# courtois-neuromod/phantom_vlb

Hardware: AMD Instinct MI355X
Metric: clips/sec fine-tune VideoLLaMA2-7B+LoRA->2k-voxel head, 1/2/4/8 MI355X (higher is better)
Workload: dtype bf16; 1 GPU; configs[2]: VideoLLaMA2-7B + LoRA r=16 + 2k-voxel head, bf16; clips_per_gpu=3, global_batch=3, seq_len=2048, frames=12, num_target=2048, weights=random-init, comm=none

## Files before the change

include/vlb.h:

```cpp
#ifndef VLB_H
#define VLB_H

#include <stdint.h>

#ifdef __cplusplus
extern "C" {
#endif
#if defined(__GNUC__) || defined(__clang__)
#pragma GCC visibility push(default)
#endif

#define VLB_OK 0
#define VLB_ERR_INVALID (-1)
#define VLB_ERR_LAUNCH (-2)

#define VLB_ABI_VERSION 2

#define VLB_ACT_NONE 0
#define VLB_ACT_QUICK_GELU 1
#define VLB_ACT_GELU 2
#define VLB_ACT_SILU 3
#define VLB_ACT_SWIGLU_PAIR 4
#define VLB_ACT_SWIGLU_BWD 5

int vlb_abi_version(void);
const char* vlb_last_error(void);

int vlb_gemm_bf16(const void* A, int lda, const void* W, int ldw, void* C, int ldc, int M, int N, int K,
                  const void* bias, const void* residual, int ldr, int act, const void* A2, int lda2,
                  const void* W2, int ldw2, int K2, void* stream);

int vlb_gemm_bf16_ws(const void* A, int lda, const void* W, int ldw, void* C, int ldc, int M, int N, int K,
                     const void* bias, const void* residual, int ldr, int act, const void* A2, int lda2,
                     const void* W2, int ldw2, int K2, void* ws, int64_t ws_bytes, void* stream);
int vlb_gemm_swiglu_save(const void* A, int lda, const void* W_il, int ldw, void* H, int ldh, void* GU, int ldgu, int M, int N,
                         int K, const void* A2, int lda2, const void* W2_il, int ldw2, int K2, void* ws, int64_t ws_bytes,
                         void* stream);
int64_t vlb_gemm_workspace_bytes(void);
int vlb_gemm_plan(int M, int N, int K, int K2, int with_workspace);

int vlb_gemm_bf16_masked_pair(const void* A, int lda, const void* W, int ldw, void* C, int ldc, int M, int N, int K,
                              const void* A2, int lda2, const void* W2, int ldw2, float drop_p, uint32_t seed,
                              void* stream);

int vlb_gemm_bf16_masked_pair_ws(const void* A, int lda, const void* W, int ldw, void* C, int ldc, int M, int N, int K,
                                 const void* A2, int lda2, const void* W2, int ldw2, float drop_p, uint32_t seed,
                                 void* ws, int64_t ws_bytes, void* stream);

int vlb_gemm_masked_pair_swiglu_bwd(const void* dY, int lddy, const void* Wt, int ldw, const void* gu, int ldgu, void* dgu,
                                    int lddgu, int M, int ff, int K, const void* U, int ldu, const void* At, int ldat,
                                    float drop_p, uint32_t seed, void* ws, int64_t ws_bytes, void* stream);

int vlb_gemm_kernel_choice(int M, int N, int K, int K2);

int vlb_transpose_bf16(const void* in, void* out, int R, int C, void* stream);

int vlb_attention_fwd(const void* q, int ldq, const void* k, int ldk, const void* v, int ldv, void* out, int ldo,
                      float* lse, const uint8_t* key_mask, int B, int S, int Hq, int Hkv, int D, int causal,
                      float scale, const int* cu_rows, void* stream);

int vlb_attention_bwd(const void* q, int ldq, const void* k, int ldk, const void* v, int ldv, const void* out,
                      int ldo, const void* dout, int lddo, const float* lse, const uint8_t* key_mask, void* dq,
                      int lddq, void* dk, int lddk, void* dv, int lddv, float* delta, float* dq_acc, int B, int S,
                      int Hq, int Hkv, int D, int causal, float scale, const int* cu_rows, int total_rows,
                      void* stream);

int vlb_rmsnorm_fwd(const void* x, const void* w, void* y, int rows, int dim, float eps, void* stream);
int vlb_rmsnorm_bwd(const void* x, const void* w, const void* dy, const void* dx_in, void* dx, int rows, int dim,
                    float eps, void* stream);
int vlb_layernorm_fwd(const void* x, const void* w, const void* b, const void* residual, void* y, int rows, int dim,
                      float eps, int act, void* stream);

int vlb_rope_inplace(void* x, int ld, const float* cos_t, const float* sin_t, int rows, int S, int heads, int D,
                     int sign, const int* pos, void* stream);
int vlb_swiglu_fwd(const void* gu, void* out, int rows, int ff, void* stream);
int vlb_swiglu_bwd(const void* gu, const void* dout, void* dgu, int rows, int ff, void* stream);
int vlb_add_bf16(const void* a, const void* b, void* y, int64_t n, void* stream);

int vlb_patchify(const float* vision, void* patches, int N, int H, int W, int P, int Kpad, void* stream);
int vlb_vit_assemble(const void* patch_emb, const void* cls, const void* pos, void* tokens, int N, int G, int D,
                     void* stream);
int vlb_drop_cls(const void* tokens, void* out, int N, int G, int D, void* stream);

int vlb_dwconv3x3(const void* x, const void* w, void* y, int N, int H, int W, int C, void* stream);
int vlb_se_pool(const void* x, void* pooled, int N, int HW, int C, void* stream);
int vlb_se_scale(const void* x, const void* gate, void* y, int N, int HW, int C, void* stream);
int vlb_im2col3d_k2s2p1(const void* x, void* cols, int B, int T, int H, int W, int C, void* stream);

int vlb_splice_embed(const int64_t* ids, const void* embed_w, const void* video_tokens, void* embeds,
                     uint8_t* key_mask, int* err_flag, int B, int L, int Nv, int D, int64_t video_id, int vocab,
                     const int* cu_rows, int* row_pos, void* stream);
int vlb_weight_mask(const int64_t* padvals, const double* vis_w, const double* lang_w, float* wmask, int B, int F,
                    int Lw, int tokens_per_frame, int S, int round_bf16, void* stream);

int vlb_head_partial_rows(int S);
int64_t vlb_head_ws_floats(int B, int S, int E, int V);
int vlb_head_fwd(const void* hidden, const float* wmask, const void* ln1_w, const void* ln1_b, const void* ln2_w,
                 const void* ln2_b, const void* ridge_w, const void* ridge_b, const float* y, const float* keep_scale,
                 float* ws, float* stats, float* pooled_raw, float* sumw, float* zhat, float* ln2_rstd, void* z,
                 float* pred, float* loss_terms, int B, int S, int E, int V, float eps, float l2_lambda, const int* cu_rows,
                 void* stream);
int vlb_head_bwd(const void* hidden, const float* wmask, const void* ln1_w, const void* ln2_w, const void* ridge_w,
                 const float* y, const float* keep_scale, const float* stats, const float* pooled_raw,
                 const float* sumw, const float* zhat, const float* ln2_rstd, const void* z, const float* pred,
                 float* d_ridge_w, float* d_ridge_b, float* d_ln2_w, float* d_ln2_b, float* d_ln1_w, float* d_ln1_b,
                 float* ws, float* dz_ws, float* dpooled_ws, void* dhidden, int B, int S, int E, int V, float eps,
                 float l2_lambda, float loss_scale, float l2_scale, const int* cu_rows, int total_rows, void* stream);

int vlb_feature_cache_store(const float* pooled_raw, const float* sumw, const int32_t* rows, float* cache_pooled,
                            float* cache_sumw, int B, int E, int n_rows, void* stream);
int vlb_head_fwd_cached(const float* cache_pooled, const float* cache_sumw, const int32_t* rows, const void* ln1_w,
                        const void* ln1_b, const void* ln2_w, const void* ln2_b, const void* ridge_w, const void* ridge_b,
                        const float* y, const float* keep_scale, float* ws, float* pooled_raw, float* sumw, float* zhat,
                        float* ln2_rstd, void* z, float* pred, float* loss_terms, int B, int E, int V, int n_rows, float eps,
                        float l2_lambda, void* stream);
int vlb_head_bwd_cached(const void* ln1_w, const void* ln2_w, const void* ridge_w, const float* y, const float* keep_scale,
                        const float* pooled_raw, const float* sumw, const float* zhat, const float* ln2_rstd, const void* z,
                        const float* pred, float* d_ridge_w, float* d_ridge_b, float* d_ln2_w, float* d_ln2_b, float* d_ln1_w,
                        float* d_ln1_b, float* ws, float* dz_ws, float* dpooled_ws, int B, int E, int V, float eps,
                        float l2_lambda, float loss_scale, float l2_scale, void* stream);

int vlb_lora_down(const void* x, int ldx, const void* A, void* t, int ldt, int M, int K, int R, float scale,
                  float drop_p, const uint32_t* seeds_host, void* stream);
int vlb_lora_merge(const void* W, int ldw, void* Wm, int ldwm, const void* Bt, const void* A, int N, int K, int R, float scale,
                   int row_map, void* stream);
int vlb_lora_dx_masked(const void* u, int ldu, const void* At, int ldat, void* dx, int lddx, int M, int K, int R, float drop_p,
                       const uint32_t* seeds_host, void* stream);
int64_t vlb_wgrad_u_ws_floats(int M, int K);
int vlb_wgrad_skinny_u(const void* G, int ldg, const void* X, int ldx, float* dW, float* ws, int M, int K, float alpha,
                       float beta, const void* Bt, float u_scale, void* u, int ldu, float* u_ws, void* stream);
int vlb_wgrad_skinny_u_multi(const void* G, int ldg, const void* X, int ldx, int M, int nproj, const int* cols, float* const* dW,
                             const void* const* Bt, float* ws, float alpha, float beta, float u_scale, void* u, int ldu,
                             float* u_ws, void* stream);
int vlb_transpose16_scatter(const void* jobs, int n_jobs, void* stream);
int vlb_wgrad_splits(int M);
int vlb_wgrad_skinny(const void* G, int ldg, const void* X, int ldx, float* dW, float* ws, int M, int N, int K,
                     float alpha, float beta, float drop_p, const uint32_t* seeds_host, void* stream);

int vlb_sumsq_ws_floats(void);
int vlb_grad_sumsq(const float* g, int64_t n, float* sumsq, float* ws, void* stream);
int vlb_adamw_step(float* master, void* param_bf16, const float* grad, float* m, float* v, int64_t n, float lr,
                   float beta1, float beta2, float eps, float weight_decay, int step, const float* sumsq,
                   float max_norm, void* stream);
int vlb_grad_accum(float* acc, const float* g, int64_t n, int first, float* sumsq, float* ws, void* stream);
int vlb_grad_accum_bf16(float* acc, const void* g_bf16, int64_t n, int first, float* sumsq, float* ws, void* stream);

int vlb_transpose_pad(const void* in, int ld_in, void* out, int ld_out, int R, int C, int Rpad, void* stream);
int64_t vlb_norm_bwd_ws_floats(int rows, int dim);
int64_t vlb_colsum_ws_floats(int rows, int dim);
int vlb_rmsnorm_bwd_dw(const void* x, const void* dy, void* dw_bf16, float* ws, int rows, int dim, float eps, void* stream);
int64_t vlb_rmsnorm_bwd_full_ws_floats(int rows, int dim);
int vlb_rmsnorm_bwd_full(const void* x, const void* w, const void* dy, const void* dx_in, void* dx, void* dw_bf16, float* ws,
                         int rows, int dim, float eps, void* stream);
int vlb_layernorm_bwd(const void* x, const void* w, const void* b, const void* residual, const void* dy, void* dx, void* dres,
                      void* dw_bf16, void* db_bf16, float* ws, int rows, int dim, float eps, int act, void* stream);
int vlb_act_fwd(const void* x, void* y, int64_t n, int act, void* stream);
int vlb_act_bwd(const void* x, const void* dy, void* dx, int64_t n, int act, void* stream);
int vlb_colsum(const void* x, int ld, void* out_bf16, float* ws, int rows, int dim, void* stream);
int vlb_embed_grad(const void* d_embeds, int ld, const int* tok, const int* beg, const int* rows, int n_tokens, void* dE, int D,
                   void* stream);
int vlb_grad_sumsq_bf16(const void* g, int64_t n, float* sumsq, float* ws, void* stream);
int vlb_adamw_step_g16(float* master, void* param_bf16, const void* grad_bf16, float* m, float* v, int64_t n, float lr,
                       float beta1, float beta2, float eps, float weight_decay, int step, const float* sumsq, float max_norm,
                       void* stream);
int64_t vlb_dwconv3x3_bwd_w_ws_floats(int N, int H, int C);
int vlb_dwconv3x3_bwd_w(const void* x, const void* dy, void* dw9_bf16, float* ws, int N, int H, int W, int C, void* stream);
int vlb_se_bwd_gate(const void* x, const void* dy, const void* s, void* ds, int N, int HW, int C, void* stream);
int vlb_se_bwd_x(const void* dy, const void* s, const void* dpool, void* dx, int N, int HW, int C, void* stream);
int vlb_col2im3d_k2s2p1(const void* dcols, void* dx, int B, int T, int H, int W, int C, void* stream);

int vlb_quantize_mxfp8(const void* x_bf16, int ldx, void* q, int ldq, void* scales, int lds, int rows, int K, void* stream);
int vlb_transpose_quantize_mxfp8(const void* x_bf16, int ldx, void* q, int ldq, void* scales, int lds, int R, int C, int Rpad,
                                 void* stream);
int vlb_quantize_dual_mxfp8(const void* x_bf16, int ldx, void* q, int ldq, void* scales, int lds, void* qt, int ldqt, void* scales_t,
                            int ldst, int R, int C, int Rpad, void* stream);
int vlb_rmsnorm_fwd_mxfp8(const void* x, const void* w, void* y, void* q, int ldq, void* scales, int lds, int rows, int dim, float eps,
                          void* stream);
int vlb_swiglu_fwd_mxfp8(const void* gu, void* out, void* q, int ldq, void* scales, int lds, int rows, int ff, void* stream);
int vlb_gemm_mxfp8(const void* Aq, int lda, const void* sA, int ldsa, const void* Wq, int ldw, const void* sW, int ldsw, void* C,
                   int ldc, int M, int N, int K, const void* residual, int ldr, void* stream);

int vlb_comm_unique_id(void* id128_host);
int vlb_comm_init(int rank, int world, const void* id128_host, void** comm_out);
int vlb_comm_destroy(void* comm);
int64_t vlb_comm_loopback_stage_bytes(int world);
int vlb_comm_init_loopback(int world, void* stage, int64_t stage_bytes, void** comms_out);
int vlb_comm_rank(void* comm);
int vlb_comm_world(void* comm);
int vlb_allgather_direct(void* comm, const void* shard, void* full, int64_t shard_bytes, void* stream);
int64_t vlb_reducescatter_stage_floats(int64_t n_per_rank, int world);
int vlb_reducescatter_direct(void* comm, const float* send, float* out, int64_t n_per_rank, float* stage, void* stream);
int vlb_reducescatter_direct_bf16(void* comm, const void* send, void* out, int64_t n_per_rank, void* stage, void* stream);
int vlb_reduce_slices(const void* stage, void* out, int64_t n_per_rank, int world, int is_bf16, void* stream);
int vlb_allreduce_scalar(void* comm, float* values, int count, void* stream);

int64_t vlb_hrf_pool_ws_floats(int B, int E);
int vlb_hrf_pool(const void* embeddings, int emb_is_f32, const float* weights, void* out, float* ws, int B, int S, int E, void* stream);
int64_t vlb_ridge_ws_floats(int V);
int vlb_ridge_fwd(const void* x, const void* ridge_w, const void* ridge_b, float* pred, float* l2_out, float* ws, int B, int E, int V,
                  float l2_lambda, void* stream);

int vlb_dropout_keep_scale(float* out, int64_t n, float p, uint32_t seed, void* stream);

int vlb_profile_marker(void* stream);
int vlb_cast_f32_to_bf16(const float* in, void* out, int64_t n, void* stream);
int vlb_cast_bf16_to_f32(const void* in, float* out, int64_t n, void* stream);

#if defined(__GNUC__) || defined(__clang__)
#pragma GCC visibility pop
#endif
#ifdef __cplusplus
}
#endif
#endif
```

phantom_vlb_amd/_lib.py:

```python
from __future__ import annotations

import ctypes
import os
from ctypes import c_char_p, c_double, c_float, c_int, c_int64, c_void_p

import torch

_HERE = os.path.dirname(os.path.abspath(__file__))
LIB_PATH = os.environ.get("VLB_LIB") or os.path.join(_HERE, "libvlb.so")
IS_PRODUCT_LIB = os.path.abspath(LIB_PATH) == os.path.join(_HERE, "libvlb.so")

P, I, F, L = c_void_p, c_int, c_float, c_int64

SIGNATURES = {
    "vlb_abi_version": [],
    "vlb_last_error": [],
    "vlb_gemm_bf16": [P, I, P, I, P, I, I, I, I, P, P, I, I, P, I, P, I, I, P],
    "vlb_gemm_bf16_ws": [P, I, P, I, P, I, I, I, I, P, P, I, I, P, I, P, I, I, P, L, P],
    "vlb_gemm_swiglu_save": [P, I, P, I, P, I, P, I, I, I, I, P, I, P, I, I, P, L, P],
    "vlb_gemm_workspace_bytes": [],
    "vlb_gemm_plan": [I, I, I, I, I],
    "vlb_gemm_kernel_choice": [I, I, I, I],
    "vlb_transpose_bf16": [P, P, I, I, P],
    "vlb_attention_fwd": [P, I, P, I, P, I, P, I, P, P, I, I, I, I, I, I, F, P, P],
    "vlb_attention_bwd": [P, I, P, I, P, I, P, I, P, I, P, P, P, I, P, I, P, I, P, P, I, I, I, I, I, I, F, P, I, P],
    "vlb_rmsnorm_fwd": [P, P, P, I, I, F, P],
    "vlb_rmsnorm_bwd": [P, P, P, P, P, I, I, F, P],
    "vlb_layernorm_fwd": [P, P, P, P, P, I, I, F, I, P],
    "vlb_rope_inplace": [P, I, P, P, I, I, I, I, I, P, P],
    "vlb_swiglu_fwd": [P, P, I, I, P],
    "vlb_swiglu_bwd": [P, P, P, I, I, P],
    "vlb_add_bf16": [P, P, P, L, P],
    "vlb_patchify": [P, P, I, I, I, I, I, P],
    "vlb_vit_assemble": [P, P, P, P, I, I, I, P],
    "vlb_drop_cls": [P, P, I, I, I, P],
    "vlb_dwconv3x3": [P, P, P, I, I, I, I, P],
    "vlb_se_pool": [P, P, I, I, I, P],
    "vlb_se_scale": [P, P, P, I, I, I, P],
    "vlb_im2col3d_k2s2p1": [P, P, I, I, I, I, I, P],
    "vlb_splice_embed": [P, P, P, P, P, P, I, I, I, I, L, I, P, P, P],
    "vlb_weight_mask": [P, P, P, P, I, I, I, I, I, I, P],
    "vlb_head_partial_rows": [I],
    "vlb_head_ws_floats": [I, I, I, I],
    "vlb_head_fwd": [P] * 19 + [I, I, I, I, F, F, P, P],
    "vlb_head_bwd": [P] * 24 + [I, I, I, I, F, F, F, F, P, I, P],
    "vlb_feature_cache_store": [P] * 5 + [I, I, I, P],
    "vlb_head_fwd_cached": [P] * 19 + [I, I, I, I, F, F, P],
    "vlb_head_bwd_cached": [P] * 20 + [I, I, I, F, F, F, F, P],
    "vlb_gemm_bf16_masked_pair": [P, I, P, I, P, I, I, I, I, P, I, P, I, F, ctypes.c_uint32, P],
    "vlb_gemm_masked_pair_swiglu_bwd": [P, I, P, I, P, I, P, I, I, I, I, P, I, P, I, F, ctypes.c_uint32, P, L, P],
    "vlb_gemm_bf16_masked_pair_ws": [P, I, P, I, P, I, I, I, I, P, I, P, I, F, ctypes.c_uint32, P, L, P],
    "vlb_wgrad_u_ws_floats": [I, I],
    "vlb_wgrad_skinny_u": [P, I, P, I, P, P, I, I, F, F, P, F, P, I, P, P],
    "vlb_wgrad_skinny_u_multi": [P, I, P, I, I, I, P, P, P, P, F, F, F, P, I, P, P],
    "vlb_transpose16_scatter": [P, I, P],
    "vlb_wgrad_splits": [I],
    "vlb_wgrad_skinny": [P, I, P, I, P, P, I, I, I, F, F, F, P, P],
    "vlb_lora_down": [P, I, P, P, I, I, I, I, F, F, P, P],
    "vlb_lora_merge": [P, I, P, I, P, P, I, I, I, F, I, P],
    "vlb_lora_dx_masked": [P, I, P, I, P, I, I, I, I, F, P, P],
    "vlb_sumsq_ws_floats": [],
    "vlb_grad_sumsq": [P, L, P, P, P],
    "vlb_adamw_step": [P, P, P, P, P, L, F, F, F, F, F, I, P, F, P],
    "vlb_grad_accum": [P, P, L, I, P, P, P],
    "vlb_grad_accum_bf16": [P, P, L, I, P, P, P],
    "vlb_dropout_keep_scale": [P, L, F, ctypes.c_uint32, P],
    "vlb_transpose_pad": [P, I, P, I, I, I, I, P],
    "vlb_norm_bwd_ws_floats": [I, I],
    "vlb_colsum_ws_floats": [I, I],
    "vlb_rmsnorm_bwd_dw": [P, P, P, P, I, I, F, P],
    "vlb_rmsnorm_bwd_full_ws_floats": [I, I],
    "vlb_rmsnorm_bwd_full": [P, P, P, P, P, P, P, I, I, F, P],
    "vlb_layernorm_bwd": [P, P, P, P, P, P, P, P, P, P, I, I, F, I, P],
    "vlb_act_fwd": [P, P, L, I, P],
    "vlb_act_bwd": [P, P, P, L, I, P],
    "vlb_colsum": [P, I, P, P, I, I, P],
    "vlb_embed_grad": [P, I, P, P, P, I, P, I, P],
    "vlb_grad_sumsq_bf16": [P, L, P, P, P],
    "vlb_adamw_step_g16": [P, P, P, P, P, L, F, F, F, F, F, I, P, F, P],
    "vlb_dwconv3x3_bwd_w_ws_floats": [I, I, I],
    "vlb_dwconv3x3_bwd_w": [P, P, P, P, I, I, I, I, P],
    "vlb_se_bwd_gate": [P, P, P, P, I, I, I, P],
    "vlb_se_bwd_x": [P, P, P, P, I, I, I, P],
    "vlb_col2im3d_k2s2p1": [P, P, I, I, I, I, I, P],
    "vlb_quantize_mxfp8": [P, I, P, I, P, I, I, I, P],
    "vlb_transpose_quantize_mxfp8": [P, I, P, I, P, I, I, I, I, P],
    "vlb_quantize_dual_mxfp8": [P, I, P, I, P, I, P, I, P, I, I, I, I, P],
    "vlb_rmsnorm_fwd_mxfp8": [P, P, P, P, I, P, I, I, I, F, P],
    "vlb_swiglu_fwd_mxfp8": [P, P, P, I, P, I, I, I, P],
    "vlb_gemm_mxfp8": [P, I, P, I, P, I, P, I, P, I, I, I, I, P, I, P],
    "vlb_comm_unique_id": [P],
    "vlb_comm_init": [I, I, P, ctypes.POINTER(c_void_p)],
    "vlb_comm_destroy": [P],
    "vlb_comm_loopback_stage_bytes": [I],
    "vlb_comm_init_loopback": [I, P, L, ctypes.POINTER(c_void_p)],
    "vlb_comm_rank": [P],
    "vlb_comm_world": [P],
    "vlb_allgather_direct": [P, P, P, L, P],
    "vlb_reducescatter_stage_floats": [L, I],
    "vlb_reducescatter_direct": [P, P, P, L, P, P],
    "vlb_reducescatter_direct_bf16": [P, P, P, L, P, P],
    "vlb_reduce_slices": [P, P, L, I, I, P],
    "vlb_profile_marker": [P],
    "vlb_hrf_pool_ws_floats": [I, I],
    "vlb_hrf_pool": [P, I, P, P, P, I, I, I, P],
    "vlb_ridge_ws_floats": [I],
    "vlb_ridge_fwd": [P, P, P, P, P, P, I, I, I, F, P],
    "vlb_allreduce_scalar": [P, P, I, P],
    "vlb_cast_f32_to_bf16": [P, P, L, P],
    "vlb_cast_bf16_to_f32": [P, P, L, P],
}
_RESTYPES = {"vlb_last_error": c_char_p, "vlb_hrf_pool_ws_floats": c_int64, "vlb_ridge_ws_floats": c_int64, "vlb_head_ws_floats": c_int64, "vlb_wgrad_u_ws_floats": c_int64,
             "vlb_gemm_workspace_bytes": c_int64, "vlb_reducescatter_stage_floats": c_int64, "vlb_comm_loopback_stage_bytes": c_int64,
             "vlb_norm_bwd_ws_floats": c_int64, "vlb_rmsnorm_bwd_full_ws_floats": c_int64, "vlb_colsum_ws_floats": c_int64, "vlb_dwconv3x3_bwd_w_ws_floats": c_int64}


class VlbError(RuntimeError):
    pass


def _load():
    if not os.path.exists(LIB_PATH):
        raise ImportError(
            f"{LIB_PATH} is missing: build it with `python -c 'import __graft_entry__ as g; g.build()'` "
            f"or `make -C phantom_vlb_amd/csrc`.  phantom_vlb_amd has no CPU fallback.")
    lib = ctypes.CDLL(LIB_PATH)
    for name, argtypes in SIGNATURES.items():
        try:
            fn = getattr(lib, name)
        except AttributeError as e:
            raise ImportError(f"libvlb.so does not export {name}: rebuild it") from e
        fn.argtypes = argtypes
        fn.restype = _RESTYPES.get(name, c_int)
    if lib.vlb_abi_version() != 2:
        raise ImportError("libvlb.so ABI version mismatch")
    return lib


lib = _load()


def check(rc: int, what: str = "") -> None:
    if rc != 0:
        raise VlbError(f"{what} failed ({rc}): {lib.vlb_last_error().decode()}")
```

phantom_vlb_amd/backbone.py:

```python
from __future__ import annotations

import math

import torch

from . import ops
from .geometry import Geometry, VIDEO_TOKEN_ID

BF16 = torch.bfloat16
V_PRE = "model.vision_tower.vision_tower.vision_model"
M_PRE = "model.mm_projector"


def _bf(t, dev):
    return t.detach().to(device=dev, dtype=BF16).contiguous()


class Weights:

    def __init__(self, g: Geometry, sd: dict, device, keep_transposed: bool = False, gate_up_interleaved: bool | None = None):
        self.g = g
        self.dev = device
        d = device
        w = sd[f"{V_PRE}.embeddings.patch_embedding.weight"].reshape(g.vit_dim, -1)
# ... 51 lines not shown
                                    sd[f"{p}.self_attn.v_proj.weight"]], 0), d),
                wo=_bf(sd[f"{p}.self_attn.o_proj.weight"], d),
                wdown=_bf(sd[f"{p}.mlp.down_proj.weight"], d))
            il = (not keep_transposed) if gate_up_interleaved is None else gate_up_interleaved
            wgu = _bf(torch.cat([sd[f"{p}.mlp.gate_proj.weight"], sd[f"{p}.mlp.up_proj.weight"]], 0), d)
            if keep_transposed:
                lw["wgu"] = wgu
                for k in ("wqkv", "wo", "wgu", "wdown"):
                    lw[k + "_t"] = ops.transpose(lw[k])
                if il:
                    del lw["wgu"]
            if il:
                lw["wgu_il"] = ops.interleave_gate_up(wgu[:g.ff], wgu[g.ff:])
            del wgu
            self.layers.append(lw)
        self.final_norm = _bf(sd["model.norm.weight"], d)
        inv = 1.0 / (g.rope_theta ** (torch.arange(0, g.head_dim, 2, dtype=torch.float32) / g.head_dim))
        fr = torch.arange(g.max_len, dtype=torch.float32)[:, None] * inv[None]
        self.rope_cos = fr.cos().to(d).contiguous()
        self.rope_sin = fr.sin().to(d).contiguous()

    @staticmethod
    def random_state_dict(g: Geometry, device, seed: int = 1234, dtype=BF16) -> dict:
        gen = torch.Generator(device=device).manual_seed(seed)

        def rn(*shape, std=0.02):
            return (torch.randn(*shape, generator=gen, device=device, dtype=torch.float32) * std).to(dtype)

        def ones(n):
            return torch.ones(n, device=device, dtype=dtype)

        def zeros(n):
            return torch.zeros(n, device=device, dtype=dtype)
        sd = {}
        sd[f"{V_PRE}.embeddings.class_embedding"] = rn(g.vit_dim)
        sd[f"{V_PRE}.embeddings.patch_embedding.weight"] = rn(g.vit_dim, 3, g.patch, g.patch)
        sd[f"{V_PRE}.embeddings.position_embedding.weight"] = rn(g.grid * g.grid + 1, g.vit_dim)
        sd[f"{V_PRE}.pre_layrnorm.weight"] = ones(g.vit_dim)
        sd[f"{V_PRE}.pre_layrnorm.bias"] = zeros(g.vit_dim)
        for i in range(g.vit_layers):
            p = f"{V_PRE}.encoder.layers.{i}"
            for ln in ("layer_norm1", "layer_norm2"):
                sd[f"{p}.{ln}.weight"] = ones(g.vit_dim)
                sd[f"{p}.{ln}.bias"] = zeros(g.vit_dim)
            for n in ("q_proj", "k_proj", "v_proj", "out_proj"):
                sd[f"{p}.self_attn.{n}.weight"] = rn(g.vit_dim, g.vit_dim)
                sd[f"{p}.self_attn.{n}.bias"] = zeros(g.vit_dim)
            sd[f"{p}.mlp.fc1.weight"] = rn(g.vit_ff, g.vit_dim)
            sd[f"{p}.mlp.fc1.bias"] = zeros(g.vit_ff)
            sd[f"{p}.mlp.fc2.weight"] = rn(g.vit_dim, g.vit_ff)
            sd[f"{p}.mlp.fc2.bias"] = zeros(g.vit_dim)
        for st, cin in (("s1", g.vit_dim), ("s2", g.dim)):
            for b in range(g.proj_depth):
                ci = cin if b == 0 else g.dim
                q = f"{M_PRE}.{st}.b{b + 1}"
                rd = int(round(ci * g.proj_se_ratio))
                sd[f"{q}.conv1.conv.weight"] = rn(g.dim, ci, 1, 1, std=1 / math.sqrt(ci))
                sd[f"{q}.conv2.conv.weight"] = rn(g.dim, 1, 3, 3, std=1 / 3)
                sd[f"{q}.se.fc1.weight"] = rn(rd, g.dim, 1, 1, std=1 / math.sqrt(g.dim))
                sd[f"{q}.se.fc1.bias"] = zeros(rd)
                sd[f"{q}.se.fc2.weight"] = rn(g.dim, rd, 1, 1, std=1 / math.sqrt(rd))
                sd[f"{q}.se.fc2.bias"] = zeros(g.dim)
                sd[f"{q}.conv3.conv.weight"] = rn(g.dim, g.dim, 1, 1, std=1 / math.sqrt(g.dim))
                for n in ("conv1", "conv2", "conv3"):
                    sd[f"{q}.{n}.bn.weight"] = ones(g.dim)
                    sd[f"{q}.{n}.bn.bias"] = zeros(g.dim)
                if ci != g.dim:
                    sd[f"{q}.downsample.conv.weight"] = rn(g.dim, ci, 1, 1, std=1 / math.sqrt(ci))
                    sd[f"{q}.downsample.bn.weight"] = ones(g.dim)
                    sd[f"{q}.downsample.bn.bias"] = zeros(g.dim)
        sd[f"{M_PRE}.sampler.0.weight"] = rn(g.dim, g.dim, 2, 2, 2, std=1 / math.sqrt(8 * g.dim))
        sd[f"{M_PRE}.sampler.0.bias"] = zeros(g.dim)
        for n in ("readout.0", "readout.2"):
            sd[f"{M_PRE}.{n}.weight"] = rn(g.dim, g.dim, std=1 / math.sqrt(g.dim))
            sd[f"{M_PRE}.{n}.bias"] = zeros(g.dim)
        sd["model.embed_tokens.weight"] = rn(g.vocab, g.dim)
        for i in range(g.layers):
            p = f"model.layers.{i}"
            sd[f"{p}.self_attn.q_proj.weight"] = rn(g.heads * g.head_dim, g.dim)
            sd[f"{p}.self_attn.k_proj.weight"] = rn(g.kv_heads * g.head_dim, g.dim)
            sd[f"{p}.self_attn.v_proj.weight"] = rn(g.kv_heads * g.head_dim, g.dim)
            sd[f"{p}.self_attn.o_proj.weight"] = rn(g.dim, g.heads * g.head_dim)
            sd[f"{p}.mlp.gate_proj.weight"] = rn(g.ff, g.dim)
            sd[f"{p}.mlp.up_proj.weight"] = rn(g.ff, g.dim)
            sd[f"{p}.mlp.down_proj.weight"] = rn(g.dim, g.ff)
            sd[f"{p}.input_layernorm.weight"] = ones(g.dim)
            sd[f"{p}.post_attention_layernorm.weight"] = ones(g.dim)
        sd["model.norm.weight"] = ones(g.dim)
        return sd


class Backbone:

    def __init__(self, g: Geometry, weights: Weights):
        self.g = g
        self.w = weights
        self.err_flag = torch.zeros(1, dtype=torch.int32, device=weights.dev)

    def vision_tower(self, vision_f32):
        g, w = self.g, self.w
        N = vision_f32.shape[0]
        G, T = g.grid * g.grid, g.grid * g.grid + 1
        hd = g.vit_dim // g.vit_heads
        patches = ops.patchify(vision_f32, g.patch, g.patch_k_padded)
        pe = ops.gemm(patches, w.patch_w)
        x = ops.vit_assemble(pe, w.cls, w.pos, N, G, g.vit_dim)
        x = ops.layernorm(x, *w.pre_ln, g.vit_eps)
        D = g.vit_dim
        for lw in w.vit:
            h = ops.layernorm(x, *lw["ln1"], g.vit_eps)
            qkv = ops.gemm(h, lw["wqkv"], bias=lw["bqkv"])
            a = ops.attention_fwd(qkv[:, :D], qkv[:, D:2 * D], qkv[:, 2 * D:], N, T, g.vit_heads, g.vit_heads, hd,
                                  False, hd ** -0.5)
            x = ops.gemm(a, lw["wo"], bias=lw["bo"], residual=x)
            h = ops.layernorm(x, *lw["ln2"], g.vit_eps)
            h = ops.gemm(h, lw["w1"], bias=lw["b1"], act=ops.ACT_QUICK_GELU)
            x = ops.gemm(h, lw["w2"], bias=lw["b2"], residual=x)
        return ops.drop_cls(x, N, G, D)

    def _bottleneck(self, x, blk, N, H):
        g = self.g
        C = g.dim
        y = ops.gemm(x, blk["conv1"])
        y = ops.layernorm(y, *blk["bn1"], g.proj_eps, act=ops.ACT_SILU)
        y = ops.dwconv3x3(y, blk["dw"], N, H, H, C)
        y = ops.layernorm(y, *blk["bn2"], g.proj_eps, act=ops.ACT_SILU)
        s = ops.se_pool(y, N, H * H, C)
        s = ops.gemm(s, blk["se1"], bias=blk["se1b"], act=ops.ACT_SILU)
        s = ops.gemm(s, blk["se2"], bias=blk["se2b"])
        y = ops.se_scale(y, s, N, H * H, C, out=y)
        y = ops.gemm(y, blk["conv3"])
        sc = x
        if "ds" in blk:
            sc = ops.layernorm(ops.gemm(x, blk["ds"]), *blk["dsbn"], g.proj_eps)
        return ops.layernorm(y, *blk["bn3"], g.proj_eps, residual=sc, act=ops.ACT_SILU)

    def connector(self, feats, B):
        g, w = self.g, self.w
        x = feats
        for blk in w.s1:
            x = self._bottleneck(x, blk, B * g.num_frames, g.grid)
        cols = ops.im2col3d(x, B, g.num_frames, g.grid, g.grid, g.dim)
        x = ops.gemm(cols, w.sampler_w, bias=w.sampler_b, act=ops.ACT_SILU)
        for blk in w.s2:
            x = self._bottleneck(x, blk, B * g.ds_frames, g.ds_grid)
        x = ops.gemm(x, w.ro0[0], bias=w.ro0[1], act=ops.ACT_GELU)
        return ops.gemm(x, w.ro2[0], bias=w.ro2[1])

    def decoder_layer(self, x, lw, key_mask, B, S, save=None, layout=None):
        g = self.g
        qd, kd = g.heads * g.head_dim, g.kv_heads * g.head_dim
        h = ops.rmsnorm(x, lw["in_norm"], g.rms_eps)
        qkv = ops.gemm(h, lw["wqkv"])
        ops.rope_(qkv, self.w.rope_cos, self.w.rope_sin, B, S, g.heads + g.kv_heads, g.head_dim,
                  pos=None if layout is None else layout.pos)
        a = ops.attention_fwd(qkv[:, :qd], qkv[:, qd:qd + kd], qkv[:, qd + kd:], B, S, g.heads, g.kv_heads, g.head_dim,
                              True, g.head_dim ** -0.5, key_mask=key_mask, layout=layout)
        x = ops.gemm(a, lw["wo"], residual=x)
        h = ops.rmsnorm(x, lw["post_norm"], g.rms_eps)
        if lw.get("wgu_il") is not None:
            h = ops.gemm(h, lw["wgu_il"], act=ops.ACT_SWIGLU_PAIR)
        else:
            h = ops.swiglu(ops.gemm(h, lw["wgu"]))
        return ops.gemm(h, lw["wdown"], residual=x)

    def named_modules(self):
        from .litmodule import _LinearInfo
        g = self.g
        qd, kd = g.heads * g.head_dim, g.kv_heads * g.head_dim
        for i in range(g.vit_layers):
            p = f"{V_PRE}.encoder.layers.{i}"
            for n in ("q_proj", "k_proj", "v_proj", "out_proj"):
                yield f"{p}.self_attn.{n}", _LinearInfo(g.vit_dim, g.vit_dim)
            yield f"{p}.mlp.fc1", _LinearInfo(g.vit_ff, g.vit_dim)
            yield f"{p}.mlp.fc2", _LinearInfo(g.vit_dim, g.vit_ff)
        for n in ("readout.0", "readout.2"):
            yield f"{M_PRE}.{n}", _LinearInfo(g.dim, g.dim)
        for i in range(g.layers):
            p = f"model.layers.{i}"
            yield f"{p}.self_attn.q_proj", _LinearInfo(qd, g.dim)
            yield f"{p}.self_attn.k_proj", _LinearInfo(kd, g.dim)
            yield f"{p}.self_attn.v_proj", _LinearInfo(kd, g.dim)
            yield f"{p}.self_attn.o_proj", _LinearInfo(g.dim, qd)
            yield f"{p}.mlp.gate_proj", _LinearInfo(g.ff, g.dim)
            yield f"{p}.mlp.up_proj", _LinearInfo(g.ff, g.dim)
            yield f"{p}.mlp.down_proj", _LinearInfo(g.dim, g.ff)
        yield "lm_head", _LinearInfo(g.vocab, g.dim)

    def splice(self, ids, video_tokens, layout=None):
        g = self.g
        return ops.splice_embed(ids, self.w.embed, video_tokens, g.vis_tokens, VIDEO_TOKEN_ID, self.err_flag, layout)

    def row_layout(self, ids_host=None, padvals=None):
        g = self.g
        if ids_host is None or ids_host.device.type != "cpu":
            return None
        B, L = ids_host.shape
        S = L - 1 + g.vis_tokens
        nz = ids_host != 0
        last = L - 1 - torch.flip(nz, dims=[1]).to(torch.int8).argmax(dim=1)
        lens = (last + g.vis_tokens).clamp(max=S)
        lens = torch.where(nz.any(dim=1), lens, torch.full_like(lens, S))
        if padvals is not None:
            lens = torch.maximum(lens, S - padvals[:, 0].to(lens.dtype).cpu().clamp(min=0))
        return ops.RowLayout(B, S, lens.tolist(), device=self.w.dev)

    def enable_sharding(self, group=None, comm=None):
        from .parallel import ShardedLayerStore
        if getattr(self, "trainable_decoder", False):
            raise ValueError("enable_sharding(): the decoder weights train in this configuration (full fine-tune); "
                             "only frozen decoder weights can be sharded per layer")
        side = torch.cuda.Stream(device=self.w.dev)
        keys = tuple(k for k in ("wqkv", "wo", "wgu", "wgu_il", "wdown") if k in self.w.layers[0])
        self.store = ShardedLayerStore(self.w.layers, keys, group, stream=side, comm=comm)
        self.store_t = None
        if "wqkv_t" in self.w.layers[0]:
            tkeys = ("wqkv_t", "wo_t", "wgu_t", "wdown_t")
            self.store_t = ShardedLayerStore(self.w.layers, tkeys, group, stream=side, comm=comm)
        for lw in self.w.layers:
            for k in list(lw):
                if k in keys or k.endswith("_t"):
                    lw[k] = None
        torch.cuda.empty_cache()

    def layer_weights(self, i, transposed=False, direction=1):
        lw = self.w.layers[i]
        store = getattr(self, "store_t" if transposed else "store", None)
        if store is None:
            return lw
        full = store.get(i)
        store.prefetch(i + direction)
        return {**lw, **full}

    def decoder(self, x, key_mask, B, S, layer_outputs=None, layout=None, layers=None):
        for i in range(len(self.w.layers)):
            lw = self.layer_weights(i) if layers is None else layers[i]
            x = self.decoder_layer(x, lw, key_mask, B, S, layout=layout)
            if layer_outputs is not None:
                layer_outputs.append(x)
        return ops.rmsnorm(x, self.w.final_norm, self.g.rms_eps)

    MAX_AHEAD = 4

    def _vision_compute(self, vision_f32, tower_only):
        g, B = self.g, vision_f32.shape[0]
        feats = self.vision_tower(vision_f32.reshape(B * g.num_frames, 3, g.image_size, g.image_size))
        return feats if tower_only else self.connector(feats, B)

    def prefetch_video_tokens(self, vision_f32, ready_event=None, tower_only=False):
        dev = self.w.dev
        if getattr(self, "_vis_stream", None) is None:
            self._vis_stream = torch.cuda.Stream(device=dev)
        if getattr(self, "_vis_queue", None) is None:
            self._vis_queue = []
        st = self._vis_stream
        if ready_event is not None:
            st.wait_event(ready_event)
        else:
            st.wait_stream(torch.cuda.current_stream(dev))
        with torch.cuda.stream(st):
            vid = self._vision_compute(vision_f32, tower_only)
            ev = torch.cuda.Event()
            ev.record(st)
        vision_f32.record_stream(st)
        self._vis_queue.append((vision_f32, vision_f32._version, tower_only, vid, ev))
        del self._vis_queue[:-self.MAX_AHEAD]

    def defer_video_tokens(self, vision_f32, ready_event=None, tower_only=False):
        if getattr(self, "_vis_pending", None) is None:
            self._vis_pending = []
        self._vis_pending.append((vision_f32, vision_f32._version, tower_only, ready_event))
        del self._vis_pending[:-self.MAX_AHEAD]

    def launch_deferred_video_tokens(self):
        pend, self._vis_pending = getattr(self, "_vis_pending", None) or [], []
        for vis, ver, tower_only, ev in pend:
            if vis._version == ver:
                self.prefetch_video_tokens(vis, ev, tower_only=tower_only)

    def discard_video_tokens(self, vision_f32=None):
        for name in ("_vis_queue", "_vis_pending"):
            q = getattr(self, name, None)
            if q:
                q[:] = [e for e in q if vision_f32 is not None and e[0] is not vision_f32]

    def video_tokens(self, vision_f32, tower_only=False):
        q = getattr(self, "_vis_queue", None)
        cur = torch.cuda.current_stream(self.w.dev)
        if q:
            for i, (vis, ver, t_only, vid, ev) in enumerate(q):
                if vis is not vision_f32:
                    continue
                del q[i]
                if ver != vision_f32._version or (t_only is False and tower_only):
                    break
                cur.wait_event(ev)
                vid.record_stream(cur)
                if t_only and not tower_only:
                    return self.connector(vid, vision_f32.shape[0])
                return vid
        pend = getattr(self, "_vis_pending", None)
        if pend:
            for i, (vis, ver, t_only, ev) in enumerate(pend):
                if vis is vision_f32:
                    del pend[i]
                    if ev is not None:
                        cur.wait_event(ev)
                    break
        return self._vision_compute(vision_f32, tower_only)

# ... 17 lines not shown
```

phantom_vlb_amd/csrc/attention.hip:

```cpp
#include "common.hpp"

namespace {

constexpr int KV = 64;
constexpr int QW = 32;
constexpr int NW = 4;
constexpr int QB = QW * NW;
constexpr float NEG = -1e30f;

__device__ __forceinline__ void glds16(const void* g, void* l) {
  __builtin_amdgcn_global_load_lds((const void __attribute__((address_space(1)))*)g,
                                   (void __attribute__((address_space(3)))*)l, 16, 0, 0);
}

typedef short s16x4 __attribute__((ext_vector_type(4)));

__device__ __forceinline__ s16x4 tr_read_asm(const char* lds_ptr) {
  s16x4 v;
  const unsigned a = (unsigned)(uintptr_t)(const char __attribute__((address_space(3)))*)lds_ptr;
  asm volatile("ds_read_b64_tr_b16 %0, %1" : "=v"(v) : "v"(a));
  return v;
}
__device__ __forceinline__ void lds_wait_all() {
  asm volatile("s_waitcnt lgkmcnt(0)" ::: "memory");
  __builtin_amdgcn_sched_barrier(0);
}
__device__ __forceinline__ bf16x8 join8(s16x4 lo, s16x4 hi) {
  typedef short s16x8 __attribute__((ext_vector_type(8)));
  return __builtin_bit_cast(bf16x8, (s16x8)__builtin_shufflevector(lo, hi, 0, 1, 2, 3, 4, 5, 6, 7));
}

struct AttnArgs {
  const bf16* q; const bf16* k; const bf16* v; bf16* o; float* lse;
  const uint8_t* mask;
  const int* cu;
  int ldq, ldk, ldv, ldo;
  int B, S, Hq, Hkv;
  float scale;
};

template <int D> __device__ __forceinline__ int slot_k(int r, int c) {
  if constexpr (D == 128) return c ^ (r & 15); else return c ^ ((r >> 1) & 7);
}
template <int D> __device__ __forceinline__ int slot_v(int r, int c) {
  if constexpr (D == 128) return c ^ ((r & 3) << 2); else return c ^ (((r >> 1) & 1) << 2);
}

__device__ __forceinline__ int xcd_head(int j, int Hq) {
  return (Hq & 7) == 0 ? (j & 7) * (Hq >> 3) + (j >> 3) : j;
}

template <int D, bool CAUSAL>
__global__ __launch_bounds__(256, 2) void attn_fwd_kernel(AttnArgs p) {
  constexpr int CPR = D / 8;
  constexpr int ROWB = D * 2;
  constexpr int TILE = KV * ROWB;
  constexpr int LD = (KV * CPR) / 256;
  constexpr int KS = D / 16;
  constexpr int DT = D / 32;
  extern __shared__ __attribute__((aligned(16))) char smem[];

  const int tid = threadIdx.x, lane = tid & 63;
  const int wave = __builtin_amdgcn_readfirstlane(tid >> 6);
  const int nqb = (p.S + QB - 1) / QB;
  const int per_qb = p.Hq * p.B, slot = blockIdx.x / per_qb;
  const int qb = CAUSAL ? (nqb - 1 - slot) : slot;
  const int hq = xcd_head((blockIdx.x % per_qb) % p.Hq, p.Hq), b = (blockIdx.x % per_qb) / p.Hq;
  const int hkv = hq / (p.Hq / p.Hkv);
  const int Sb = p.cu ? p.cu[b + 1] - p.cu[b] : p.S;
  const int64_t row0 = p.cu ? p.cu[b] : (int64_t)b * p.S;
  if (qb * QB >= Sb) return;
  const int q0 = qb * QB + wave * QW;
  const int ql = lane & 31, h = lane >> 5;

  bf16x8 qf[KS];
  {
    const int qr = min(q0 + ql, Sb - 1);
    const bf16* qp = p.q + (row0 + qr) * p.ldq + hq * D + 8 * h;
#pragma unroll
    for (int ks = 0; ks < KS; ++ks) qf[ks] = *reinterpret_cast<const bf16x8*>(qp + 16 * ks);
  }

  f32x16 ot[DT];
#pragma unroll
  for (int i = 0; i < DT; ++i)
#pragma unroll
    for (int r = 0; r < 16; ++r) ot[i][r] = 0.f;
  float m_run = NEG, l_run = 0.f;
  const float c2 = p.scale * 1.44269504088896341f;

  const int q_hi = min(qb * QB + QB, Sb) - 1;
  const int ntiles = CAUSAL ? (q_hi / KV + 1) : (Sb + KV - 1) / KV;

  const bf16* kbase = p.k + row0 * p.ldk + hkv * D;
  const bf16* vbase = p.v + row0 * p.ldv + hkv * D;

  constexpr int RPI = 1024 / ROWB;
  const int sr = lane / CPR, sp = lane % CPR;
  auto stage = [&](int buf, int t) {
    char* kb = smem + buf * 2 * TILE; char* vb = kb + TILE;
#pragma unroll
    for (int i = 0; i < LD; ++i) {
      const int r = (4 * i + wave) * RPI + sr;
      const int key = min(t * KV + r, Sb - 1);
      glds16(kbase + (int64_t)key * p.ldk + slot_k<D>(r, sp) * 8, kb + (4 * i + wave) * 1024);
      glds16(vbase + (int64_t)key * p.ldv + slot_v<D>(r, sp) * 8, vb + (4 * i + wave) * 1024);
    }
  };

  stage(0, 0);
  asm volatile("s_waitcnt vmcnt(0)" ::: "memory");
  __syncthreads();

  const int g1 = (lane >> 4) & 1, li = lane & 15, tq = li >> 2, tp = li & 3;
  int k_rd[KS], v_rd[DT];
#pragma unroll
  for (int ks = 0; ks < KS; ++ks) k_rd[ks] = ql * ROWB + slot_k<D>(ql, 2 * ks + h) * 16;
#pragma unroll
  for (int dt = 0; dt < DT; ++dt) {
    const int r0 = 4 * h + tq;
    v_rd[dt] = r0 * ROWB + slot_v<D>(r0, 4 * dt + 2 * g1 + (tp >> 1)) * 16 + (tp & 1) * 8;
  }

  for (int t = 0; t < ntiles; ++t) {
    const int cur = t & 1;
    const bool more = (t + 1 < ntiles);
    if (more) stage(cur ^ 1, t + 1);
    const char* kb = smem + cur * 2 * TILE; const char* vb = kb + TILE;
    const int key0 = t * KV;
    const bool active = !CAUSAL || (key0 <= q0 + QW - 1);
    if (active) {
      f32x16 st[2];
#pragma unroll
      for (int s = 0; s < 2; ++s)
#pragma unroll
        for (int r = 0; r < 16; ++r) st[s][r] = 0.f;
#pragma unroll
      for (int ks = 0; ks < KS; ++ks) {
#pragma unroll
        for (int s = 0; s < 2; ++s) {
          const bf16x8 kf = *reinterpret_cast<const bf16x8*>(kb + k_rd[ks] + 32 * s * ROWB);
          st[s] = __builtin_amdgcn_mfma_f32_32x32x16_bf16(kf, qf[ks], st[s], 0, 0, 0);
        }
      }
      unsigned long long kvalid;
      {
        const int key = key0 + lane;
        bool ok = key < Sb;
        if (ok && p.mask) ok = p.mask[row0 + key] != 0;
        kvalid = __ballot(ok);
      }
      const bool diag = CAUSAL && (key0 + KV - 1 > q0);
      const bool partial = diag || (kvalid != ~0ull);
      if (partial) {
        const int qrow = q0 + ql;
        const unsigned lo = (unsigned)(kvalid >> (4 * h)), hi = (unsigned)(kvalid >> (32 + 4 * h));
#pragma unroll
        for (int s = 0; s < 2; ++s) {
          const unsigned word = s ? hi : lo;
#pragma unroll
          for (int r = 0; r < 16; ++r) {
            const int kb = (r & 3) + 8 * (r >> 2);
            bool ok = (word >> kb) & 1u;
            if (CAUSAL) ok = ok && (key0 + 32 * s + 4 * h + kb <= qrow);
            st[s][r] = ok ? st[s][r] : NEG;
          }
        }
        asm volatile("" ::: "memory");
      }
      float mloc = fmaxf(st[0][0], st[1][0]);
#pragma unroll
      for (int r = 1; r < 16; ++r) mloc = fmaxf(fmaxf(mloc, st[0][r]), st[1][r]);
      mloc = fmaxf(mloc, __shfl_xor(mloc, 32, 64));
      const float m_new = fmaxf(m_run, mloc);
      const float alpha = __builtin_amdgcn_exp2f((m_run - m_new) * c2);
      const float mc = m_new * c2;
      float lsum = 0.f;
      const float live = (m_new > 0.5f * NEG) ? 1.f : 0.f;
#pragma unroll
      for (int s = 0; s < 2; ++s)
#pragma unroll
        for (int r = 0; r < 16; ++r) {
          const float e = __builtin_amdgcn_exp2f(st[s][r] * c2 - mc);
          st[s][r] = e;
          lsum += e;
        }
      if (partial && live == 0.f) {
#pragma unroll
        for (int s = 0; s < 2; ++s)
#pragma unroll
          for (int r = 0; r < 16; ++r) st[s][r] = 0.f;
        lsum = 0.f;
      }
      l_run = l_run * alpha + lsum;
      m_run = m_new;
#pragma unroll
      for (int i = 0; i < DT; ++i)
#pragma unroll
        for (int r = 0; r < 16; ++r) ot[i][r] *= alpha;
#pragma unroll
      for (int s = 0; s < 2; ++s)
#pragma unroll
        for (int s2 = 0; s2 < 2; ++s2) {
          bf16x8 pf;
#pragma unroll
          for (int j = 0; j < 8; ++j) pf[j] = (bf16)st[s][8 * s2 + j];
          const int roff = (32 * s + 16 * s2) * ROWB;
#pragma unroll
          for (int dt = 0; dt < DT; ++dt) {
            const s16x4 lo = __builtin_amdgcn_ds_read_tr16_b64_v4i16(
                (s16x4 __attribute__((address_space(3)))*)(vb + v_rd[dt] + roff));
            const s16x4 hi = __builtin_amdgcn_ds_read_tr16_b64_v4i16(
                (s16x4 __attribute__((address_space(3)))*)(vb + v_rd[dt] + roff + 8 * ROWB));
            ot[dt] = __builtin_amdgcn_mfma_f32_32x32x16_bf16(join8(lo, hi), pf, ot[dt], 0, 0, 0);
          }
        }
    }
    asm volatile("s_waitcnt vmcnt(0)" ::: "memory");
    __syncthreads();
  }

  const float l_tot = l_run + __shfl_xor(l_run, 32, 64);
  const float inv = l_tot > 0.f ? 1.f / l_tot : 0.f;
  const int qrow = q0 + ql;
  if (qrow < Sb) {
    bf16* op = p.o + (row0 + qrow) * p.ldo + hq * D;
#pragma unroll
    for (int dt = 0; dt < DT; ++dt)
#pragma unroll
      for (int g = 0; g < 4; ++g) {
        bf16x4 o;
#pragma unroll
        for (int e = 0; e < 4; ++e) o[e] = (bf16)(ot[dt][4 * g + e] * inv);
        *reinterpret_cast<bf16x4*>(op + 32 * dt + 8 * g + 4 * h) = o;
      }
    if (p.lse && h == 0)
      p.lse[((int64_t)b * p.Hq + hq) * p.S + qrow] = l_tot > 0.f ? m_run * p.scale + logf(l_tot) : -INFINITY;
  }
}

template <int D, bool CAUSAL>
int launch_fwd(const AttnArgs& a, hipStream_t s) {
  constexpr int LDS = 2 * 2 * KV * D * 2;
  static const hipError_t attr = hipFuncSetAttribute(reinterpret_cast<const void*>(&attn_fwd_kernel<D, CAUSAL>),
                                                     hipFuncAttributeMaxDynamicSharedMemorySize, LDS);
  if (attr != hipSuccess) { vlb_set_error("attention: LDS reservation failed: %s", hipGetErrorString(attr)); return VLB_ERR_LAUNCH; }
  dim3 grid(((a.S + QB - 1) / QB) * a.Hq * a.B);
  hipLaunchKernelGGL((attn_fwd_kernel<D, CAUSAL>), grid, dim3(256), LDS, s, a);
  VLB_LAUNCH_CHECK();
  return VLB_OK;
}
}

extern "C" int vlb_attention_fwd(const void* q, int ldq, const void* k, int ldk, const void* v, int ldv, void* out,
                                 int ldo, float* lse, const uint8_t* key_mask, int B, int S, int Hq, int Hkv, int D,
                                 int causal, float scale, const int* cu_rows, void* stream) {
  VLB_REQUIRE(q && k && v && out, "attention_fwd: null operand");
  VLB_REQUIRE(D == 64 || D == 128, "attention_fwd: head dim %d not in {64,128}", D);
  VLB_REQUIRE(B > 0 && S > 0 && Hq > 0 && Hkv > 0 && Hq % Hkv == 0, "attention_fwd: bad shape B=%d S=%d Hq=%d Hkv=%d", B, S, Hq, Hkv);
  VLB_REQUIRE(ldq % 8 == 0 && ldk % 8 == 0 && ldv % 8 == 0 && ldo % 4 == 0, "attention_fwd: strides must keep 16-byte alignment");
  VLB_REQUIRE((((uintptr_t)q | (uintptr_t)k | (uintptr_t)v) % 16 == 0) && ((uintptr_t)out % 8 == 0), "attention_fwd: misaligned pointer");
  AttnArgs a{(const bf16*)q, (const bf16*)k, (const bf16*)v, (bf16*)out, lse, key_mask, cu_rows, ldq, ldk, ldv, ldo, B, S, Hq, Hkv, scale};
  hipStream_t s = as_stream(stream);
  if (D == 128) return causal ? launch_fwd<128, true>(a, s) : launch_fwd<128, false>(a, s);
  return causal ? launch_fwd<64, true>(a, s) : launch_fwd<64, false>(a, s);
}

namespace {

constexpr int BK_KEYS = 128;
constexpr int BQ = 32;

#ifdef VLB_TOOLS
int g_attn_ablate = 0;
#else
constexpr int g_attn_ablate = 0;
#endif
struct AttnBwdArgs {
  const bf16* q; const bf16* k; const bf16* v; const bf16* dout;
  const float* lse; const float* delta; const uint8_t* mask; const int* cu;
  bf16* dk; bf16* dv; float* dq_acc;
  int ldq, ldk, ldv, lddo, lddk, lddv;
  int B, S, Hq, Hkv;
  float scale;
  int ablate;
};

__device__ __forceinline__ int sw2(int r) { return ((r & 3) << 2) | ((r >> 2) & 3); }

__global__ __launch_bounds__(256) void attn_delta_kernel(const bf16* __restrict__ o, int ldo, const bf16* __restrict__ d_o,
                                                         int lddo, float* __restrict__ delta, int S, int Hq, int B,
                                                         const int* __restrict__ cu, int64_t total) {
  const int64_t gid = (int64_t)blockIdx.x * 16 + (threadIdx.x >> 4);
  const int c = threadIdx.x & 15;
  float s = 0.f;
  if (gid < total) {
    const int h = gid % Hq; const int64_t tok = gid / Hq;
    const bf16x8 a = *reinterpret_cast<const bf16x8*>(o + tok * ldo + h * 128 + c * 8);
    const bf16x8 b = *reinterpret_cast<const bf16x8*>(d_o + tok * lddo + h * 128 + c * 8);
#pragma unroll
    for (int i = 0; i < 8; ++i) s += (float)a[i] * (float)b[i];
  }
#pragma unroll
  for (int off = 8; off > 0; off >>= 1) s += __shfl_xor(s, off, 64);
  if (gid < total && c == 0) {
    const int h = gid % Hq; const int64_t tok = gid / Hq;
    int64_t b = tok / S; int sidx = tok % S;
    if (cu) {
      int bb = 0;
      while (bb + 1 < B && tok >= cu[bb + 1]) ++bb;
      b = bb; sidx = (int)(tok - cu[bb]);
    }
    delta[(b * Hq + h) * S + sidx] = s;
  }
}

template <bool CAUSAL>
__global__ __launch_bounds__(256, 2) void attn_bwd_dkdv_kernel(AttnBwdArgs p, bf16* __restrict__ part) {
  constexpr int D = 128, ROWB = 256;
  constexpr int V_OFF = 0;
  constexpr int QT_BYTES = BQ * ROWB;
  constexpr int Q_OFF = BK_KEYS * ROWB;
  constexpr int L_OFF = Q_OFF + 4 * QT_BYTES;
  extern __shared__ __attribute__((aligned(16))) char smem[];

  const int tid = threadIdx.x, lane = tid & 63;
  const int w4 = __builtin_amdgcn_readfirstlane(tid >> 6);
  const int per_kb = p.Hq * p.B;
  const int kb = blockIdx.x / per_kb, hq = xcd_head((blockIdx.x % per_kb) % p.Hq, p.Hq), b = (blockIdx.x % per_kb) / p.Hq;
  const int gsz = p.Hq / p.Hkv;
  const int hkv = hq / gsz;
  const int k0 = kb * BK_KEYS;
  const int Sb = p.cu ? p.cu[b + 1] - p.cu[b] : p.S;
  const int64_t row0 = p.cu ? p.cu[b] : (int64_t)b * p.S;
  if (k0 >= Sb) return;
  const int ql = lane & 31, h = lane >> 5;
  const int g1 = (lane >> 4) & 1, li = lane & 15, tq = li >> 2, tp = li & 3;
  const int sr = lane >> 4, sp = lane & 15;

  const int krow = w4 * 32 + ql;
  const int key = k0 + krow;
  bf16x8 kf[8];
  {
    const bf16* kp = p.k + (row0 + min(key, Sb - 1)) * p.ldk + hkv * D + 8 * h;
#pragma unroll
    for (int ks = 0; ks < 8; ++ks) kf[ks] = *reinterpret_cast<const bf16x8*>(kp + 16 * ks);
  }
  const bf16* vbase = p.v + row0 * p.ldv + hkv * D;
#pragma unroll
  for (int i = 0; i < 8; ++i) {
    const int piece = 4 * i + w4, r = piece * 4 + sr;
    glds16(vbase + (int64_t)min(k0 + r, Sb - 1) * p.ldv + (sp ^ sw2(r)) * 8, smem + V_OFF + piece * 1024);
  }
  const int nqb = (Sb + BQ - 1) / BQ;
  const int qb0 = CAUSAL ? (k0 / BQ) : 0;
  const int total = nqb - qb0;
  const bf16* qbase = p.q + row0 * p.ldq + hq * D;
  const bf16* dobase = p.dout + row0 * p.lddo + hq * D;
  const float* lsebase = p.lse + ((int64_t)b * p.Hq + hq) * p.S;
  const float* delbase = p.delta + ((int64_t)b * p.Hq + hq) * p.S;

  auto stage_q = [&](int buf, int item) {
    const int qb = qb0 + item;
    char* qt = smem + Q_OFF + buf * 2 * QT_BYTES;
#pragma unroll
    for (int i = 0; i < 2; ++i) {
      const int piece = 4 * i + w4, r = piece * 4 + sr;
      const int qr = min(qb * BQ + r, Sb - 1);
      glds16(qbase + (int64_t)qr * p.ldq + (sp ^ sw2(r)) * 8, qt + piece * 1024);
      glds16(dobase + (int64_t)qr * p.lddo + (sp ^ sw2(r)) * 8, qt + QT_BYTES + piece * 1024);
    }
    if (w4 == 0) {
      const int qr = min(qb * BQ + (lane & 31), Sb - 1);
      const float* src = (lane < 32 ? lsebase : delbase) + qr;
      __builtin_amdgcn_global_load_lds((const void __attribute__((address_space(1)))*)src,
                                       (void __attribute__((address_space(3)))*)(smem + L_OFF + buf * 256), 4, 0, 0);
    }
  };

  f32x16 dkt[4], dvt[4];
#pragma unroll
  for (int i = 0; i < 4; ++i)
#pragma unroll
    for (int r = 0; r < 16; ++r) { dkt[i][r] = 0.f; dvt[i][r] = 0.f; }

  if (total > 0) stage_q(0, 0);
  asm volatile("s_waitcnt vmcnt(0)" ::: "memory");
  __syncthreads();

  const int v_base = krow * ROWB, v_x = h ^ sw2(krow);
  const int q_base = ql * ROWB, q_x = h ^ sw2(ql);
  int qt_rd[4][2];
#pragma unroll
  for (int dt = 0; dt < 4; ++dt)
#pragma unroll
    for (int e = 0; e < 2; ++e) {
      const int r = 8 * e + 4 * h + tq;
      qt_rd[dt][e] = r * ROWB + (((4 * dt + 2 * g1 + (tp >> 1)) ^ sw2(r)) << 4) + (tp & 1) * 8;
    }

  const float c2 = p.scale * 1.44269504088896341f;
  bool key_ok = key < Sb;
  if (key_ok && p.mask) key_ok = p.mask[row0 + key] != 0;

  for (int item = 0; item < total; ++item) {
    const int cur = item & 1;
    if (item + 1 < total) stage_q(cur ^ 1, item + 1);
    const char* qt = smem + Q_OFF + cur * 2 * QT_BYTES;
    const char* dot = qt + QT_BYTES;
    const float* ls = reinterpret_cast<const float*>(smem + L_OFF) + cur * 64;
    const int q0 = (qb0 + item) * BQ;
    const bool active = !CAUSAL || (k0 + w4 * 32 <= q0 + BQ - 1);
    if (active) {
      f32x16 sacc, pacc;
#pragma unroll
      for (int r = 0; r < 16; ++r) { sacc[r] = 0.f; pacc[r] = 0.f; }
#pragma unroll
      for (int ks = 0; ks < 8; ++ks) {
        const bf16x8 qf = *reinterpret_cast<const bf16x8*>(qt + q_base + (((2 * ks) ^ q_x) << 4));
        sacc = __builtin_amdgcn_mfma_f32_32x32x16_bf16(qf, kf[ks], sacc, 0, 0, 0);
        const bf16x8 dof = *reinterpret_cast<const bf16x8*>(dot + q_base + (((2 * ks) ^ q_x) << 4));
        const bf16x8 vf = *reinterpret_cast<const bf16x8*>(smem + V_OFF + v_base + (((2 * ks) ^ v_x) << 4));
        pacc = __builtin_amdgcn_mfma_f32_32x32x16_bf16(dof, vf, pacc, 0, 0, 0);
      }
      bf16x8 pb[2], dsb[2];
#pragma unroll
      for (int g = 0; g < 4; ++g) {
        const f32x4 l4 = *reinterpret_cast<const f32x4*>(ls + 8 * g + 4 * h);
        const f32x4 d4 = *reinterpret_cast<const f32x4*>(ls + 32 + 8 * g + 4 * h);
#pragma unroll
        for (int e = 0; e < 4; ++e) {
          const int r = 4 * g + e;
          const int qrow = q0 + 8 * g + 4 * h + e;
          bool ok = key_ok && qrow < Sb;
          if (CAUSAL) ok = ok && (key <= qrow);
          const float pv = ok ? __builtin_amdgcn_exp2f(sacc[r] * c2 - l4[e] * 1.44269504088896341f) : 0.f;
          const float ds = pv * (pacc[r] - d4[e]) * p.scale;
          pb[r >> 3][r & 7] = (bf16)pv;
          dsb[r >> 3][r & 7] = (bf16)ds;
        }
      }
#pragma unroll
      for (int s = 0; s < 2; ++s) {
        s16x4 ra[4][2];
#pragma unroll
        for (int dt = 0; dt < 4; ++dt)
#pragma unroll
          for (int e = 0; e < 2; ++e) ra[dt][e] = tr_read_asm(dot + qt_rd[dt][e] + 16 * s * ROWB);
        lds_wait_all();
#pragma unroll
        for (int dt = 0; dt < 4; ++dt)
          dvt[dt] = __builtin_amdgcn_mfma_f32_32x32x16_bf16(join8(ra[dt][0], ra[dt][1]), pb[s], dvt[dt], 0, 0, 0);
#pragma unroll
        for (int dt = 0; dt < 4; ++dt)
#pragma unroll
          for (int e = 0; e < 2; ++e) ra[dt][e] = tr_read_asm(qt + qt_rd[dt][e] + 16 * s * ROWB);
        lds_wait_all();
#pragma unroll
        for (int dt = 0; dt < 4; ++dt)
          dkt[dt] = __builtin_amdgcn_mfma_f32_32x32x16_bf16(join8(ra[dt][0], ra[dt][1]), dsb[s], dkt[dt], 0, 0, 0);
      }
    }
    asm volatile("s_waitcnt vmcnt(0)" ::: "memory");
    asm volatile("s_waitcnt lgkmcnt(0)" ::: "memory");
    __builtin_amdgcn_s_barrier();
  }

  if (key < Sb) {
    bf16* dkp = gsz == 1 ? p.dk + (row0 + key) * p.lddk + hkv * D : part + ((row0 + key) * p.Hq + hq) * (2 * D);
    bf16* dvp = gsz == 1 ? p.dv + (row0 + key) * p.lddv + hkv * D : dkp + D;
#pragma unroll
    for (int dt = 0; dt < 4; ++dt)
#pragma unroll
      for (int g = 0; g < 4; ++g) {
        bf16x4 a, c;
#pragma unroll
        for (int e = 0; e < 4; ++e) { a[e] = (bf16)dkt[dt][4 * g + e]; c[e] = (bf16)dvt[dt][4 * g + e]; }
        *reinterpret_cast<bf16x4*>(dkp + 32 * dt + 8 * g + 4 * h) = a;
        *reinterpret_cast<bf16x4*>(dvp + 32 * dt + 8 * g + 4 * h) = c;
      }
  }
}

__global__ __launch_bounds__(256) void attn_dkdv_reduce_kernel(const bf16* __restrict__ part, bf16* __restrict__ dk, int lddk,
                                                               bf16* __restrict__ dv, int lddv, int Hq, int Hkv, int64_t total) {
  const int64_t i = blockIdx.x * (int64_t)blockDim.x + threadIdx.x;
  if (i >= total) return;
  const int c = i & 15, which = (i >> 4) & 1;
  const int hkv = (int)((i >> 5) % Hkv);
  const int64_t row = (i >> 5) / Hkv;
  const int gsz = Hq / Hkv;
  float acc[8] = {0.f, 0.f, 0.f, 0.f, 0.f, 0.f, 0.f, 0.f};
  const bf16* src = part + (row * Hq + (int64_t)hkv * gsz) * 256 + which * 128 + c * 8;
  for (int j = 0; j < gsz; ++j) {
    const bf16x8 v = *reinterpret_cast<const bf16x8*>(src + (int64_t)j * 256);
#pragma unroll
    for (int e = 0; e < 8; ++e) acc[e] += (float)v[e];
  }
  bf16x8 o;
#pragma unroll
  for (int e = 0; e < 8; ++e) o[e] = (bf16)acc[e];
  bf16* dst = which ? dv + row * lddv : dk + row * lddk;
  *reinterpret_cast<bf16x8*>(dst + hkv * 128 + c * 8) = o;
}

struct AttnDqArgs {
  const bf16* q; const bf16* k; const bf16* v; const bf16* dout;
  const float* lse; const float* delta; const uint8_t* mask; const int* cu;
  bf16* dq;
  int ldq, ldk, ldv, lddo, lddq;
  int B, S, Hq, Hkv;
  float scale;
};

template <bool CAUSAL>
__global__ __launch_bounds__(256, 2) void attn_bwd_dq_kernel(AttnDqArgs p) {
  constexpr int D = 128, ROWB = 256, TILE = KV * ROWB, KS = 8, DT = 4;
  extern __shared__ __attribute__((aligned(16))) char smem[];

  const int tid = threadIdx.x, lane = tid & 63;
  const int wave = __builtin_amdgcn_readfirstlane(tid >> 6);
  const int nqb = (p.S + QB - 1) / QB;
  const int per_qb = p.Hq * p.B, slot = blockIdx.x / per_qb;
  const int qb = CAUSAL ? (nqb - 1 - slot) : slot;
  const int hq = xcd_head((blockIdx.x % per_qb) % p.Hq, p.Hq), b = (blockIdx.x % per_qb) / p.Hq;
  const int hkv = hq / (p.Hq / p.Hkv);
  const int Sb = p.cu ? p.cu[b + 1] - p.cu[b] : p.S;
  const int64_t row0 = p.cu ? p.cu[b] : (int64_t)b * p.S;
  if (qb * QB >= Sb) return;
  const int q0 = qb * QB + wave * QW;
  const int ql = lane & 31, h = lane >> 5;
  const int qrow = q0 + ql;
  const int qr = min(qrow, Sb - 1);

  bf16x8 qf[KS], dof[KS];
  {
    const bf16* qp = p.q + (row0 + qr) * p.ldq + hq * D + 8 * h;
    const bf16* dp = p.dout + (row0 + qr) * p.lddo + hq * D + 8 * h;
#pragma unroll
    for (int ks = 0; ks < KS; ++ks) {
      qf[ks] = *reinterpret_cast<const bf16x8*>(qp + 16 * ks);
      dof[ks] = *reinterpret_cast<const bf16x8*>(dp + 16 * ks);
    }
  }
  const float lse_q = p.lse[((int64_t)b * p.Hq + hq) * p.S + qr];
  const float delta_q = p.delta[((int64_t)b * p.Hq + hq) * p.S + qr];
  const float c2 = p.scale * 1.44269504088896341f;
  const float lse2 = (lse_q > -1e37f) ? lse_q * 1.44269504088896341f : 1e37f;

  f32x16 dqt[DT];
#pragma unroll
  for (int i = 0; i < DT; ++i)
#pragma unroll
    for (int r = 0; r < 16; ++r) dqt[i][r] = 0.f;

  const int q_hi = min(qb * QB + QB, Sb) - 1;
  const int ntiles = CAUSAL ? (q_hi / KV + 1) : (Sb + KV - 1) / KV;
  const bf16* kbase = p.k + row0 * p.ldk + hkv * D;
  const bf16* vbase = p.v + row0 * p.ldv + hkv * D;

  const int sr = lane >> 4, sp = lane & 15;
  auto stage = [&](int buf, int t) {
    char* kb = smem + buf * 2 * TILE; char* vb = kb + TILE;
#pragma unroll
    for (int i = 0; i < 4; ++i) {
      const int r = (4 * i + wave) * 4 + sr;
      const int key = min(t * KV + r, Sb - 1);
      glds16(kbase + (int64_t)key * p.ldk + (sp ^ sw2(r)) * 8, kb + (4 * i + wave) * 1024);
      glds16(vbase + (int64_t)key * p.ldv + (sp ^ sw2(r)) * 8, vb + (4 * i + wave) * 1024);
    }
  };
  stage(0, 0);
  asm volatile("s_waitcnt vmcnt(0)" ::: "memory");
  __syncthreads();

  const int g1 = (lane >> 4) & 1, li = lane & 15, tq = li >> 2, tp = li & 3;
  int row_rd[KS];
#pragma unroll
  for (int ks = 0; ks < KS; ++ks) row_rd[ks] = ql * ROWB + (((2 * ks + h) ^ sw2(ql)) << 4);
  int tr_rd[DT][2];
#pragma unroll
  for (int dt = 0; dt < DT; ++dt)
#pragma unroll
    for (int e = 0; e < 2; ++e) {
      const int r = 4 * h + tq + 8 * e;
      tr_rd[dt][e] = r * ROWB + (((4 * dt + 2 * g1 + (tp >> 1)) ^ sw2(r)) << 4) + (tp & 1) * 8;
    }

  for (int t = 0; t < ntiles; ++t) {
    const int cur = t & 1;
    if (t + 1 < ntiles) stage(cur ^ 1, t + 1);
    const char* kb = smem + cur * 2 * TILE; const char* vb = kb + TILE;
    const int key0 = t * KV;
    const bool active = !CAUSAL || (key0 <= q0 + QW - 1);
    if (active) {
      f32x16 st[2], dp[2];
#pragma unroll
      for (int s = 0; s < 2; ++s)
#pragma unroll
        for (int r = 0; r < 16; ++r) { st[s][r] = 0.f; dp[s][r] = 0.f; }
#pragma unroll
      for (int ks = 0; ks < KS; ++ks) {
#pragma unroll
        for (int s = 0; s < 2; ++s) {
          const bf16x8 kf = *reinterpret_cast<const bf16x8*>(kb + row_rd[ks] + 32 * s * ROWB);
          st[s] = __builtin_amdgcn_mfma_f32_32x32x16_bf16(kf, qf[ks], st[s], 0, 0, 0);
          const bf16x8 vf = *reinterpret_cast<const bf16x8*>(vb + row_rd[ks] + 32 * s * ROWB);
          dp[s] = __builtin_amdgcn_mfma_f32_32x32x16_bf16(vf, dof[ks], dp[s], 0, 0, 0);
        }
      }
      unsigned long long kvalid;
      {
        const int key = key0 + lane;
        bool ok = key < Sb;
        if (ok && p.mask) ok = p.mask[row0 + key] != 0;
        kvalid = __ballot(ok);
      }
      const bool diag = CAUSAL && (key0 + KV - 1 > q0);
      const bool partial = diag || (kvalid != ~0ull);
      if (partial) {
        const unsigned lo = (unsigned)(kvalid >> (4 * h)), hi = (unsigned)(kvalid >> (32 + 4 * h));
#pragma unroll
        for (int s = 0; s < 2; ++s) {
          const unsigned word = s ? hi : lo;
#pragma unroll
          for (int r = 0; r < 16; ++r) {
            const int kb2 = (r & 3) + 8 * (r >> 2);
            bool ok = (word >> kb2) & 1u;
            if (CAUSAL) ok = ok && (key0 + 32 * s + 4 * h + kb2 <= qrow);
            st[s][r] = ok ? st[s][r] : NEG;
          }
        }
        asm volatile("" ::: "memory");
      }
#pragma unroll
      for (int s = 0; s < 2; ++s)
#pragma unroll
        for (int r = 0; r < 16; ++r) {
          const float pv = __builtin_amdgcn_exp2f(st[s][r] * c2 - lse2);
          st[s][r] = pv * (dp[s][r] - delta_q) * p.scale;
        }
#pragma unroll
      for (int s = 0; s < 2; ++s)
#pragma unroll
        for (int s2 = 0; s2 < 2; ++s2) {
          bf16x8 df;
#pragma unroll
          for (int j = 0; j < 8; ++j) df[j] = (bf16)st[s][8 * s2 + j];
          const int roff = (32 * s + 16 * s2) * ROWB;
#pragma unroll
          for (int dt = 0; dt < DT; ++dt) {
            const s16x4 lo = __builtin_amdgcn_ds_read_tr16_b64_v4i16(
                (s16x4 __attribute__((address_space(3)))*)(kb + tr_rd[dt][0] + roff));
            const s16x4 hi = __builtin_amdgcn_ds_read_tr16_b64_v4i16(
                (s16x4 __attribute__((address_space(3)))*)(kb + tr_rd[dt][1] + roff));
            dqt[dt] = __builtin_amdgcn_mfma_f32_32x32x16_bf16(join8(lo, hi), df, dqt[dt], 0, 0, 0);
          }
        }
    }
    asm volatile("s_waitcnt vmcnt(0)" ::: "memory");
    __syncthreads();
  }

  if (qrow < Sb) {
    bf16* op = p.dq + (row0 + qrow) * p.lddq + hq * D;
#pragma unroll
    for (int dt = 0; dt < DT; ++dt)
#pragma unroll
      for (int g = 0; g < 4; ++g) {
        bf16x4 o;
#pragma unroll
        for (int e = 0; e < 4; ++e) o[e] = (bf16)dqt[dt][4 * g + e];
        *reinterpret_cast<bf16x4*>(op + 32 * dt + 8 * g + 4 * h) = o;
      }
  }
}

}

extern "C" int vlb_attention_bwd(const void* q, int ldq, const void* k, int ldk, const void* v, int ldv, const void* out,
                                 int ldo, const void* dout, int lddo, const float* lse, const uint8_t* key_mask, void* dq,
                                 int lddq, void* dk, int lddk, void* dv, int lddv, float* delta, float* dq_acc, int B,
                                 int S, int Hq, int Hkv, int D, int causal, float scale, const int* cu_rows, int total_rows,
                                 void* stream) {
  VLB_REQUIRE(q && k && v && out && dout && lse && dq && dk && dv && delta, "attention_bwd: null operand");
  VLB_REQUIRE(dq_acc || Hq == Hkv, "attention_bwd: the [rows, Hq, D] fp32-sized workspace is required");
  VLB_REQUIRE(D == 128, "attention_bwd: head dim %d unsupported (only 128: the decoder)", D);
  VLB_REQUIRE(B > 0 && S > 0 && Hq > 0 && Hkv > 0 && Hq % Hkv == 0, "attention_bwd: bad shape");
  VLB_REQUIRE(ldq % 8 == 0 && ldk % 8 == 0 && ldv % 8 == 0 && ldo % 8 == 0 && lddo % 8 == 0 && lddq % 8 == 0 &&
                  lddk % 4 == 0 && lddv % 4 == 0, "attention_bwd: strides must keep vector alignment");
  VLB_REQUIRE(((((uintptr_t)q | (uintptr_t)k | (uintptr_t)v | (uintptr_t)out | (uintptr_t)dout) % 16) == 0) &&
                  ((uintptr_t)dq % 8 == 0), "attention_bwd: misaligned pointer");
  hipStream_t st = as_stream(stream);
  const int64_t rows = cu_rows ? (int64_t)total_rows : (int64_t)B * S;
  VLB_REQUIRE(rows > 0 && rows <= (int64_t)B * S, "attention_bwd: total_rows=%d out of range", total_rows);
  const int64_t th = rows * Hq;
  hipLaunchKernelGGL(attn_delta_kernel, dim3((unsigned)((th + 15) / 16)), dim3(256), 0, st, (const bf16*)out, ldo,
                     (const bf16*)dout, lddo, delta, S, Hq, B, cu_rows, th);
  VLB_LAUNCH_CHECK();
  AttnBwdArgs a{(const bf16*)q, (const bf16*)k, (const bf16*)v, (const bf16*)dout, lse, delta, key_mask, cu_rows,
                (bf16*)dk, (bf16*)dv, dq_acc, ldq, ldk, ldv, lddo, lddk, lddv, B, S, Hq, Hkv, scale, g_attn_ablate};
  dim3 grid((S + BK_KEYS - 1) / BK_KEYS, Hkv, B);
  {
    const int gsz = Hq / Hkv;
    VLB_REQUIRE(gsz == 1 || dq_acc, "attention_bwd: the workspace (fp32 [rows, Hq, D]) is required for grouped-query heads");
    VLB_REQUIRE(lddk % 8 == 0 && lddv % 8 == 0 && (((uintptr_t)dk | (uintptr_t)dv) % 16) == 0, "attention_bwd: dk/dv rows must be 16-byte aligned");
    constexpr int LDS_KV = BK_KEYS * 256 + 4 * BQ * 256 + 512;
    static const hipError_t k1 = hipFuncSetAttribute(reinterpret_cast<const void*>(&attn_bwd_dkdv_kernel<true>), hipFuncAttributeMaxDynamicSharedMemorySize, LDS_KV);
    static const hipError_t k2 = hipFuncSetAttribute(reinterpret_cast<const void*>(&attn_bwd_dkdv_kernel<false>), hipFuncAttributeMaxDynamicSharedMemorySize, LDS_KV);
    if (k1 != hipSuccess || k2 != hipSuccess) { vlb_set_error("attention_bwd: LDS reservation failed (dk/dv)"); return VLB_ERR_LAUNCH; }
    bf16* part = reinterpret_cast<bf16*>(dq_acc);
    dim3 gridh(grid.x * Hq * B);
    if (causal) hipLaunchKernelGGL(attn_bwd_dkdv_kernel<true>, gridh, dim3(256), LDS_KV, st, a, part);
    else hipLaunchKernelGGL(attn_bwd_dkdv_kernel<false>, gridh, dim3(256), LDS_KV, st, a, part);
    VLB_LAUNCH_CHECK();
    if (gsz > 1) {
      const int64_t tot = rows * Hkv * 32;
      hipLaunchKernelGGL(attn_dkdv_reduce_kernel, dim3((unsigned)((tot + 255) / 256)), dim3(256), 0, st, part, (bf16*)dk, lddk,
                         (bf16*)dv, lddv, Hq, Hkv, tot);
      VLB_LAUNCH_CHECK();
    }
  }
  AttnDqArgs d{(const bf16*)q, (const bf16*)k, (const bf16*)v, (const bf16*)dout, lse, delta, key_mask, cu_rows,
               (bf16*)dq, ldq, ldk, ldv, lddo, lddq, B, S, Hq, Hkv, scale};
  constexpr int LDS_DQ = 2 * 2 * KV * 256;
  static const hipError_t q1 = hipFuncSetAttribute(reinterpret_cast<const void*>(&attn_bwd_dq_kernel<true>), hipFuncAttributeMaxDynamicSharedMemorySize, LDS_DQ);
  static const hipError_t q2 = hipFuncSetAttribute(reinterpret_cast<const void*>(&attn_bwd_dq_kernel<false>), hipFuncAttributeMaxDynamicSharedMemorySize, LDS_DQ);
  if (q1 != hipSuccess || q2 != hipSuccess) { vlb_set_error("attention_bwd: LDS reservation failed (dq)"); return VLB_ERR_LAUNCH; }
  dim3 gq(((S + QB - 1) / QB) * Hq * B);
  if (causal) hipLaunchKernelGGL(attn_bwd_dq_kernel<true>, gq, dim3(256), LDS_DQ, st, d);
  else hipLaunchKernelGGL(attn_bwd_dq_kernel<false>, gq, dim3(256), LDS_DQ, st, d);
  VLB_LAUNCH_CHECK();
  return VLB_OK;
}

#ifdef VLB_TOOLS
extern "C" void vlb_attn_set_ablation(int bits) { g_attn_ablate = bits & 3; }
#endif
```

phantom_vlb_amd/csrc/common.hpp:

```cpp
#pragma once
#include <hip/hip_runtime.h>
#include <stdint.h>
#include <stdio.h>
#include <string.h>

#include "../../include/vlb.h"

typedef __bf16 bf16;
typedef __bf16 bf16x2 __attribute__((ext_vector_type(2)));
typedef __bf16 bf16x4 __attribute__((ext_vector_type(4)));
typedef __bf16 bf16x8 __attribute__((ext_vector_type(8)));
typedef float f32x2 __attribute__((ext_vector_type(2)));
typedef float f32x4 __attribute__((ext_vector_type(4)));
typedef float f32x16 __attribute__((ext_vector_type(16)));
typedef unsigned int u32x2 __attribute__((ext_vector_type(2)));
typedef unsigned int u32x4 __attribute__((ext_vector_type(4)));

#define VLB_WAVE 64

void vlb_set_error(const char* fmt, ...);

#define VLB_REQUIRE(cond, ...)                 \
  do {                                         \
    if (!(cond)) {                             \
      vlb_set_error(__VA_ARGS__);              \
      return VLB_ERR_INVALID;                  \
    }                                          \
  } while (0)

#define VLB_LAUNCH_CHECK()                                                   \
  do {                                                                       \
    hipError_t e__ = hipGetLastError();                                      \
    if (e__ != hipSuccess) {                                                 \
      vlb_set_error("%s:%d launch failed: %s", __FILE__, __LINE__,           \
                    hipGetErrorString(e__));                                 \
      return VLB_ERR_LAUNCH;                                                 \
    }                                                                        \
  } while (0)

static inline hipStream_t as_stream(void* s) {
  (void)hipGetLastError();
  return reinterpret_cast<hipStream_t>(s);
}

__device__ __forceinline__ float bf2f(bf16 x) { return (float)x; }
__device__ __forceinline__ bf16 f2bf(float x) { return (bf16)x; }

__device__ __forceinline__ float wave_sum(float v) {
#pragma unroll
  for (int o = 32; o > 0; o >>= 1) v += __shfl_xor(v, o, 64);
  return v;
}
__device__ __forceinline__ float wave_max(float v) {
#pragma unroll
  for (int o = 32; o > 0; o >>= 1) v = fmaxf(v, __shfl_xor(v, o, 64));
  return v;
}

__device__ __forceinline__ float block_sum(float v, float* red) {
  v = wave_sum(v);
  const int w = threadIdx.x >> 6, nw = blockDim.x >> 6;
  __syncthreads();
  if ((threadIdx.x & 63) == 0) red[w] = v;
  __syncthreads();
  float t = 0.f;
  for (int i = 0; i < nw; ++i) t += red[i];
  return t;
}

__device__ __forceinline__ float sigmoid_f(float x) { return __builtin_amdgcn_rcpf(1.f + __expf(-x)); }
__device__ __forceinline__ float silu_f(float x) { return x * sigmoid_f(x); }
__device__ __forceinline__ float quick_gelu_f(float x) { return x * sigmoid_f(1.702f * x); }
__device__ __forceinline__ float gelu_erf_f(float x) { return 0.5f * x * (1.f + erff(x * 0.70710678118654752f)); }

__device__ __forceinline__ int mx_shared_exp(float amax) {
  int E = -127;
  if (amax > 0.f) {
    int e; const float f = frexpf(amax / 448.f, &e);
    E = (f == 0.5f) ? e - 1 : e;
    E = max(-127, min(127, E));
  }
  return E;
}
__device__ __forceinline__ uint32_t mx_pack4(float a, float b, float c, float d, float inv) {
  int pk = 0;
  pk = __builtin_amdgcn_cvt_pk_fp8_f32(a * inv, b * inv, pk, false);
  pk = __builtin_amdgcn_cvt_pk_fp8_f32(c * inv, d * inv, pk, true);
  return (uint32_t)pk;
}
__device__ __forceinline__ void mx_quantize_lane8(const float (&v)[8], uint8_t* qrow, uint8_t* srow, int c, int lane) {
  float amax = 0.f;
#pragma unroll
  for (int i = 0; i < 8; ++i) amax = fmaxf(amax, fabsf(v[i]));
  amax = fmaxf(amax, __shfl_xor(amax, 1, 64));
  amax = fmaxf(amax, __shfl_xor(amax, 2, 64));
  const int E = mx_shared_exp(amax);
  const float inv = exp2f((float)-E);
  typedef unsigned u32x2_ __attribute__((ext_vector_type(2)));
  *reinterpret_cast<u32x2_*>(qrow + c) = u32x2_{mx_pack4(v[0], v[1], v[2], v[3], inv), mx_pack4(v[4], v[5], v[6], v[7], inv)};
  if ((lane & 3) == 0) srow[c >> 5] = (uint8_t)(E + 127);
}
__device__ __forceinline__ void load_pair16(const bf16* row, int n, int fq, bf16x4& a, bf16x4& b) {
  typedef unsigned u32x2 __attribute__((ext_vector_type(2)));
  typedef unsigned u32x4 __attribute__((ext_vector_type(4)));
  const u32x4 l = *reinterpret_cast<const u32x4*>(row + n + ((fq & 1) ? 12 : 0));
  const auto r0 = __builtin_amdgcn_permlane16_swap(l[0], l[2], false, false);
  const auto r1 = __builtin_amdgcn_permlane16_swap(l[1], l[3], false, false);
  a = __builtin_bit_cast(bf16x4, u32x2{r0[0], r1[0]});
  b = __builtin_bit_cast(bf16x4, u32x2{r0[1], r1[1]});
}
__device__ __forceinline__ void store_pair16(bf16* row, int n, bf16x4 a, bf16x4 b, int fq) {
  typedef unsigned u32x2 __attribute__((ext_vector_type(2)));
  typedef unsigned u32x4 __attribute__((ext_vector_type(4)));
  u32x2 ua = __builtin_bit_cast(u32x2, a), ub = __builtin_bit_cast(u32x2, b);
  const auto r0 = __builtin_amdgcn_permlane16_swap(ua[0], ub[0], false, false);
  const auto r1 = __builtin_amdgcn_permlane16_swap(ua[1], ub[1], false, false);
  const u32x4 o = {r0[0], r1[0], r0[1], r1[1]};
  *reinterpret_cast<u32x4*>(row + n + ((fq & 1) ? 12 : 0)) = o;
}
```

phantom_vlb_amd/csrc/ops.hip:

```cpp
#include "common.hpp"

namespace {

constexpr int kMaxBlocks = 256 * 8;

__device__ __forceinline__ void load8(const bf16* p, float (&v)[8]) {
  const bf16x8 t = *reinterpret_cast<const bf16x8*>(p);
#pragma unroll
  for (int i = 0; i < 8; ++i) v[i] = (float)t[i];
}
__device__ __forceinline__ void store8(bf16* p, const float (&v)[8]) {
  bf16x8 t;
#pragma unroll
  for (int i = 0; i < 8; ++i) t[i] = (bf16)v[i];
  *reinterpret_cast<bf16x8*>(p) = t;
}

__global__ __launch_bounds__(256) void rmsnorm_fwd_kernel(const bf16* __restrict__ x, const bf16* __restrict__ w,
                                                          bf16* __restrict__ y, int rows, int dim, float eps) {
  const int row = blockIdx.x * 4 + (threadIdx.x >> 6), lane = threadIdx.x & 63;
  if (row >= rows) return;
  const bf16* xr = x + (int64_t)row * dim;
  float ss = 0.f;
  for (int c = lane * 8; c < dim; c += 512) {
// ... 107 lines not shown
  }
}

template <int NI>
__global__ __launch_bounds__(256) void rmsnorm_bwd_cached_kernel(const bf16* __restrict__ x, const bf16* __restrict__ w,
                                                                 const bf16* __restrict__ dy, const bf16* __restrict__ dx_in,
                                                                 bf16* __restrict__ dx, int rows, int dim, float eps) {
  const int row = blockIdx.x * 4 + (threadIdx.x >> 6), lane = threadIdx.x & 63;
  if (row >= rows) return;
  const bf16* xr = x + (int64_t)row * dim;
  const bf16* gr = dy + (int64_t)row * dim;
  bf16x8 xb[NI], gb[NI], rb[NI];
#pragma unroll
  for (int k = 0; k < NI; ++k) {
    const int c = lane * 8 + k * 512;
    const bool in = c < dim;
    xb[k] = in ? *reinterpret_cast<const bf16x8*>(xr + c) : bf16x8{};
    gb[k] = in ? *reinterpret_cast<const bf16x8*>(gr + c) : bf16x8{};
    rb[k] = (in && dx_in) ? *reinterpret_cast<const bf16x8*>(dx_in + (int64_t)row * dim + c) : bf16x8{};
  }
  float ss = 0.f, dot = 0.f;
#pragma unroll
  for (int k = 0; k < NI; ++k) {
    const int c = lane * 8 + k * 512;
    if (c < dim) {
      float ww[8]; load8(w + c, ww);
#pragma unroll
      for (int i = 0; i < 8; ++i) { const float v = (float)xb[k][i]; ss += v * v; dot += v * (float)gb[k][i] * ww[i]; }
    }
  }
  const float rstd = rsqrtf(wave_sum(ss) / dim + eps);
  const float coef = wave_sum(dot) * rstd * rstd * rstd / dim;
  bf16* dr = dx + (int64_t)row * dim;
#pragma unroll
  for (int k = 0; k < NI; ++k) {
    const int c = lane * 8 + k * 512;
    if (c < dim) {
      float ww[8], o[8]; load8(w + c, ww);
#pragma unroll
      for (int i = 0; i < 8; ++i) o[i] = rstd * ww[i] * (float)gb[k][i] - coef * (float)xb[k][i];
      if (dx_in) {
#pragma unroll
        for (int i = 0; i < 8; ++i) o[i] += (float)rb[k][i];
      }
      store8(dr + c, o);
    }
  }
}

template <int NI>
__global__ __launch_bounds__(256) void layernorm_fwd_cached_kernel(const bf16* __restrict__ x, const bf16* __restrict__ w,
                                                                   const bf16* __restrict__ b, const bf16* __restrict__ res,
                                                                   bf16* __restrict__ y, int rows, int dim, float eps, int act) {
  const int row = blockIdx.x * 4 + (threadIdx.x >> 6), lane = threadIdx.x & 63;
  if (row >= rows) return;
  const bf16* xr = x + (int64_t)row * dim;
  bf16x8 xb[NI], rb[NI];
#pragma unroll
  for (int k = 0; k < NI; ++k) {
    const int c = lane * 8 + k * 512;
    xb[k] = c < dim ? *reinterpret_cast<const bf16x8*>(xr + c) : bf16x8{};
    rb[k] = (c < dim && res) ? *reinterpret_cast<const bf16x8*>(res + (int64_t)row * dim + c) : bf16x8{};
  }
  float s = 0.f;
#pragma unroll
  for (int k = 0; k < NI; ++k)
#pragma unroll
    for (int i = 0; i < 8; ++i) s += (float)xb[k][i];
  const float mean = wave_sum(s) / dim;
  float ss = 0.f;
#pragma unroll
  for (int k = 0; k < NI; ++k) {
    if (lane * 8 + k * 512 < dim) {
#pragma unroll
      for (int i = 0; i < 8; ++i) { const float d = (float)xb[k][i] - mean; ss += d * d; }
    }
  }
  const float rstd = rsqrtf(wave_sum(ss) / dim + eps);
  bf16* yr = y + (int64_t)row * dim;
#pragma unroll
  for (int k = 0; k < NI; ++k) {
    const int c = lane * 8 + k * 512;
    if (c < dim) {
      float v[8], g[8], bb[8]; load8(w + c, g); load8(b + c, bb);
#pragma unroll
      for (int i = 0; i < 8; ++i) v[i] = ((float)xb[k][i] - mean) * rstd * g[i] + bb[i];
      if (res) {
#pragma unroll
        for (int i = 0; i < 8; ++i) v[i] += (float)rb[k][i];
      }
      if (act != VLB_ACT_NONE) {
#pragma unroll
        for (int i = 0; i < 8; ++i) v[i] = act_f(v[i], act);
      }
      store8(yr + c, v);
    }
  }
}

__global__ __launch_bounds__(256) void layernorm_fwd_kernel(const bf16* __restrict__ x, const bf16* __restrict__ w,
                                                            const bf16* __restrict__ b, const bf16* __restrict__ res,
                                                            bf16* __restrict__ y, int rows, int dim, float eps, int act) {
  const int row = blockIdx.x * 4 + (threadIdx.x >> 6), lane = threadIdx.x & 63;
  if (row >= rows) return;
  const bf16* xr = x + (int64_t)row * dim;
  float s = 0.f;
  for (int c = lane * 8; c < dim; c += 512) {
    float v[8]; load8(xr + c, v);
#pragma unroll
    for (int i = 0; i < 8; ++i) s += v[i];
  }
  const float mean = wave_sum(s) / dim;
  float ss = 0.f;
  for (int c = lane * 8; c < dim; c += 512) {
    float v[8]; load8(xr + c, v);
#pragma unroll
    for (int i = 0; i < 8; ++i) { const float d = v[i] - mean; ss += d * d; }
  }
  const float rstd = rsqrtf(wave_sum(ss) / dim + eps);
  bf16* yr = y + (int64_t)row * dim;
  for (int c = lane * 8; c < dim; c += 512) {
    float v[8], g[8], bb[8]; load8(xr + c, v); load8(w + c, g); load8(b + c, bb);
#pragma unroll
    for (int i = 0; i < 8; ++i) v[i] = (v[i] - mean) * rstd * g[i] + bb[i];
    if (res) {
      float r[8]; load8(res + (int64_t)row * dim + c, r);
#pragma unroll
      for (int i = 0; i < 8; ++i) v[i] += r[i];
    }
    if (act != VLB_ACT_NONE) {
#pragma unroll
      for (int i = 0; i < 8; ++i) v[i] = act_f(v[i], act);
    }
    store8(yr + c, v);
  }
}

__global__ void rope_kernel(bf16* __restrict__ x, int ld, const float* __restrict__ cs, const float* __restrict__ sn,
                            int S, int heads, int D, float sign, const int* __restrict__ pos, int64_t total) {
  const int half = D >> 1, cpr = half >> 3;
  for (int64_t idx = blockIdx.x * (int64_t)blockDim.x + threadIdx.x; idx < total; idx += (int64_t)gridDim.x * blockDim.x) {
    const int ch = idx % cpr;
    const int h = (idx / cpr) % heads;
    const int64_t tok = idx / ((int64_t)cpr * heads);
    const int s = pos ? pos[tok] : (int)(tok % S);
    bf16* p = x + tok * ld + h * D + ch * 8;
    float a[8], b[8]; load8(p, a); load8(p + half, b);
    const float* c = cs + (int64_t)s * half + ch * 8;
    const float* n = sn + (int64_t)s * half + ch * 8;
    float oa[8], ob[8];
#pragma unroll
    for (int i = 0; i < 8; ++i) {
      const float co = c[i], si = sign * n[i];
      oa[i] = a[i] * co - b[i] * si;
      ob[i] = b[i] * co + a[i] * si;
    }
    store8(p, oa); store8(p + half, ob);
  }
}

__global__ void swiglu_fwd_kernel(const bf16* __restrict__ gu, bf16* __restrict__ out, int ff, int64_t total) {
  const int cpr = ff >> 3;
  for (int64_t idx = blockIdx.x * (int64_t)blockDim.x + threadIdx.x; idx < total; idx += (int64_t)gridDim.x * blockDim.x) {
    const int64_t r = idx / cpr; const int c = (idx % cpr) * 8;
    float g[8], u[8]; load8(gu + r * 2 * ff + c, g); load8(gu + r * 2 * ff + ff + c, u);
#pragma unroll
    for (int i = 0; i < 8; ++i) g[i] = silu_f(g[i]) * u[i];
    store8(out + r * ff + c, g);
  }
}
__global__ void swiglu_fwd_q8_kernel(const bf16* __restrict__ gu, bf16* __restrict__ out, uint8_t* __restrict__ q, int ldq,
                                     uint8_t* __restrict__ s, int lds_, int ff, int64_t total) {
  const int cpr = ff >> 3;
  for (int64_t idx = blockIdx.x * (int64_t)blockDim.x + threadIdx.x; idx < total; idx += (int64_t)gridDim.x * blockDim.x) {
    const int64_t r = idx / cpr; const int c = (idx % cpr) * 8;
    float g[8], u[8]; load8(gu + r * 2 * ff + c, g); load8(gu + r * 2 * ff + ff + c, u);
#pragma unroll
    for (int i = 0; i < 8; ++i) g[i] = (float)(bf16)(silu_f(g[i]) * u[i]);
    store8(out + r * ff + c, g);
    mx_quantize_lane8(g, q + r * ldq, s + r * lds_, c, threadIdx.x & 63);
  }
}
__global__ void swiglu_bwd_kernel(const bf16* __restrict__ gu, const bf16* __restrict__ dout, bf16* __restrict__ dgu,
                                  int ff, int64_t total) {
  const int cpr = ff >> 3;
  for (int64_t idx = blockIdx.x * (int64_t)blockDim.x + threadIdx.x; idx < total; idx += (int64_t)gridDim.x * blockDim.x) {
    const int64_t r = idx / cpr; const int c = (idx % cpr) * 8;
    float g[8], u[8], d[8], dg[8], du[8];
    load8(gu + r * 2 * ff + c, g); load8(gu + r * 2 * ff + ff + c, u); load8(dout + r * ff + c, d);
#pragma unroll
    for (int i = 0; i < 8; ++i) {
      const float sg = sigmoid_f(g[i]);
      const float si = g[i] * sg;
      du[i] = d[i] * si;
      dg[i] = d[i] * u[i] * (sg * (1.f + g[i] * (1.f - sg)));
    }
    store8(dgu + r * 2 * ff + c, dg); store8(dgu + r * 2 * ff + ff + c, du);
  }
}
__global__ void add_kernel(const bf16* __restrict__ a, const bf16* __restrict__ b, bf16* __restrict__ y, int64_t n8) {
  for (int64_t idx = blockIdx.x * (int64_t)blockDim.x + threadIdx.x; idx < n8; idx += (int64_t)gridDim.x * blockDim.x) {
    float x[8], z[8]; load8(a + idx * 8, x); load8(b + idx * 8, z);
#pragma unroll
    for (int i = 0; i < 8; ++i) x[i] += z[i];
    store8(y + idx * 8, x);
  }
}

__global__ void patchify_kernel(const float* __restrict__ vis, bf16* __restrict__ out, int H, int W, int P, int Kpad,
                                int64_t total) {
  const int G = W / P, GH = H / P, K = 3 * P * P, cpr = Kpad >> 3;
  for (int64_t idx = blockIdx.x * (int64_t)blockDim.x + threadIdx.x; idx < total; idx += (int64_t)gridDim.x * blockDim.x) {
    const int kc = (idx % cpr) * 8;
    const int64_t prow = idx / cpr;
    const int gx = prow % G, gy = (prow / G) % GH;
    const int64_t n = prow / ((int64_t)G * GH);
    float v[8];
#pragma unroll
    for (int i = 0; i < 8; ++i) {
      const int k = kc + i;
      if (k < K) {
        const int c = k / (P * P), py = (k / P) % P, px = k % P;
        v[i] = vis[((n * 3 + c) * H + gy * P + py) * (int64_t)W + gx * P + px];
      } else {
        v[i] = 0.f;
      }
    }
    store8(out + prow * Kpad + kc, v);
  }
}
__global__ void vit_assemble_kernel(const bf16* __restrict__ pe, const bf16* __restrict__ cls, const bf16* __restrict__ pos,
                                    bf16* __restrict__ tok, int G, int D, int64_t total) {
  const int cpr = D >> 3;
  for (int64_t idx = blockIdx.x * (int64_t)blockDim.x + threadIdx.x; idx < total; idx += (int64_t)gridDim.x * blockDim.x) {
    const int c = (idx % cpr) * 8;
    const int t = (idx / cpr) % (G + 1);
    const int64_t n = idx / ((int64_t)cpr * (G + 1));
    float a[8], p[8];
    if (t == 0) load8(cls + c, a); else load8(pe + (n * G + t - 1) * D + c, a);
    load8(pos + (int64_t)t * D + c, p);
#pragma unroll
    for (int i = 0; i < 8; ++i) a[i] += p[i];
    store8(tok + (n * (G + 1) + t) * D + c, a);
  }
}
__global__ void drop_cls_kernel(const bf16* __restrict__ tok, bf16* __restrict__ out, int G, int D, int64_t total) {
  const int cpr = D >> 3;
  for (int64_t idx = blockIdx.x * (int64_t)blockDim.x + threadIdx.x; idx < total; idx += (int64_t)gridDim.x * blockDim.x) {
    const int c = (idx % cpr) * 8;
    const int t = (idx / cpr) % G;
    const int64_t n = idx / ((int64_t)cpr * G);
    *reinterpret_cast<bf16x8*>(out + (n * G + t) * D + c) =
        *reinterpret_cast<const bf16x8*>(tok + (n * (G + 1) + t + 1) * D + c);
  }
}

__global__ __launch_bounds__(256) void dwconv3x3_kernel(const bf16* __restrict__ x, const bf16* __restrict__ w9,
                                                        bf16* __restrict__ y, int H, int W, int C) {
  extern __shared__ __attribute__((aligned(16))) char plane[];
  const int c0 = blockIdx.x * 32;
  const int64_t n = blockIdx.y;
  const int HW = H * W;
  const bf16* xb = x + n * HW * (int64_t)C + c0;
  for (int i = threadIdx.x; i < HW * 4; i += 256) {
    const int p = i >> 2, ch = i & 3;
    *reinterpret_cast<bf16x8*>(plane + i * 16) = *reinterpret_cast<const bf16x8*>(xb + (int64_t)p * C + ch * 8);
  }
  const int ch = threadIdx.x & 3;
  float k[9][8];
#pragma unroll
  for (int t = 0; t < 9; ++t) load8(w9 + (int64_t)t * C + c0 + ch * 8, k[t]);
  __syncthreads();
  bf16* yb = y + n * HW * (int64_t)C + c0 + ch * 8;
  for (int p = threadIdx.x >> 2; p < HW; p += 64) {
    const int hy = p / W, wx = p % W;
    float acc[8] = {0, 0, 0, 0, 0, 0, 0, 0};
#pragma unroll
    for (int dy = -1; dy <= 1; ++dy)
#pragma unroll
      for (int dx = -1; dx <= 1; ++dx) {
        const int yy = hy + dy, xx = wx + dx;
        if (yy < 0 || yy >= H || xx < 0 || xx >= W) continue;
        float v[8]; load8(reinterpret_cast<const bf16*>(plane + ((yy * W + xx) * 4 + ch) * 16), v);
#pragma unroll
        for (int i = 0; i < 8; ++i) acc[i] += v[i] * k[(dy + 1) * 3 + (dx + 1)][i];
      }
    store8(yb + (int64_t)p * C, acc);
  }
}
__global__ __launch_bounds__(256) void se_pool_kernel(const bf16* __restrict__ x, bf16* __restrict__ pooled, int HW, int C) {
  __shared__ float red[4][64][8];
  const int cc = threadIdx.x & 63, rg = threadIdx.x >> 6;
  const int c = (blockIdx.x * 64 + cc) * 8;
  const int64_t n = blockIdx.y;
  float acc[8] = {0, 0, 0, 0, 0, 0, 0, 0};
  if (c < C) {
    for (int r = rg; r < HW; r += 4) {
      float v[8]; load8(x + (n * HW + r) * C + c, v);
#pragma unroll
      for (int i = 0; i < 8; ++i) acc[i] += v[i];
    }
  }
#pragma unroll
  for (int i = 0; i < 8; ++i) red[rg][cc][i] = acc[i];
  __syncthreads();
  if (rg == 0 && c < C) {
    float o[8];
#pragma unroll
// ... 464 lines not shown
```

phantom_vlb_amd/fullft.py:

```python
from __future__ import annotations

import os

import numpy as np
import torch

from . import ops
from ._lib import check, lib
from .flat import SEG_ALIGN
from .geometry import Geometry, VIDEO_TOKEN_ID

BF16 = torch.bfloat16
CONN_W = ("conv1", "dw", "se1", "se1b", "se2", "se2b", "conv3", "ds")
CONN_LN = ("bn1", "bn2", "bn3", "dsbn")


def _stream():
    return torch.cuda.current_stream().cuda_stream


FUSED_QUANT = os.environ.get("VLB_FP8_FUSED_QUANT", "1") == "1"


def _up(n, m):
# ... 227 lines not shown

    def _transposed(self, x, tag, gran=64):
        M, C = x.shape
        Mp = _up(M, gran)
        buf = self._tbuf(tag, C, Mp)
        ops.transpose_pad(x, buf, Mp)
        return buf[:C, :Mp]

    def wgrad(self, dy, x, out, dyT=None, xT=None, fp8=False, dyTq=None):
        if fp8 and out.shape[1] % 256 == 0:
            Mp = _up(dy.shape[0], 128)
            if dyTq is None:
                qa, sa = self._qbuf("dyTq", dy.shape[1], Mp)
                ops.transpose_quantize_mxfp8(dy, qa, sa, Mp)
            else:
                qa, sa = dyTq
            qb, sb = self._qbuf("xTq", x.shape[1], Mp)
            ops.transpose_quantize_mxfp8(x, qb, sb, Mp)
            ops.gemm_mxfp8(qa, sa, qb, sb, out=out)
            return
        dyT = self._transposed(dy, "dyT") if dyT is None else dyT
        xT = self._transposed(x, "xT") if xT is None else xT
        ops.gemm(dyT, xT, out=out)

    def _qbuf(self, tag, rows, cols):
        need = rows * cols
        buf = self._tb.get(tag)
        if buf is None or buf[0].numel() < need:
            buf = self._tb[tag] = (torch.empty(need, dtype=torch.uint8, device=self.dev), torch.empty(need // 32, dtype=torch.uint8, device=self.dev))
        return buf[0][:need].view(rows, cols), buf[1][:need // 32].view(rows, cols // 32)

    def _lin(self, x, li, key, residual=None, xq=None):
        if self.fp8:
            xq, xs = ops.quantize_mxfp8(x) if xq is None else xq
            wq, ws = self._lq[key]
            return ops.gemm_mxfp8(xq, xs, wq, ws, residual=residual)
        return ops.gemm(x, self._lw[key], residual=residual)

    def _norm(self, x, wn):
        if self.fp8 and FUSED_QUANT and x.shape[1] % 32 == 0 and x.shape[1] <= 4096:
            h, q, s = ops.rmsnorm_mxfp8(x, wn, self.g.rms_eps)
            return h, (q, s)
        return ops.rmsnorm(x, wn, self.g.rms_eps), None

    def _dual(self, dy):
        if not self.fp8 or not FUSED_QUANT or dy.shape[1] % 64 != 0:
            return None
        M, C = dy.shape
        Mp = _up(M, 128)
        q, s = self._qbuf("dyq", M, C)
        qt, st = self._qbuf("dyTq", C, Mp)
        ops.quantize_dual_mxfp8(dy, q, s, qt, st, Mp)
        return (q, s), (qt, st)

    def _block_fwd(self, x, blk, N, H, save):
        g, C = self.g, self.g.dim
        y1 = ops.gemm(x, blk["conv1"])
        a1 = ops.layernorm(y1, *blk["bn1"], g.proj_eps, act=ops.ACT_SILU)
        y2 = ops.dwconv3x3(a1, blk["dw"], N, H, H, C)
        a2 = ops.layernorm(y2, *blk["bn2"], g.proj_eps, act=ops.ACT_SILU)
        p = ops.se_pool(a2, N, H * H, C)
        q1 = ops.gemm(p, blk["se1"], bias=blk["se1b"])
        r1 = ops.act_fwd(q1, ops.ACT_SILU)
        s = ops.gemm(r1, blk["se2"], bias=blk["se2b"])
        a3 = ops.se_scale(a2, s, N, H * H, C)
        y3 = ops.gemm(a3, blk["conv3"])
        ysc, sc = None, x
        if "ds" in blk:
            ysc = ops.gemm(x, blk["ds"])
            sc = ops.layernorm(ysc, *blk["dsbn"], g.proj_eps)
        out = ops.layernorm(y3, *blk["bn3"], g.proj_eps, residual=sc, act=ops.ACT_SILU)
        save.append(dict(x=x, y1=y1, a1=a1, y2=y2, a2=a2, p=p, q1=q1, r1=r1, s=s, a3=a3, y3=y3, ysc=ysc, sc=sc, N=N, H=H))
        return out

    def connector_forward(self, feats, B):
        g, w = self.g, self.w
        sv = self.conn_saved = dict(s1=[], s2=[], B=B)
        x = feats
        for blk in w.s1:
            x = self._block_fwd(x, blk, B * g.num_frames, g.grid, sv["s1"])
        cols = ops.im2col3d(x, B, g.num_frames, g.grid, g.grid, g.dim)
        ypre = ops.gemm(cols, w.sampler_w, bias=w.sampler_b)
        x = ops.act_fwd(ypre, ops.ACT_SILU)
        sv.update(cols=cols, ypre=ypre)
        for blk in w.s2:
            x = self._block_fwd(x, blk, B * g.ds_frames, g.ds_grid, sv["s2"])
        t0 = ops.gemm(x, w.ro0[0], bias=w.ro0[1])
        t1 = ops.act_fwd(t0, ops.ACT_GELU)
        sv.update(ro_in=x, t0=t0, t1=t1)
        return ops.gemm(t1, w.ro2[0], bias=w.ro2[1])

    def _block_bwd(self, d_out, blk, st, bi, sv, need_dx):
        g, C, G = self.g, self.g.dim, self.flat.g_
        pre = f"mm_projector.{st}.b{bi + 1}"
        N, H = sv["N"], sv["H"]
        dy3, dsc = ops.layernorm_bwd(sv["y3"], *blk["bn3"], d_out, g.proj_eps, G(f"{pre}.bn3.weight"), G(f"{pre}.bn3.bias"),
                                     residual=sv["sc"], act=ops.ACT_SILU, want_dres=True)
        self.wgrad(dy3, sv["a3"], G(f"{pre}.conv3"))
        d_a3 = ops.gemm(dy3, self.conn_t[f"{st}.{bi}.conv3"])
        ds = ops.se_bwd_gate(sv["a2"], d_a3, sv["s"], N, H * H, C)
        self.wgrad(ds, sv["r1"], G(f"{pre}.se2"))
        ops.colsum(ds, G(f"{pre}.se2b"))
        d_r1 = ops.gemm(ds, self.conn_t[f"{st}.{bi}.se2"])
        d_q1 = ops.act_bwd(sv["q1"], d_r1, ops.ACT_SILU)
        self.wgrad(d_q1, sv["p"], G(f"{pre}.se1"))
        ops.colsum(d_q1, G(f"{pre}.se1b"))
        d_p = ops.gemm(d_q1, self.conn_t[f"{st}.{bi}.se1"])
        d_a2 = ops.se_bwd_x(d_a3, sv["s"], d_p, N, H * H, C)
        dy2, _ = ops.layernorm_bwd(sv["y2"], *blk["bn2"], d_a2, g.proj_eps, G(f"{pre}.bn2.weight"), G(f"{pre}.bn2.bias"), act=ops.ACT_SILU)
        ops.dwconv3x3_bwd_w(sv["a1"], dy2, N, H, H, C, G(f"{pre}.dw"))
        d_a1 = ops.dwconv3x3(dy2, self.dw_flipped[(st, bi)], N, H, H, C)
        dy1, _ = ops.layernorm_bwd(sv["y1"], *blk["bn1"], d_a1, g.proj_eps, G(f"{pre}.bn1.weight"), G(f"{pre}.bn1.bias"), act=ops.ACT_SILU)
        xT = self._transposed(sv["x"], "xT")
        self.wgrad(dy1, sv["x"], G(f"{pre}.conv1"), xT=xT)
        dysc = None
        if "ds" in blk:
            dysc, _ = ops.layernorm_bwd(sv["ysc"], *blk["dsbn"], dsc, g.proj_eps, G(f"{pre}.dsbn.weight"), G(f"{pre}.dsbn.bias"))
            self.wgrad(dysc, sv["x"], G(f"{pre}.ds"), xT=xT)
        if not need_dx:
            return None
        if dysc is not None:
            dx = ops.gemm(dy1, self.conn_t[f"{st}.{bi}.conv1"])
            return ops.gemm(dysc, self.conn_t[f"{st}.{bi}.ds"], residual=dx)
        return ops.gemm(dy1, self.conn_t[f"{st}.{bi}.conv1"], residual=dsc)

    def connector_backward(self, d_vid):
        g, w, sv, G = self.g, self.w, self.conn_saved, self.flat.g_
        B = sv["B"]
        self.wgrad(d_vid, sv["t1"], G("mm_projector.ro2.weight"))
        ops.colsum(d_vid, G("mm_projector.ro2.bias"))
        d_t1 = ops.gemm(d_vid, self.conn_t["ro2"])
        d_t0 = ops.act_bwd(sv["t0"], d_t1, ops.ACT_GELU)
        self.wgrad(d_t0, sv["ro_in"], G("mm_projector.ro0.weight"))
        ops.colsum(d_t0, G("mm_projector.ro0.bias"))
        dx = ops.gemm(d_t0, self.conn_t["ro0"])
        for bi in range(len(w.s2) - 1, -1, -1):
            dx = self._block_bwd(dx, w.s2[bi], "s2", bi, sv["s2"][bi], True)
        d_ypre = ops.act_bwd(sv["ypre"], dx, ops.ACT_SILU)
        self.wgrad(d_ypre, sv["cols"], G("mm_projector.sampler.weight"))
        ops.colsum(d_ypre, G("mm_projector.sampler.bias"))
        dcols = ops.gemm(d_ypre, self.conn_t["sampler"])
        dx = ops.col2im3d(dcols, B, g.num_frames, g.grid, g.grid, g.dim)
        for bi in range(len(w.s1) - 1, -1, -1):
            dx = self._block_bwd(dx, w.s1[bi], "s1", bi, sv["s1"][bi], bi > 0)
        self.conn_saved = None

    def forward(self, vision_f32, ids, layout=None, ids_host=None):
        g, bb, w = self.g, self.bb, self.w
        B = vision_f32.shape[0]
        vid = self.connector_forward(bb.video_tokens(vision_f32, tower_only=True), B)
        x, key_mask = bb.splice(ids, vid, layout)
        self._ids_host = ids_host if ids_host is not None else ids.cpu()
        S = g.max_len
        pos = None if layout is None else layout.pos
        qd, kd = g.heads * g.head_dim, g.kv_heads * g.head_dim
        self.saved = []
        for li in range(g.layers):
            lw = self._enter(li, backward=False)
            h1, h1q = self._norm(x, lw["in_norm"])
            qkv = self._lin(h1, li, "wqkv", xq=h1q)
            ops.rope_(qkv, w.rope_cos, w.rope_sin, B, S, g.heads + g.kv_heads, g.head_dim, pos=pos)
            a, lse = ops.attention_fwd(qkv[:, :qd], qkv[:, qd:qd + kd], qkv[:, qd + kd:], B, S, g.heads, g.kv_heads, g.head_dim,
                                       True, g.head_dim ** -0.5, key_mask=key_mask, need_lse=True, layout=layout)
            x2 = self._lin(a, li, "wo", residual=x)
            h2, h2q = self._norm(x2, lw["post_norm"])
            gu = self._lin(h2, li, "wgu", xq=h2q)
            if self.fp8 and FUSED_QUANT and gu.shape[1] % 64 == 0:
                hh, hq, hs = ops.swiglu_mxfp8(gu)
                x3 = self._lin(hh, li, "wdown", residual=x2, xq=(hq, hs))
            else:
                hh = ops.swiglu(gu)
                x3 = self._lin(hh, li, "wdown", residual=x2)
            self.saved.append(dict(x=x, h1=h1, qkv=qkv, a=a, lse=lse, x2=x2, h2=h2, gu=gu, hh=hh))
            x = x3
        self.x_last, self.key_mask, self.B, self.layout = x, key_mask, B, layout
        return ops.rmsnorm(x, w.final_norm, g.rms_eps), key_mask

    def backward(self, dhidden):
        g, w, G = self.g, self.w, self.flat.g_
        B, S = self.B, g.max_len
        qd, kd = g.heads * g.head_dim, g.kv_heads * g.head_dim
        layout = self.layout
        pos = None if layout is None else layout.pos
        dx = ops.rmsnorm_bwd_full(self.x_last, w.final_norm, dhidden, g.rms_eps, G("norm"))
        delta = torch.empty(B, g.heads, S, dtype=torch.float32, device=self.dev)
        for li in range(g.layers - 1, -1, -1):
            lw, sv = self._enter(li, backward=True), self.saved[li]
            pre = f"layers.{li}"
            dq_ = self._dual(dx) or (None, None)
            self.wgrad(dx, sv["hh"], G(f"{pre}.wdown"), fp8=self.fp8, dyTq=dq_[1])
            d_hh = self._lin(dx, li, "wdown_t", xq=dq_[0])
            d_gu = ops.swiglu_bwd(sv["gu"], d_hh)
            dq_ = self._dual(d_gu) or (None, None)
            self.wgrad(d_gu, sv["h2"], G(f"{pre}.wgu"), fp8=self.fp8, dyTq=dq_[1])
            d_h2 = self._lin(d_gu, li, "wgu_t", xq=dq_[0])
            dx2 = ops.rmsnorm_bwd_full(sv["x2"], lw["post_norm"], d_h2, g.rms_eps, G(f"{pre}.post_norm"), dx_in=dx)
            dq_ = self._dual(dx2) or (None, None)
            self.wgrad(dx2, sv["a"], G(f"{pre}.wo"), fp8=self.fp8, dyTq=dq_[1])
            d_a = self._lin(dx2, li, "wo_t", xq=dq_[0])
            dqkv = ops.attention_bwd(sv["qkv"], qd, kd, sv["a"], d_a, sv["lse"], self.key_mask, B, S, g.heads, g.kv_heads,
                                     g.head_dim, True, g.head_dim ** -0.5, layout=layout, delta=delta)
            ops.rope_(dqkv, w.rope_cos, w.rope_sin, B, S, g.heads + g.kv_heads, g.head_dim, sign=-1, pos=pos)
            dq_ = self._dual(dqkv) or (None, None)
            self.wgrad(dqkv, sv["h1"], G(f"{pre}.wqkv"), fp8=self.fp8, dyTq=dq_[1])
            d_h1 = self._lin(dqkv, li, "wqkv_t", xq=dq_[0])
            dx = ops.rmsnorm_bwd_full(sv["x"], lw["in_norm"], d_h1, g.rms_eps, G(f"{pre}.in_norm"), dx_in=dx2)
            self.saved[li] = None
            if self.grad_hook is not None:
                self.grad_hook(li)
        self._splice_backward(dx)
        self.saved = []

    def _splice_backward(self, d_embeds):
        g = self.g
        ids = self._ids_host.numpy() if torch.is_tensor(self._ids_host) else np.asarray(self._ids_host)
        B, L = ids.shape
        Nv, S = g.vis_tokens, g.max_len
        layout = self.layout
        lens = layout.lens if (layout is not None and layout.packed) else [S] * B
        cu = np.concatenate([[0], np.cumsum(lens)]) if (layout is not None and layout.packed) else np.arange(B + 1) * S
        tok_rows, tok_ids, vid_rows = [], [], []
        for b in range(B):
            vpos = int(np.nonzero(ids[b] == VIDEO_TOKEN_ID)[0][0])
            j = np.arange(L)
            p = np.where(j < vpos, j, j + Nv - 1)
            keep = (j != vpos) & (p < lens[b])
            tok_rows.append(cu[b] + p[keep])
            tok_ids.append(ids[b][keep])
            vid_rows.append(cu[b] + vpos + np.arange(Nv))
        tok_rows, tok_ids = np.concatenate(tok_rows), np.concatenate(tok_ids)
        order = np.lexsort((tok_rows, tok_ids))
        tok_rows, tok_ids = tok_rows[order], tok_ids[order]
        uniq, first = np.unique(tok_ids, return_index=True)
        beg = np.concatenate([first, [len(tok_ids)]])
        dev = self.dev
        i32 = lambda a: torch.from_numpy(np.ascontiguousarray(a, dtype=np.int32)).to(dev)
        dE = self.flat.g_("embed_tokens")
        dE.zero_()
        ops.embed_grad(d_embeds, i32(uniq), i32(beg), i32(tok_rows), dE, g.dim)
        vr = np.concatenate(vid_rows)
        d_vid = torch.empty(B * Nv, g.dim, dtype=BF16, device=dev)
        n = B * Nv
        ops.embed_grad(d_embeds, i32(np.arange(n)), i32(np.arange(n + 1)), i32(vr), d_vid, g.dim)
        self.connector_backward(d_vid)

    def state_dict(self, which: str = "master") -> dict:
        g, f = self.g, self.flat
        buf = getattr(f, which)
        if self.shards is not None and (buf is None or buf.numel() < f.numel):
            buf = self.shards.gather_full(which)
        M = lambda n: f.view(buf, n).detach().float().cpu()
        qd, kd = g.heads * g.head_dim, g.kv_heads * g.head_dim
        sd = {"model.embed_tokens.weight": M("embed_tokens"), "model.norm.weight": M("norm")}
        for li in range(g.layers):
            p, q = f"model.layers.{li}", f"layers.{li}"
            wqkv, wgu = M(f"{q}.wqkv"), M(f"{q}.wgu")
            sd[f"{p}.self_attn.q_proj.weight"] = wqkv[:qd].clone()
            sd[f"{p}.self_attn.k_proj.weight"] = wqkv[qd:qd + kd].clone()
            sd[f"{p}.self_attn.v_proj.weight"] = wqkv[qd + kd:].clone()
            sd[f"{p}.self_attn.o_proj.weight"] = M(f"{q}.wo")
            sd[f"{p}.mlp.gate_proj.weight"] = wgu[:g.ff].clone()
            sd[f"{p}.mlp.up_proj.weight"] = wgu[g.ff:].clone()
            sd[f"{p}.mlp.down_proj.weight"] = M(f"{q}.wdown")
            sd[f"{p}.input_layernorm.weight"] = M(f"{q}.in_norm")
            sd[f"{p}.post_attention_layernorm.weight"] = M(f"{q}.post_norm")
        P = "model.mm_projector"
        for st, blocks in (("s1", self.w.s1), ("s2", self.w.s2)):
            for bi, blk in enumerate(blocks):
                q, n = f"{P}.{st}.b{bi + 1}", f"mm_projector.{st}.b{bi + 1}"
                C = blk["conv1"].shape[0]
                sd[f"{q}.conv1.conv.weight"] = M(f"{n}.conv1")[:, :, None, None].clone()
                sd[f"{q}.conv2.conv.weight"] = M(f"{n}.dw").t().reshape(C, 1, 3, 3).clone()
                sd[f"{q}.conv3.conv.weight"] = M(f"{n}.conv3")[:, :, None, None].clone()
                for k, u in (("se1", "se.fc1"), ("se2", "se.fc2")):
                    sd[f"{q}.{u}.weight"] = M(f"{n}.{k}")[:, :, None, None].clone()
                    sd[f"{q}.{u}.bias"] = M(f"{n}.{k}b")
                for k, u in (("bn1", "conv1.bn"), ("bn2", "conv2.bn"), ("bn3", "conv3.bn")):
                    sd[f"{q}.{u}.weight"], sd[f"{q}.{u}.bias"] = M(f"{n}.{k}.weight"), M(f"{n}.{k}.bias")
                if "ds" in blk:
                    sd[f"{q}.downsample.conv.weight"] = M(f"{n}.ds")[:, :, None, None].clone()
                    sd[f"{q}.downsample.bn.weight"], sd[f"{q}.downsample.bn.bias"] = M(f"{n}.dsbn.weight"), M(f"{n}.dsbn.bias")
        sw = M("mm_projector.sampler.weight")
        C = sw.shape[0]
        sd[f"{P}.sampler.0.weight"] = sw.view(C, 2, 2, 2, C).permute(0, 4, 1, 2, 3).contiguous()
        sd[f"{P}.sampler.0.bias"] = M("mm_projector.sampler.bias")
        for k, u in (("ro0", "readout.0"), ("ro2", "readout.2")):
            sd[f"{P}.{u}.weight"], sd[f"{P}.{u}.bias"] = M(f"mm_projector.{k}.weight"), M(f"mm_projector.{k}.bias")
        return sd
```

phantom_vlb_amd/lora.py:

```python
from __future__ import annotations

import ctypes
import math

import torch

from . import ops
from ._lib import check, lib
from .geometry import Geometry

BF16 = torch.bfloat16
PAD = 64
FUSE_SWIGLU_BWD = True
MERGE_DB_U = True


def _stream():
    return torch.cuda.current_stream().cuda_stream


def _seeds(vals):
    return (ctypes.c_uint32 * len(vals))(*[v & 0xFFFFFFFF for v in vals])


# ... 116 lines not shown
        return list(self.master.items())

    def compute_copies(self):
        out = {}
        for i, lay in enumerate(self.layers):
            for gname, targets in GROUPS:
                for j, t in enumerate(targets):
                    pre = f"model.layers.{i}.{t}"
                    out[f"{pre}.lora_A.weight"] = lay[gname]["A"][self.rp * j:self.rp * j + self.rp]
                    out[f"{pre}.lora_B.weight"] = self.bt[f"{pre}.lora_B.weight"]
        return out

    def _scatter_jobs(self):
        import struct
        cc = self.compute_copies()
        key = tuple(t.data_ptr() for t in cc.values())
        if getattr(self, "_jobs_key", None) == key:
            return self._jobs
        rec = []
        for i, lay in enumerate(self.layers):
            for gname, targets in GROUPS:
                blk = lay[gname]
                row = 0
                for j, t in enumerate(targets):
                    pre = f"model.layers.{i}.{t}"
                    a, bt = cc[f"{pre}.lora_A.weight"], cc[f"{pre}.lora_B.weight"]
                    for b in range(self.c):
                        col = self.rp * j + 16 * b
                        il = int(self.gu_il and gname == "gu")
                        brow = 16 * j if il else row
                        for src, dst, n, mode in ((a[16 * b:16 * b + 16], blk["At"][:, col:], a.shape[1], 0),
                                                  (bt[16 * b:16 * b + 16], blk["Bpad"][brow:, col:], bt.shape[1], il)):
                            assert src.is_contiguous() and src.shape[0] == 16 and dst.stride(0) == blk["Rpad"]
                            for n0 in range(0, n, 256):
                                rec.append(struct.pack("<QQiiii", src.data_ptr(), dst.data_ptr(), n, n0, blk["Rpad"], mode))
                    row += self.out_dims[t]
        buf = torch.frombuffer(bytearray(b"".join(rec)), dtype=torch.uint8).to(self.dev)
        self._jobs, self._jobs_key, self._n_jobs = buf, key, len(rec)
        return buf

    def refresh(self, from_master=False):
        if from_master:
            cc = self.compute_copies()
            for n, t in cc.items():
                t.copy_(self.master[n])
        jobs = self._scatter_jobs()
        check(lib.vlb_transpose16_scatter(jobs.data_ptr(), self._n_jobs, _stream()), "vlb_transpose16_scatter")
        self.version += 1

    def merge(self):
        layers = self.w.layers
        if any(lw.get(k) is None for lw in layers for k in ("wqkv", "wo", "wdown", "wgu_il" if self.gu_il else "wgu")):
            raise ValueError("LoraState.merge(): the frozen decoder weights are sharded (Backbone.enable_sharding): a rank holds "
                             "1/world of every layer, and merging gathered shards is not supported")
        if self._merged is not None and self._merged_version == self.version:
            return self._merged
        if self._merged is None:
            keys = ("wqkv", "wo", "wdown", "wgu_il" if self.gu_il else "wgu")
            self._merged = [{"in_norm": lw["in_norm"], "post_norm": lw["post_norm"], **{k: torch.empty_like(lw[k]) for k in keys}}
                            for lw in layers]
        g, rp = self.g, self.rp
        for li, (lw, mw, lay) in enumerate(zip(layers, self._merged, self.layers)):
            def one(gname, j, w, wm, row_map=ops.MERGE_PLAIN):
                pre = f"model.layers.{li}.{lay[gname]['targets'][j]}"
                ops.lora_merge(w, wm, self.bt[f"{pre}.lora_B.weight"], lay[gname]["A"][rp * j:rp * j + rp], self.scale, row_map)
            row = 0
            for j, t in enumerate(lay["qkv"]["targets"]):
                n = self.out_dims[t]
                one("qkv", j, lw["wqkv"][row:row + n], mw["wqkv"][row:row + n])
                row += n
            one("o", 0, lw["wo"], mw["wo"])
            if self.gu_il:
                one("gu", 0, lw["wgu_il"], mw["wgu_il"], ops.MERGE_GATE)
                one("gu", 1, lw["wgu_il"], mw["wgu_il"], ops.MERGE_UP)
            else:
                one("gu", 0, lw["wgu"][:g.ff], mw["wgu"][:g.ff])
                one("gu", 1, lw["wgu"][g.ff:], mw["wgu"][g.ff:])
            one("down", 0, lw["wdown"], mw["wdown"])
        self._merged_version = self.version
        return self._merged

    def state_dict(self):
        r = self.r
        return {n: (t[:r].t().contiguous() if "lora_B" in n else t[:r].clone()) for n, t in self.master.items()}

    def load_state_dict(self, sd: dict):
        r = self.r
        for n, t in self.master.items():
            src = sd[n].to(self.dev, torch.float32)
            t[:r].copy_(src.t() if "lora_B" in n else src)
        self.refresh(from_master=True)

    def _seed(self, layer, target_idx):
        x = (self.base_seed * 0x9E3779B1 + self.step * 0x85EBCA6B + layer * 0xC2B2AE35 + target_idx * 0x27D4EB2F
             + self.rank * 0x7F4A7C15) & 0xFFFFFFFF
        return x or 1

    def _workspace(self, M):
        if self._ws is None or self._ws["cap"] < M:
            g, d = self.g, self.dev
            kmax = max(g.ff, g.dim, g.heads * g.head_dim)
            kgrp = max(2 * g.ff, (g.heads + 2 * g.kv_heads) * g.head_dim)
            self._ws = dict(cap=M, wg=torch.empty(lib.vlb_wgrad_splits(M) * 48 * kmax, dtype=torch.float32, device=d),
                            uws=torch.empty(lib.vlb_wgrad_u_ws_floats(M, kgrp), dtype=torch.float32, device=d),
                            u_full=torch.zeros(M, self._rpad_max(), dtype=BF16, device=d))
        self._ws["u"] = self._ws["u_full"][:M]
        return self._ws

    def _rpad_max(self):
        return max(blk["Rpad"] for blk in self.layers[0].values())

    def _group_seeds(self, seeds, n_targets):
        return None if seeds is None else [seeds[j] for j in range(n_targets) for _ in range(self.c)]

    def _t_buffer(self, li, gi, M):
        if getattr(self, "_t_cap", 0) < M:
            self._t_cap = M
            self._t_bufs = torch.zeros(len(self.layers), len(GROUPS), M, self._rpad_max(), dtype=BF16, device=self.dev)
        return self._t_bufs[li, gi, :M, :self.layers[li][GROUPS[gi][0]]["Rpad"]]

    def _lora_t(self, x, blk, seeds, slot=None, p=None):
        t = self._t_buffer(*slot, x.shape[0]) if slot is not None else torch.zeros(x.shape[0], blk["Rpad"], dtype=BF16, device=self.dev)
        p = self.p if p is None else p
        gs = self._group_seeds(seeds, len(blk["targets"])) if p > 0 else None
        for r0 in range(0, blk["R"], 48):
            n = min(48, blk["R"] - r0)
            lora_down(x, blk["A"][r0:r0 + n], n, self.scale, p, None if gs is None else gs[r0 // 16:(r0 + n) // 16], t[:, r0:])
        return t

    def _adapted(self, x, W, blk, seeds, residual=None, slot=None, p=None):
        t = self._lora_t(x, blk, seeds, slot, p)
        return ops.gemm(x, W, residual=residual, a2=t, w2=blk["Bpad"]), t

    def _adapted_mlp_in(self, x, lw, blk, seeds, slot, p=None, save=True):
        if self.gu_il:
            t = self._lora_t(x, blk, seeds, slot, p)
            if save:
                hh, gu = ops.gemm_swiglu_save(x, lw["wgu_il"], a2=t, w2_il=blk["Bpad"])
                return hh, gu, t
            return ops.gemm(x, lw["wgu_il"], act=ops.ACT_SWIGLU_PAIR, a2=t, w2=blk["Bpad"]), None, t
        gu, t = self._adapted(x, lw["wgu"], blk, seeds, slot=slot, p=p)
        return ops.swiglu(gu), gu, t

    def forward(self, backbone, vision_f32, ids, layout=None, train=True):
        g = self.g
        B = vision_f32.shape[0]
        vid = backbone.video_tokens(vision_f32)
        x, key_mask = backbone.splice(ids, vid, layout)
        return self.decoder_forward(backbone, x, key_mask, B, layout, train=train)

    def decoder_forward(self, backbone, x, key_mask, B, layout=None, train=True):
        g, w = self.g, self.w
        S = g.max_len
        pos = None if layout is None else layout.pos
        qd, kd = g.heads * g.head_dim, g.kv_heads * g.head_dim
        if not train:
            return self._decoder_eval(backbone, x, key_mask, B, layout)
        self.saved = []
        self.step += 1
        for li, lay in enumerate(self.layers):
            lw = backbone.layer_weights(li)
            sd = [self._seed(li, k) for k in range(7)]
            h1 = ops.rmsnorm(x, lw["in_norm"], g.rms_eps)
            qkv, t_qkv = self._adapted(h1, lw["wqkv"], lay["qkv"], sd[0:3], slot=(li, 0))
            ops.rope_(qkv, w.rope_cos, w.rope_sin, B, S, g.heads + g.kv_heads, g.head_dim, pos=pos)
            a, lse = ops.attention_fwd(qkv[:, :qd], qkv[:, qd:qd + kd], qkv[:, qd + kd:], B, S, g.heads, g.kv_heads,
                                       g.head_dim, True, g.head_dim ** -0.5, key_mask=key_mask, need_lse=True,
                                       layout=layout)
            x2, t_o = self._adapted(a, lw["wo"], lay["o"], sd[3:4], residual=x, slot=(li, 1))
            h2 = ops.rmsnorm(x2, lw["post_norm"], g.rms_eps)
            hh, gu, t_gu = self._adapted_mlp_in(h2, lw, lay["gu"], sd[4:6], (li, 2))
            x3, t_d = self._adapted(hh, lw["wdown"], lay["down"], sd[6:7], residual=x2, slot=(li, 3))
            self.saved.append(dict(x=x, h1=h1, qkv=qkv, a=a, lse=lse, x2=x2, h2=h2, gu=gu, hh=hh, t_qkv=t_qkv, t_o=t_o,
                                   t_gu=t_gu, t_d=t_d, seeds=sd))
            x = x3
        self.x_last, self.key_mask, self.B, self.layout = x, key_mask, B, layout
        return ops.rmsnorm(x, w.final_norm, g.rms_eps), key_mask

    def _decoder_eval(self, backbone, x, key_mask, B, layout):
        g, w = self.g, self.w
        S = g.max_len
        pos = None if layout is None else layout.pos
        qd, kd = g.heads * g.head_dim, g.kv_heads * g.head_dim
        for li, lay in enumerate(self.layers):
            lw = backbone.layer_weights(li)
            h = ops.rmsnorm(x, lw["in_norm"], g.rms_eps)
            qkv, _ = self._adapted(h, lw["wqkv"], lay["qkv"], None, slot=(li, 0), p=0.0)
            ops.rope_(qkv, w.rope_cos, w.rope_sin, B, S, g.heads + g.kv_heads, g.head_dim, pos=pos)
            a = ops.attention_fwd(qkv[:, :qd], qkv[:, qd:qd + kd], qkv[:, qd + kd:], B, S, g.heads, g.kv_heads, g.head_dim,
                                  True, g.head_dim ** -0.5, key_mask=key_mask, layout=layout)
            x, _ = self._adapted(a, lw["wo"], lay["o"], None, residual=x, slot=(li, 1), p=0.0)
            h = ops.rmsnorm(x, lw["post_norm"], g.rms_eps)
            hh, _, _ = self._adapted_mlp_in(h, lw, lay["gu"], None, (li, 2), p=0.0, save=False)
            x, _ = self._adapted(hh, lw["wdown"], lay["down"], None, residual=x, slot=(li, 3), p=0.0)
        return ops.rmsnorm(x, w.final_norm, g.rms_eps), key_mask

    def _group_backward(self, li, gname, dy, x_in, t, seeds, W_t, need_dx, swiglu_gu=None):
        lay = self.layers[li][gname]
        ws = self._workspace(dy.shape[0])
        u = ws["u"]
        col = 0
        u = u[:, :lay["Rpad"]]
        rp = self.rp
        names = [f"model.layers.{li}.{tname}" for tname in lay["targets"]]
        cols = [self.out_dims[tname] for tname in lay["targets"]]
        multi = MERGE_DB_U and self.c == 1 and len(cols) > 1 and all(n % 256 == 0 for n in cols) and dy.shape[1] == sum(cols)
        if multi:
            wgrad_skinny_u_multi(t, dy, cols, [self.grads[f"{pre}.lora_B.weight"] for pre in names],
                                 [self.bt[f"{pre}.lora_B.weight"] for pre in names], ws["wg"], self.scale, u, ws["uws"])
        for j, tname in enumerate(() if multi else lay["targets"]):
            n = self.out_dims[tname]
            pre = f"model.layers.{li}.{tname}"
            dyj = dy[:, col:col + n]
            for b in range(self.c):
                k = rp * j + 16 * b
                wgrad_skinny_u(t[:, k:k + 16], dyj, self.grads[f"{pre}.lora_B.weight"][16 * b:16 * b + 16], ws["wg"],
                               self.bt[f"{pre}.lora_B.weight"][16 * b:16 * b + 16], self.scale, u[:, k:k + 16], ws["uws"])
            col += n
        gs = self._group_seeds(seeds, len(lay["targets"])) if self.p > 0 else None
        for r0 in range(0, lay["R"], 48):
            n = min(48, lay["R"] - r0)
            wgrad_skinny(u[:, r0:], x_in, self.grad_A[li][gname][r0:r0 + n], ws["wg"], n, p=self.p,
                         seeds=None if gs is None else gs[r0 // 16:(r0 + n) // 16])
        if not need_dx:
            return None
        if self.p == 0.0:
            dx = ops.gemm(dy, W_t, a2=u, w2=lay["At"])
        elif lay["R"] == 16 and ops.gemm_masked_pair_ok(dy.shape[0], W_t.shape[0], dy.shape[1]):
            if swiglu_gu is not None and FUSE_SWIGLU_BWD:
                return ops.gemm_masked_pair_swiglu_bwd(dy, W_t, swiglu_gu, u, lay["At"], self.p, seeds[0])
            dx = ops.gemm_masked_pair(dy, W_t, u, lay["At"], self.p, seeds[0])
        else:
            dx = ops.gemm(dy, W_t)
            for r0 in range(0, lay["R"], 48):
                n = min(48, lay["R"] - r0)
                lora_dx_masked(u[:, r0:], lay["At"][:, r0:], dx, n, self.p, gs[r0 // 16:(r0 + n) // 16])
        return dx if swiglu_gu is None else ops.swiglu_bwd(swiglu_gu, dx)

    def backward(self, backbone, dhidden):
        g, w = self.g, self.w
        B, S = self.B, g.max_len
        qd, kd = g.heads * g.head_dim, g.kv_heads * g.head_dim
        layout = self.layout
        pos = None if layout is None else layout.pos
        M = self.x_last.shape[0]
        dx = ops.rmsnorm_bwd(self.x_last, w.final_norm, dhidden, g.rms_eps)
        delta = torch.empty(B, g.heads, S, dtype=torch.float32, device=self.dev)
        for li in range(g.layers - 1, -1, -1):
            lw, sv = backbone.layer_weights(li, transposed=True, direction=-1), self.saved[li]
            sd = sv["seeds"]
            d_gu = self._group_backward(li, "down", dx, sv["hh"], sv["t_d"], sd[6:7], lw["wdown_t"], True, swiglu_gu=sv["gu"])
            d_h2 = self._group_backward(li, "gu", d_gu, sv["h2"], sv["t_gu"], sd[4:6], lw["wgu_t"], True)
            dx2 = ops.rmsnorm_bwd(sv["x2"], lw["post_norm"], d_h2, g.rms_eps, dx_in=dx)
            d_a = self._group_backward(li, "o", dx2, sv["a"], sv["t_o"], sd[3:4], lw["wo_t"], True)
            qkv = sv["qkv"]
            dqkv = ops.attention_bwd(qkv, qd, kd, sv["a"], d_a, sv["lse"], self.key_mask, B, S, g.heads, g.kv_heads,
                                     g.head_dim, True, g.head_dim ** -0.5, layout=layout, delta=delta)
            ops.rope_(dqkv, w.rope_cos, w.rope_sin, B, S, g.heads + g.kv_heads, g.head_dim, sign=-1, pos=pos)
            need_dx = li > 0
            d_h1 = self._group_backward(li, "qkv", dqkv, sv["h1"], sv["t_qkv"], sd[0:3], lw["wqkv_t"], need_dx)
            if need_dx:
                dx = ops.rmsnorm_bwd(sv["x"], lw["in_norm"], d_h1, g.rms_eps, dx_in=dx2)
            if self.grad_hook is not None:
                self.grad_hook(li)
        self.saved = []
```

phantom_vlb_amd/ops.py:

```python
from __future__ import annotations

import torch

from ._lib import check, lib

ACT_NONE, ACT_QUICK_GELU, ACT_GELU, ACT_SILU, ACT_SWIGLU_PAIR = 0, 1, 2, 3, 4
BF16 = torch.bfloat16


def _stream():
    return torch.cuda.current_stream().cuda_stream


def _p(t):
    return None if t is None else t.data_ptr()


def _dev(t):
    if not t.is_cuda:
        raise RuntimeError("phantom_vlb_amd ops need GPU tensors (no CPU fallback)")
    return t


class _GemmProbe:
# ... 82 lines not shown
    M, K = a.shape
    N = w.shape[0]
    assert w.shape[1] == K and a.stride(1) == 1 and w.stride(1) == 1
    if out is None:
        out = torch.empty(M, N // 2 if act == ACT_SWIGLU_PAIR else N, dtype=BF16, device=a.device)
    K2 = 0
    if a2 is not None:
        K2 = a2.shape[1]
        assert w2.shape == (N, K2) and a2.shape[0] == M
    ws = _gemm_workspace(a.device) if K + K2 >= 4096 and M * N > 256 * 192 * 256 else None
    with _Timed("plain", M, N, K, K2):
        check(lib.vlb_gemm_bf16_ws(a.data_ptr(), a.stride(0), w.data_ptr(), w.stride(0), out.data_ptr(), out.stride(0),
                                   M, N, K, _p(bias), _p(residual), residual.stride(0) if residual is not None else 0, act,
                                   _p(a2), a2.stride(0) if a2 is not None else 0, _p(w2),
                                   w2.stride(0) if w2 is not None else 0, K2, _p(ws), ws.numel() if ws is not None else 0,
                                   _stream()), "vlb_gemm_bf16")
    return out


def gemm_swiglu_save(a, w_il, a2=None, w2_il=None):
    _dev(a)
    M, K = a.shape
    N = w_il.shape[0]
    assert w_il.shape[1] == K and a.stride(1) == 1 and w_il.stride(1) == 1 and N % 32 == 0
    h = torch.empty(M, N // 2, dtype=BF16, device=a.device)
    gu = torch.empty(M, N, dtype=BF16, device=a.device)
    K2 = 0
    if a2 is not None:
        K2 = a2.shape[1]
        assert w2_il.shape == (N, K2) and a2.shape[0] == M
    ws = _gemm_workspace(a.device) if K + K2 >= 4096 and M * N > 256 * 192 * 256 else None
    with _Timed("gate_up+swiglu", M, N, K, K2):
        check(lib.vlb_gemm_swiglu_save(a.data_ptr(), a.stride(0), w_il.data_ptr(), w_il.stride(0), h.data_ptr(), h.stride(0),
                                       gu.data_ptr(), gu.stride(0), M, N, K, _p(a2), a2.stride(0) if a2 is not None else 0, _p(w2_il),
                                       w2_il.stride(0) if w2_il is not None else 0, K2, _p(ws), ws.numel() if ws is not None else 0,
                                       _stream()), "vlb_gemm_swiglu_save")
    return h, gu


def gemm_masked_pair_ok(M, N, K):
    return N % 256 == 0 and K % 64 == 0 and K >= 128 and M * (N // 2) < 2 ** 32


def gemm_masked_pair(a, w, a2, w2, p, seed, out=None):
    _dev(a)
    M, K = a.shape
    N = w.shape[0]
    assert w.shape[1] == K and a2.shape[0] == M and w2.shape[0] == N and a2.shape[1] >= 64 and w2.shape[1] >= 64
    if out is None:
        out = torch.empty(M, N, dtype=BF16, device=a.device)
    ws = _gemm_workspace(a.device) if K + 64 >= 4096 and M * N > 256 * 192 * 256 else None
    with _Timed("masked", M, N, K, 64):
        check(lib.vlb_gemm_bf16_masked_pair_ws(a.data_ptr(), a.stride(0), w.data_ptr(), w.stride(0), out.data_ptr(), out.stride(0),
                                               M, N, K, a2.data_ptr(), a2.stride(0), w2.data_ptr(), w2.stride(0), float(p),
                                               int(seed) & 0xFFFFFFFF, _p(ws), ws.numel() if ws is not None else 0, _stream()),
              "vlb_gemm_bf16_masked_pair")
    return out


def gemm_masked_pair_swiglu_bwd(dy, w_t, gu, a2, w2, p, seed, out=None):
    _dev(dy)
    M, K = dy.shape
    ff = w_t.shape[0]
    assert w_t.shape[1] == K and gu.shape == (M, 2 * ff) and a2.shape[0] == M and w2.shape[0] == ff
    if out is None:
        out = torch.empty(M, 2 * ff, dtype=BF16, device=dy.device)
    ws = _gemm_workspace(dy.device) if K + 64 >= 4096 and M * ff > 256 * 192 * 256 else None
    with _Timed("masked", M, ff, K, 64):
        check(lib.vlb_gemm_masked_pair_swiglu_bwd(dy.data_ptr(), dy.stride(0), w_t.data_ptr(), w_t.stride(0), gu.data_ptr(), gu.stride(0),
                                                  out.data_ptr(), out.stride(0), M, ff, K, a2.data_ptr(), a2.stride(0), w2.data_ptr(),
                                                  w2.stride(0), float(p), int(seed) & 0xFFFFFFFF, _p(ws),
                                                  ws.numel() if ws is not None else 0, _stream()), "vlb_gemm_masked_pair_swiglu_bwd")
    return out


def interleave_gate_up(w_gate, w_up):
    ff, k = w_gate.shape
    assert ff % 16 == 0
    return torch.stack([w_gate.view(ff // 16, 16, k), w_up.view(ff // 16, 16, k)], 1).reshape(2 * ff, k).contiguous()


MERGE_PLAIN, MERGE_GATE, MERGE_UP = 0, 1, 2
merge_launches = 0


def lora_merge(w, wm, bt, a, scale, row_map=MERGE_PLAIN):
    global merge_launches
    _dev(w)
    R, K = a.shape
    N = bt.shape[1]
    rows = N if row_map == MERGE_PLAIN else 2 * N
    assert bt.shape[0] == R and w.shape == (rows, K) and wm.shape == (rows, K)
    assert w.stride(1) == 1 and wm.stride(1) == 1 and a.is_contiguous() and bt.is_contiguous()
    assert w.dtype == wm.dtype == bt.dtype == a.dtype == BF16
    check(lib.vlb_lora_merge(w.data_ptr(), w.stride(0), wm.data_ptr(), wm.stride(0), bt.data_ptr(), a.data_ptr(), N, K, R,
                             float(scale), int(row_map), _stream()), "vlb_lora_merge")
    merge_launches += 1
    return wm


def transpose(x):
    R, C = x.shape
    out = torch.empty(C, R, dtype=BF16, device=x.device)
    check(lib.vlb_transpose_bf16(_dev(x).data_ptr(), out.data_ptr(), R, C, _stream()), "vlb_transpose_bf16")
    return out


class RowLayout:

    def __init__(self, B, S, lens=None, device=None):
        self.B, self.S = int(B), int(S)
        if lens is None:
            self.cu = self.pos = self.lens = None
            self.rows, self.smax = self.B * self.S, self.S
            return
        lens = [int(x) for x in lens]
        if len(lens) != self.B or min(lens) < 1 or max(lens) > self.S:
            raise ValueError(f"RowLayout: lens {lens} do not fit B={B}, S={S}")
        cu = [0]
        for n in lens:
            cu.append(cu[-1] + n)
        self.lens, self.rows, self.smax = lens, cu[-1], max(lens)
        self.cu = torch.tensor(cu, dtype=torch.int32).to(device, non_blocking=True)
        self.pos = torch.empty(self.rows, dtype=torch.int32, device=device)

    @property
    def packed(self):
        return self.cu is not None

    def unpack(self, x, fill=0.0):
        if not self.packed:
            return x.view(self.B, self.S, -1)
        out = torch.full((self.B, self.S, x.shape[1]), fill, dtype=x.dtype, device=x.device)
        o = 0
        for b, n in enumerate(self.lens):
            out[b, :n] = x[o:o + n]
            o += n
        return out


def attention_fwd(q, k, v, B, S, Hq, Hkv, D, causal, scale, key_mask=None, need_lse=False, out=None, layout=None):
    _dev(q)
    cu, rows = None, B * S
    if layout is not None and layout.packed:
        B, S, cu, rows = layout.B, layout.smax, layout.cu, layout.rows
    assert q.shape[0] == rows, f"attention_fwd: {q.shape[0]} rows, layout has {rows}"
    if out is None:
        out = torch.empty(rows, Hq * D, dtype=BF16, device=q.device)
    lse = torch.empty(B, Hq, S, dtype=torch.float32, device=q.device) if need_lse else None
    check(lib.vlb_attention_fwd(q.data_ptr(), q.stride(0), k.data_ptr(), k.stride(0), v.data_ptr(), v.stride(0),
                                out.data_ptr(), out.stride(0), _p(lse), _p(key_mask), B, S, Hq, Hkv, D,
                                1 if causal else 0, float(scale), _p(cu), _stream()), "vlb_attention_fwd")
    return (out, lse) if need_lse else out


_ATTN_WS = [None]


def _attn_workspace(n_floats, device):
    ws = _ATTN_WS[0]
    if ws is None or ws.numel() < n_floats or ws.device != device:
        ws = _ATTN_WS[0] = torch.empty(n_floats, dtype=torch.float32, device=device)
    return ws


def attention_bwd(qkv, qd, kd, out, dout, lse, key_mask, B, S, Hq, Hkv, D, causal, scale, layout=None, delta=None,
                  dq_acc=None):
    cu, rows = None, B * S
    if layout is not None and layout.packed:
        B, S, cu, rows = layout.B, layout.smax, layout.cu, layout.rows
    assert qkv.shape[0] == rows and dout.shape[0] == rows
    if delta is None:
        delta = torch.empty(B, Hq, S, dtype=torch.float32, device=qkv.device)
    if dq_acc is None and Hq != Hkv:
        dq_acc = _attn_workspace(rows * qd, qkv.device)
    assert delta.numel() >= B * Hq * S and (dq_acc is None or dq_acc.numel() >= rows * qd)
    dqkv = torch.empty_like(qkv)
    check(lib.vlb_attention_bwd(qkv.data_ptr(), qkv.stride(0), qkv[:, qd:].data_ptr(), qkv.stride(0),
                                qkv[:, qd + kd:].data_ptr(), qkv.stride(0), out.data_ptr(), out.stride(0),
                                dout.data_ptr(), dout.stride(0), lse.data_ptr(), _p(key_mask),
                                dqkv.data_ptr(), dqkv.stride(0), dqkv[:, qd:].data_ptr(), dqkv.stride(0),
                                dqkv[:, qd + kd:].data_ptr(), dqkv.stride(0), delta.data_ptr(), _p(dq_acc),
                                B, S, Hq, Hkv, D, 1 if causal else 0, float(scale), _p(cu), rows, _stream()),
          "vlb_attention_bwd")
    return dqkv


def rmsnorm(x, w, eps, out=None):
    rows, dim = x.shape
    if out is None:
        out = torch.empty_like(x)
    check(lib.vlb_rmsnorm_fwd(_dev(x).data_ptr(), w.data_ptr(), out.data_ptr(), rows, dim, eps, _stream()), "vlb_rmsnorm_fwd")
    return out


def rmsnorm_bwd(x, w, dy, eps, dx_in=None, out=None):
    rows, dim = x.shape
    if out is None:
        out = torch.empty_like(x)
    check(lib.vlb_rmsnorm_bwd(_dev(x).data_ptr(), w.data_ptr(), dy.data_ptr(), _p(dx_in), out.data_ptr(), rows, dim, eps,
                              _stream()), "vlb_rmsnorm_bwd")
    return out


def layernorm(x, w, b, eps, residual=None, act=ACT_NONE, out=None):
    rows, dim = x.shape
    if out is None:
        out = torch.empty_like(x)
    check(lib.vlb_layernorm_fwd(_dev(x).data_ptr(), w.data_ptr(), b.data_ptr(), _p(residual), out.data_ptr(), rows, dim,
                                eps, act, _stream()), "vlb_layernorm_fwd")
    return out


def rope_(x, cos, sin, B, S, heads, D, sign=1, pos=None):
    rows = B * S if pos is None else pos.shape[0]
    assert x.shape[0] == rows and cos.shape[0] >= S
    check(lib.vlb_rope_inplace(_dev(x).data_ptr(), x.stride(0), cos.data_ptr(), sin.data_ptr(), rows, S, heads, D, sign,
                               _p(pos), _stream()), "vlb_rope_inplace")
    return x


def swiglu(gu, out=None):
    rows, ff2 = gu.shape
    if out is None:
        out = torch.empty(rows, ff2 // 2, dtype=BF16, device=gu.device)
    check(lib.vlb_swiglu_fwd(_dev(gu).data_ptr(), out.data_ptr(), rows, ff2 // 2, _stream()), "vlb_swiglu_fwd")
    return out


def swiglu_bwd(gu, dout, out=None):
    rows, ff2 = gu.shape
    if out is None:
        out = torch.empty_like(gu)
    check(lib.vlb_swiglu_bwd(_dev(gu).data_ptr(), dout.data_ptr(), out.data_ptr(), rows, ff2 // 2, _stream()), "vlb_swiglu_bwd")
    return out


def add(a, b, out=None):
    if out is None:
        out = torch.empty_like(a)
    check(lib.vlb_add_bf16(_dev(a).data_ptr(), b.data_ptr(), out.data_ptr(), a.numel(), _stream()), "vlb_add_bf16")
    return out


def patchify(vision_f32, P, Kpad):
    N, C, H, W = vision_f32.shape
    assert C == 3 and vision_f32.dtype == torch.float32 and vision_f32.is_contiguous()
    out = torch.empty(N * (H // P) * (W // P), Kpad, dtype=BF16, device=vision_f32.device)
    check(lib.vlb_patchify(_dev(vision_f32).data_ptr(), out.data_ptr(), N, H, W, P, Kpad, _stream()), "vlb_patchify")
    return out


def vit_assemble(patch_emb, cls, pos, N, G, D):
    out = torch.empty(N * (G + 1), D, dtype=BF16, device=patch_emb.device)
    check(lib.vlb_vit_assemble(_dev(patch_emb).data_ptr(), cls.data_ptr(), pos.data_ptr(), out.data_ptr(), N, G, D,
                               _stream()), "vlb_vit_assemble")
    return out


def drop_cls(tokens, N, G, D):
    out = torch.empty(N * G, D, dtype=BF16, device=tokens.device)
    check(lib.vlb_drop_cls(_dev(tokens).data_ptr(), out.data_ptr(), N, G, D, _stream()), "vlb_drop_cls")
    return out


def dwconv3x3(x, w9, N, H, W, C):
    out = torch.empty_like(x)
    check(lib.vlb_dwconv3x3(_dev(x).data_ptr(), w9.data_ptr(), out.data_ptr(), N, H, W, C, _stream()), "vlb_dwconv3x3")
    return out


def se_pool(x, N, HW, C):
    out = torch.empty(N, C, dtype=BF16, device=x.device)
    check(lib.vlb_se_pool(_dev(x).data_ptr(), out.data_ptr(), N, HW, C, _stream()), "vlb_se_pool")
    return out


def se_scale(x, gate, N, HW, C, out=None):
    if out is None:
        out = torch.empty_like(x)
    check(lib.vlb_se_scale(_dev(x).data_ptr(), gate.data_ptr(), out.data_ptr(), N, HW, C, _stream()), "vlb_se_scale")
    return out


def im2col3d(x, B, T, H, W, C):
    T2, H2, W2 = T // 2 + 1, H // 2 + 1, W // 2 + 1
    out = torch.empty(B * T2 * H2 * W2, 8 * C, dtype=BF16, device=x.device)
    check(lib.vlb_im2col3d_k2s2p1(_dev(x).data_ptr(), out.data_ptr(), B, T, H, W, C, _stream()), "vlb_im2col3d_k2s2p1")
    return out


def splice_embed(ids, embed_w, video_tokens, Nv, video_id, err_flag, layout=None):
    B, L = ids.shape
    D = embed_w.shape[1]
    S = L - 1 + Nv
    assert ids.dtype == torch.int64 and ids.is_contiguous()
    packed = layout is not None and layout.packed
    if packed:
        assert layout.B == B and layout.S == S
    rows = layout.rows if packed else B * S
    out = torch.empty(rows, D, dtype=BF16, device=ids.device)
    mask = torch.empty((rows,) if packed else (B, S), dtype=torch.uint8, device=ids.device)
    check(lib.vlb_splice_embed(_dev(ids).data_ptr(), embed_w.data_ptr(), video_tokens.data_ptr(), out.data_ptr(),
                               mask.data_ptr(), err_flag.data_ptr(), B, L, Nv, D, video_id, embed_w.shape[0],
                               _p(layout.cu) if packed else None, _p(layout.pos) if packed else None,
                               _stream()), "vlb_splice_embed")
    return out, mask


def weight_mask(padvals, vis_w, lang_w, tokens_per_frame, S, round_bf16=True):
    B, F = vis_w.shape
    assert padvals.dtype == torch.int64 and vis_w.dtype == torch.float64 and lang_w.dtype == torch.float64
    out = torch.empty(B, S, dtype=torch.float32, device=padvals.device)
    check(lib.vlb_weight_mask(_dev(padvals).contiguous().data_ptr(), vis_w.contiguous().data_ptr(),
                              lang_w.contiguous().data_ptr(), out.data_ptr(), B, F, lang_w.shape[1], tokens_per_frame, S,
                              1 if round_bf16 else 0, _stream()), "vlb_weight_mask")
    return out


def dropout_keep_scale(B, E, p, seed, device):
    out = torch.empty(B, E, dtype=torch.float32, device=device)
    check(lib.vlb_dropout_keep_scale(_dev(out).data_ptr(), out.numel(), float(p), int(seed) & 0xFFFFFFFF, _stream()),
          "vlb_dropout_keep_scale")
    return out


def profile_marker():
    check(lib.vlb_profile_marker(_stream()), "vlb_profile_marker")


def cast_bf16(x_f32):
    out = torch.empty(x_f32.shape, dtype=BF16, device=x_f32.device)
    check(lib.vlb_cast_f32_to_bf16(_dev(x_f32).data_ptr(), out.data_ptr(), x_f32.numel(), _stream()), "vlb_cast_f32_to_bf16")
    return out


_ws_cache = {}


def _ws(n_floats, device, tag="norm"):
# ... 158 lines not shown
```

Before: 15.22 clips/s.

## Fuse RoPE into decoder attention forward and backward kernels

Applies the rotary embedding to Q inside the flash-attention forward kernel, and to dQ in the epilogue of the backward dQ kernel. The inverse rotation of dK is folded into the GQA dK/dV reduce kernel, and the delta (out·dout) computation moves into the dQ kernel. This removes the separate full-tensor RoPE passes over QKV and dQKV and the standalone delta kernel, saving memory traffic and launches. In exchange it adds register pressure and extra cos/sin table loads inside the attention kernels. K is still rotated with a separate in-place pass, and with save_q off Q is only rotated in registers.

```diff
diff --git a/include/vlb.h b/include/vlb.h
--- a/include/vlb.h
+++ b/include/vlb.h
@@ -64,6 +64,16 @@
                       int lddq, void* dk, int lddk, void* dv, int lddv, float* delta, float* dq_acc, int B, int S,
                       int Hq, int Hkv, int D, int causal, float scale, const int* cu_rows, int total_rows,
                       void* stream);
+
+int vlb_attention_fwd_rope(void* q, int ldq, void* k, int ldk, const void* v, int ldv, void* out, int ldo, float* lse,
+                           const uint8_t* key_mask, int B, int S, int Hq, int Hkv, int D, int causal, float scale,
+                           const int* cu_rows, int total_rows, const float* cos_t, const float* sin_t, const int* pos,
+                           int save_q, void* stream);
+int vlb_attention_bwd_rope(const void* q, int ldq, const void* k, int ldk, const void* v, int ldv, const void* out,
+                           int ldo, const void* dout, int lddo, const float* lse, const uint8_t* key_mask, void* dq,
+                           int lddq, void* dk, int lddk, void* dv, int lddv, float* delta, float* dq_acc, int B, int S,
+                           int Hq, int Hkv, int D, int causal, float scale, const int* cu_rows, int total_rows,
+                           const float* cos_t, const float* sin_t, const int* pos, void* stream);
 
 int vlb_rmsnorm_fwd(const void* x, const void* w, void* y, int rows, int dim, float eps, void* stream);
 int vlb_rmsnorm_bwd(const void* x, const void* w, const void* dy, const void* dx_in, void* dx, int rows, int dim,
diff --git a/phantom_vlb_amd/_lib.py b/phantom_vlb_amd/_lib.py
--- a/phantom_vlb_amd/_lib.py
+++ b/phantom_vlb_amd/_lib.py
@@ -24,6 +24,8 @@
     "vlb_transpose_bf16": [P, P, I, I, P],
     "vlb_attention_fwd": [P, I, P, I, P, I, P, I, P, P, I, I, I, I, I, I, F, P, P],
     "vlb_attention_bwd": [P, I, P, I, P, I, P, I, P, I, P, P, P, I, P, I, P, I, P, P, I, I, I, I, I, I, F, P, I, P],
+    "vlb_attention_fwd_rope": [P, I, P, I, P, I, P, I, P, P, I, I, I, I, I, I, F, P, I, P, P, P, I, P],
+    "vlb_attention_bwd_rope": [P, I, P, I, P, I, P, I, P, I, P, P, P, I, P, I, P, I, P, P, I, I, I, I, I, I, F, P, I, P, P, P, P],
     "vlb_rmsnorm_fwd": [P, P, P, I, I, F, P],
     "vlb_rmsnorm_bwd": [P, P, P, P, P, I, I, F, P],
     "vlb_layernorm_fwd": [P, P, P, P, P, I, I, F, I, P],
diff --git a/phantom_vlb_amd/backbone.py b/phantom_vlb_amd/backbone.py
--- a/phantom_vlb_amd/backbone.py
+++ b/phantom_vlb_amd/backbone.py
@@ -227,10 +227,8 @@
         qd, kd = g.heads * g.head_dim, g.kv_heads * g.head_dim
         h = ops.rmsnorm(x, lw["in_norm"], g.rms_eps)
         qkv = ops.gemm(h, lw["wqkv"])
-        ops.rope_(qkv, self.w.rope_cos, self.w.rope_sin, B, S, g.heads + g.kv_heads, g.head_dim,
-                  pos=None if layout is None else layout.pos)
-        a = ops.attention_fwd(qkv[:, :qd], qkv[:, qd:qd + kd], qkv[:, qd + kd:], B, S, g.heads, g.kv_heads, g.head_dim,
-                              True, g.head_dim ** -0.5, key_mask=key_mask, layout=layout)
+        a = ops.rope_attention_fwd(qkv, qd, kd, self.w.rope_cos, self.w.rope_sin, B, S, g.heads, g.kv_heads, g.head_dim,
+                                   g.head_dim ** -0.5, key_mask=key_mask, layout=layout, save_q=False)
         x = ops.gemm(a, lw["wo"], residual=x)
         h = ops.rmsnorm(x, lw["post_norm"], g.rms_eps)
         if lw.get("wgu_il") is not None:
diff --git a/phantom_vlb_amd/csrc/attention.hip b/phantom_vlb_amd/csrc/attention.hip
--- a/phantom_vlb_amd/csrc/attention.hip
+++ b/phantom_vlb_amd/csrc/attention.hip
@@ -37,7 +37,18 @@
   int ldq, ldk, ldv, ldo;
   int B, S, Hq, Hkv;
   float scale;
+  const float* cs; const float* sn; const int* pos; int save_q; float rsign;
 };
+
+__device__ __forceinline__ void gqa_sum8(const bf16* src, int gsz, float (&acc)[8]) {
+#pragma unroll
+  for (int e = 0; e < 8; ++e) acc[e] = 0.f;
+  for (int j = 0; j < gsz; ++j) {
+    const bf16x8 v = *reinterpret_cast<const bf16x8*>(src + (int64_t)j * 256);
+#pragma unroll
+    for (int e = 0; e < 8; ++e) acc[e] += (float)v[e];
+  }
+}
 
 template <int D> __device__ __forceinline__ int slot_k(int r, int c) {
   if constexpr (D == 128) return c ^ (r & 15); else return c ^ ((r >> 1) & 7);
@@ -50,8 +61,9 @@
   return (Hq & 7) == 0 ? (j & 7) * (Hq >> 3) + (j >> 3) : j;
 }
 
-template <int D, bool CAUSAL>
+template <int D, bool CAUSAL, bool ROPE_Q = false>
 __global__ __launch_bounds__(256, 2) void attn_fwd_kernel(AttnArgs p) {
+  static_assert(!ROPE_Q || D == 128, "the in-kernel Q rotation is written for D = 128");
   constexpr int CPR = D / 8;
   constexpr int ROWB = D * 2;
   constexpr int TILE = KV * ROWB;
@@ -109,8 +121,34 @@
   };
 
   stage(0, 0);
+  if constexpr (ROPE_Q) {
+    const int qr = min(q0 + ql, Sb - 1);
+    const int s = p.pos ? p.pos[row0 + qr] : qr;
+    const float* cp = p.cs + (int64_t)s * (D / 2) + 8 * h;
+    const float* np = p.sn + (int64_t)s * (D / 2) + 8 * h;
+#pragma unroll
+    for (int ks = 0; ks < KS / 2; ++ks) {
+      const f32x4 c0 = *reinterpret_cast<const f32x4*>(cp + 16 * ks), c1 = *reinterpret_cast<const f32x4*>(cp + 16 * ks + 4);
+      const f32x4 n0 = *reinterpret_cast<const f32x4*>(np + 16 * ks), n1 = *reinterpret_cast<const f32x4*>(np + 16 * ks + 4);
+#pragma unroll
+      for (int j = 0; j < 8; ++j) {
+        const float co = j < 4 ? c0[j & 3] : c1[j & 3], si = p.rsign * (j < 4 ? n0[j & 3] : n1[j & 3]);
+        float oa, ob;
+        rope_rotate((float)qf[ks][j], (float)qf[ks + KS / 2][j], co, si, oa, ob);
+        qf[ks][j] = (bf16)oa;
+        qf[ks + KS / 2][j] = (bf16)ob;
+      }
+    }
+  }
   asm volatile("s_waitcnt vmcnt(0)" ::: "memory");
   __syncthreads();
+  if constexpr (ROPE_Q) {
+    if (p.save_q && q0 + ql < Sb) {
+      bf16* qw = const_cast<bf16*>(p.q) + (row0 + q0 + ql) * p.ldq + hq * D + 8 * h;
+#pragma unroll
+      for (int ks = 0; ks < KS; ++ks) *reinterpret_cast<bf16x8*>(qw + 16 * ks) = qf[ks];
+    }
+  }
 
   const int g1 = (lane >> 4) & 1, li = lane & 15, tq = li >> 2, tp = li & 3;
   int k_rd[KS], v_rd[DT];
@@ -239,31 +277,57 @@
   }
 }
 
-template <int D, bool CAUSAL>
+template <int D, bool CAUSAL, bool ROPE_Q = false>
 int launch_fwd(const AttnArgs& a, hipStream_t s) {
   constexpr int LDS = 2 * 2 * KV * D * 2;
-  static const hipError_t attr = hipFuncSetAttribute(reinterpret_cast<const void*>(&attn_fwd_kernel<D, CAUSAL>),
+  static const hipError_t attr = hipFuncSetAttribute(reinterpret_cast<const void*>(&attn_fwd_kernel<D, CAUSAL, ROPE_Q>),
                                                      hipFuncAttributeMaxDynamicSharedMemorySize, LDS);
   if (attr != hipSuccess) { vlb_set_error("attention: LDS reservation failed: %s", hipGetErrorString(attr)); return VLB_ERR_LAUNCH; }
   dim3 grid(((a.S + QB - 1) / QB) * a.Hq * a.B);
-  hipLaunchKernelGGL((attn_fwd_kernel<D, CAUSAL>), grid, dim3(256), LDS, s, a);
+  hipLaunchKernelGGL((attn_fwd_kernel<D, CAUSAL, ROPE_Q>), grid, dim3(256), LDS, s, a);
   VLB_LAUNCH_CHECK();
   return VLB_OK;
 }
 }
 
-extern "C" int vlb_attention_fwd(const void* q, int ldq, const void* k, int ldk, const void* v, int ldv, void* out,
-                                 int ldo, float* lse, const uint8_t* key_mask, int B, int S, int Hq, int Hkv, int D,
-                                 int causal, float scale, const int* cu_rows, void* stream) {
+namespace {
+int attention_fwd_check(const void* q, int ldq, const void* k, int ldk, const void* v, int ldv, void* out, int ldo, int B,
+                        int S, int Hq, int Hkv, int D) {
   VLB_REQUIRE(q && k && v && out, "attention_fwd: null operand");
   VLB_REQUIRE(D == 64 || D == 128, "attention_fwd: head dim %d not in {64,128}", D);
   VLB_REQUIRE(B > 0 && S > 0 && Hq > 0 && Hkv > 0 && Hq % Hkv == 0, "attention_fwd: bad shape B=%d S=%d Hq=%d Hkv=%d", B, S, Hq, Hkv);
   VLB_REQUIRE(ldq % 8 == 0 && ldk % 8 == 0 && ldv % 8 == 0 && ldo % 4 == 0, "attention_fwd: strides must keep 16-byte alignment");
   VLB_REQUIRE((((uintptr_t)q | (uintptr_t)k | (uintptr_t)v) % 16 == 0) && ((uintptr_t)out % 8 == 0), "attention_fwd: misaligned pointer");
-  AttnArgs a{(const bf16*)q, (const bf16*)k, (const bf16*)v, (bf16*)out, lse, key_mask, cu_rows, ldq, ldk, ldv, ldo, B, S, Hq, Hkv, scale};
+  return VLB_OK;
+}
+}
+
+extern "C" int vlb_attention_fwd(const void* q, int ldq, const void* k, int ldk, const void* v, int ldv, void* out,
+                                 int ldo, float* lse, const uint8_t* key_mask, int B, int S, int Hq, int Hkv, int D,
+                                 int causal, float scale, const int* cu_rows, void* stream) {
+  if (const int rc = attention_fwd_check(q, ldq, k, ldk, v, ldv, out, ldo, B, S, Hq, Hkv, D)) return rc;
+  AttnArgs a{(const bf16*)q, (const bf16*)k, (const bf16*)v, (bf16*)out, lse, key_mask, cu_rows, ldq, ldk, ldv, ldo, B, S, Hq, Hkv, scale,
+             nullptr, nullptr, nullptr, 0, 1.f};
   hipStream_t s = as_stream(stream);
   if (D == 128) return causal ? launch_fwd<128, true>(a, s) : launch_fwd<128, false>(a, s);
   return causal ? launch_fwd<64, true>(a, s) : launch_fwd<64, false>(a, s);
+}
+
+extern "C" int vlb_attention_fwd_rope(void* q, int ldq, void* k, int ldk, const void* v, int ldv, void* out, int ldo,
+                                      float* lse, const uint8_t* key_mask, int B, int S, int Hq, int Hkv, int D, int causal,
+                                      float scale, const int* cu_rows, int total_rows, const float* cos_t,
+                                      const float* sin_t, const int* pos, int save_q, void* stream) {
+  if (const int rc = attention_fwd_check(q, ldq, k, ldk, v, ldv, out, ldo, B, S, Hq, Hkv, D)) return rc;
+  VLB_REQUIRE(D == 128, "attention_fwd_rope: head dim %d unsupported (only 128: the decoder)", D);
+  VLB_REQUIRE(cos_t && sin_t && (((uintptr_t)cos_t | (uintptr_t)sin_t) % 16 == 0), "attention_fwd_rope: cos / sin tables missing or misaligned");
+  VLB_REQUIRE(pos || !cu_rows, "attention_fwd_rope: packed rows need their positions");
+  const int64_t rows = cu_rows ? (int64_t)total_rows : (int64_t)B * S;
+  VLB_REQUIRE(rows > 0 && rows <= (int64_t)B * S, "attention_fwd_rope: total_rows=%d out of range", total_rows);
+  if (const int rc = vlb_rope_inplace(k, ldk, cos_t, sin_t, (int)rows, S, Hkv, D, 1, pos, stream)) return rc;
+  AttnArgs a{(const bf16*)q, (const bf16*)k, (const bf16*)v, (bf16*)out, lse, key_mask, cu_rows, ldq, ldk, ldv, ldo, B, S, Hq, Hkv, scale,
+             cos_t, sin_t, pos, save_q, 1.f};
+  hipStream_t s = as_stream(stream);
+  return causal ? launch_fwd<128, true, true>(a, s) : launch_fwd<128, false, true>(a, s);
 }
 
 namespace {
@@ -298,8 +362,7 @@
     const int h = gid % Hq; const int64_t tok = gid / Hq;
     const bf16x8 a = *reinterpret_cast<const bf16x8*>(o + tok * ldo + h * 128 + c * 8);
     const bf16x8 b = *reinterpret_cast<const bf16x8*>(d_o + tok * lddo + h * 128 + c * 8);
-#pragma unroll
-    for (int i = 0; i < 8; ++i) s += (float)a[i] * (float)b[i];
+    s = dot8_seq(a, b);
   }
 #pragma unroll
   for (int off = 8; off > 0; off >>= 1) s += __shfl_xor(s, off, 64);
@@ -490,18 +553,55 @@
   const int hkv = (int)((i >> 5) % Hkv);
   const int64_t row = (i >> 5) / Hkv;
   const int gsz = Hq / Hkv;
-  float acc[8] = {0.f, 0.f, 0.f, 0.f, 0.f, 0.f, 0.f, 0.f};
-  const bf16* src = part + (row * Hq + (int64_t)hkv * gsz) * 256 + which * 128 + c * 8;
-  for (int j = 0; j < gsz; ++j) {
-    const bf16x8 v = *reinterpret_cast<const bf16x8*>(src + (int64_t)j * 256);
-#pragma unroll
-    for (int e = 0; e < 8; ++e) acc[e] += (float)v[e];
-  }
+  float acc[8];
+  gqa_sum8(part + (row * Hq + (int64_t)hkv * gsz) * 256 + which * 128 + c * 8, gsz, acc);
   bf16x8 o;
 #pragma unroll
   for (int e = 0; e < 8; ++e) o[e] = (bf16)acc[e];
   bf16* dst = which ? dv + row * lddv : dk + row * lddk;
   *reinterpret_cast<bf16x8*>(dst + hkv * 128 + c * 8) = o;
+}
+
+__global__ __launch_bounds__(256) void attn_dkdv_reduce_rope_kernel(const bf16* __restrict__ part, bf16* __restrict__ dk, int lddk,
+                                                                    bf16* __restrict__ dv, int lddv, int Hq, int Hkv, int64_t total,
+                                                                    const float* __restrict__ cs, const float* __restrict__ sn,
+                                                                    const int* __restrict__ pos, int S, float sign) {
+  const int64_t i = blockIdx.x * (int64_t)blockDim.x + threadIdx.x;
+  if (i >= total) return;
+  const int item = (int)(i % 24);
+  const int hkv = (int)((i / 24) % Hkv);
+  const int64_t row = (i / 24) / Hkv;
+  const int gsz = Hq / Hkv;
+  const bf16* src = part + (row * Hq + (int64_t)hkv * gsz) * 256;
+  if (item >= 8) {
+    const int c = item - 8;
+    float acc[8];
+    gqa_sum8(src + 128 + c * 8, gsz, acc);
+    bf16x8 o;
+#pragma unroll
+    for (int e = 0; e < 8; ++e) o[e] = (bf16)acc[e];
+    *reinterpret_cast<bf16x8*>(dv + row * lddv + hkv * 128 + c * 8) = o;
+    return;
+  }
+  const int c = item;
+  float a[8], b[8];
+  gqa_sum8(src + c * 8, gsz, a);
+  gqa_sum8(src + 64 + c * 8, gsz, b);
+  const int s = pos ? pos[row] : (int)(row % S);
+  const float* cp = cs + (int64_t)s * 64 + c * 8;
+  const float* np = sn + (int64_t)s * 64 + c * 8;
+  bf16x8 oa8, ob8;
+#pragma unroll
+  for (int e = 0; e < 8; ++e) {
+    const float co = cp[e], si = sign * np[e];
+    float oa, ob;
+    rope_rotate((float)(bf16)a[e], (float)(bf16)b[e], co, si, oa, ob);
+    oa8[e] = (bf16)oa;
+    ob8[e] = (bf16)ob;
+  }
+  bf16* dst = dk + row * lddk + hkv * 128 + c * 8;
+  *reinterpret_cast<bf16x8*>(dst) = oa8;
+  *reinterpret_cast<bf16x8*>(dst + 64) = ob8;
 }
 
 struct AttnDqArgs {
@@ -511,9 +611,11 @@
   int ldq, ldk, ldv, lddo, lddq;
   int B, S, Hq, Hkv;
   float scale;
+  const bf16* out; int ldo; float* delta_out;
+  const float* cs; const float* sn; const int* pos; float rsign;
 };
 
-template <bool CAUSAL>
+template <bool CAUSAL, bool FUSED = false>
 __global__ __launch_bounds__(256, 2) void attn_bwd_dq_kernel(AttnDqArgs p) {
   constexpr int D = 128, ROWB = 256, TILE = KV * ROWB, KS = 8, DT = 4;
   extern __shared__ __attribute__((aligned(16))) char smem[];
@@ -544,7 +646,21 @@
     }
   }
   const float lse_q = p.lse[((int64_t)b * p.Hq + hq) * p.S + qr];
-  const float delta_q = p.delta[((int64_t)b * p.Hq + hq) * p.S + qr];
+  float delta_q;
+  if constexpr (FUSED) {
+    const bf16* op = p.out + (row0 + qr) * p.ldo + hq * D + 8 * h;
+    float ps[KS];
+#pragma unroll
+    for (int ks = 0; ks < KS; ++ks) ps[ks] = dot8_seq(*reinterpret_cast<const bf16x8*>(op + 16 * ks), dof[ks]);
+#pragma unroll
+    for (int ks = 0; ks < 4; ++ks) ps[ks] += ps[ks + 4];
+    ps[0] += ps[2]; ps[1] += ps[3];
+    ps[0] += ps[1];
+    delta_q = ps[0] + __shfl_xor(ps[0], 32, 64);
+    if (h == 0 && qrow < Sb) p.delta_out[((int64_t)b * p.Hq + hq) * p.S + qrow] = delta_q;
+  } else {
+    delta_q = p.delta[((int64_t)b * p.Hq + hq) * p.S + qr];
+  }
   const float c2 = p.scale * 1.44269504088896341f;
   const float lse2 = (lse_q > -1e37f) ? lse_q * 1.44269504088896341f : 1e37f;
 
@@ -664,25 +780,51 @@
 
   if (qrow < Sb) {
     bf16* op = p.dq + (row0 + qrow) * p.lddq + hq * D;
-#pragma unroll
-    for (int dt = 0; dt < DT; ++dt)
-#pragma unroll
-      for (int g = 0; g < 4; ++g) {
-        bf16x4 o;
-#pragma unroll
-        for (int e = 0; e < 4; ++e) o[e] = (bf16)dqt[dt][4 * g + e];
-        *reinterpret_cast<bf16x4*>(op + 32 * dt + 8 * g + 4 * h) = o;
-      }
-  }
-}
-
-}
-
-extern "C" int vlb_attention_bwd(const void* q, int ldq, const void* k, int ldk, const void* v, int ldv, const void* out,
-                                 int ldo, const void* dout, int lddo, const float* lse, const uint8_t* key_mask, void* dq,
-                                 int lddq, void* dk, int lddk, void* dv, int lddv, float* delta, float* dq_acc, int B,
-                                 int S, int Hq, int Hkv, int D, int causal, float scale, const int* cu_rows, int total_rows,
-                                 void* stream) {
+    if constexpr (FUSED) {
+      const int s = p.pos ? p.pos[row0 + qrow] : qrow;
+      const float* cp = p.cs + (int64_t)s * (D / 2) + 4 * h;
+      const float* np = p.sn + (int64_t)s * (D / 2) + 4 * h;
+#pragma unroll
+      for (int dt = 0; dt < DT / 2; ++dt)
+#pragma unroll
+        for (int g = 0; g < 4; ++g) {
+          const f32x4 c4 = *reinterpret_cast<const f32x4*>(cp + 32 * dt + 8 * g);
+          const f32x4 n4 = *reinterpret_cast<const f32x4*>(np + 32 * dt + 8 * g);
+          bf16x4 o0, o1;
+#pragma unroll
+          for (int e = 0; e < 4; ++e) {
+            const float co = c4[e], si = p.rsign * n4[e];
+            float oa, ob;
+            rope_rotate((float)(bf16)dqt[dt][4 * g + e], (float)(bf16)dqt[dt + DT / 2][4 * g + e], co, si, oa, ob);
+            o0[e] = (bf16)oa;
+            o1[e] = (bf16)ob;
+          }
+          *reinterpret_cast<bf16x4*>(op + 32 * dt + 8 * g + 4 * h) = o0;
+          *reinterpret_cast<bf16x4*>(op + 32 * (dt + DT / 2) + 8 * g + 4 * h) = o1;
+        }
+    } else {
+#pragma unroll
+      for (int dt = 0; dt < DT; ++dt)
+#pragma unroll
+        for (int g = 0; g < 4; ++g) {
+          bf16x4 o;
+#pragma unroll
+          for (int e = 0; e < 4; ++e) o[e] = (bf16)dqt[dt][4 * g + e];
+          *reinterpret_cast<bf16x4*>(op + 32 * dt + 8 * g + 4 * h) = o;
+        }
+    }
+  }
+}
+
+}
+
+namespace {
+struct RopeArgs { const float* cs; const float* sn; const int* pos; };
+
+int attention_bwd_impl(const void* q, int ldq, const void* k, int ldk, const void* v, int ldv, const void* out, int ldo,
+                       const void* dout, int lddo, const float* lse, const uint8_t* key_mask, void* dq, int lddq, void* dk,
+                       int lddk, void* dv, int lddv, float* delta, float* dq_acc, int B, int S, int Hq, int Hkv, int D,
+                       int causal, float scale, const int* cu_rows, int total_rows, const RopeArgs* rope, void* stream) {
   VLB_REQUIRE(q && k && v && out && dout && lse && dq && dk && dv && delta, "attention_bwd: null operand");
   VLB_REQUIRE(dq_acc || Hq == Hkv, "attention_bwd: the [rows, Hq, D] fp32-sized workspace is required");
   VLB_REQUIRE(D == 128, "attention_bwd: head dim %d unsupported (only 128: the decoder)", D);
@@ -691,47 +833,94 @@
                   lddk % 4 == 0 && lddv % 4 == 0, "attention_bwd: strides must keep vector alignment");
   VLB_REQUIRE(((((uintptr_t)q | (uintptr_t)k | (uintptr_t)v | (uintptr_t)out | (uintptr_t)dout) % 16) == 0) &&
                   ((uintptr_t)dq % 8 == 0), "attention_bwd: misaligned pointer");
+  if (rope) {
+    VLB_REQUIRE(rope->cs && rope->sn && (((uintptr_t)rope->cs | (uintptr_t)rope->sn) % 16 == 0), "attention_bwd_rope: cos / sin tables missing or misaligned");
+    VLB_REQUIRE(rope->pos || !cu_rows, "attention_bwd_rope: packed rows need their positions");
+  }
   hipStream_t st = as_stream(stream);
   const int64_t rows = cu_rows ? (int64_t)total_rows : (int64_t)B * S;
   VLB_REQUIRE(rows > 0 && rows <= (int64_t)B * S, "attention_bwd: total_rows=%d out of range", total_rows);
-  const int64_t th = rows * Hq;
-  hipLaunchKernelGGL(attn_delta_kernel, dim3((unsigned)((th + 15) / 16)), dim3(256), 0, st, (const bf16*)out, ldo,
-                     (const bf16*)dout, lddo, delta, S, Hq, B, cu_rows, th);
-  VLB_LAUNCH_CHECK();
+  const int gsz = Hq / Hkv;
+  VLB_REQUIRE(gsz == 1 || dq_acc, "attention_bwd: the workspace (fp32 [rows, Hq, D]) is required for grouped-query heads");
+  VLB_REQUIRE(lddk % 8 == 0 && lddv % 8 == 0 && (((uintptr_t)dk | (uintptr_t)dv) % 16) == 0, "attention_bwd: dk/dv rows must be 16-byte aligned");
+
+  auto launch_dq = [&]() -> int {
+    AttnDqArgs d{(const bf16*)q, (const bf16*)k, (const bf16*)v, (const bf16*)dout, lse, delta, key_mask, cu_rows,
+                 (bf16*)dq, ldq, ldk, ldv, lddo, lddq, B, S, Hq, Hkv, scale,
+                 (const bf16*)out, ldo, delta, rope ? rope->cs : nullptr, rope ? rope->sn : nullptr, rope ? rope->pos : nullptr, -1.f};
+    constexpr int LDS_DQ = 2 * 2 * KV * 256;
+    static const hipError_t q1 = hipFuncSetAttribute(reinterpret_cast<const void*>(&attn_bwd_dq_kernel<true>), hipFuncAttributeMaxDynamicSharedMemorySize, LDS_DQ);
+    static const hipError_t q2 = hipFuncSetAttribute(reinterpret_cast<const void*>(&attn_bwd_dq_kernel<false>), hipFuncAttributeMaxDynamicSharedMemorySize, LDS_DQ);
+    static const hipError_t q3 = hipFuncSetAttribute(reinterpret_cast<const void*>(&attn_bwd_dq_kernel<true, true>), hipFuncAttributeMaxDynamicSharedMemorySize, LDS_DQ);
+    static const hipError_t q4 = hipFuncSetAttribute(reinterpret_cast<const void*>(&attn_bwd_dq_kernel<false, true>), hipFuncAttributeMaxDynamicSharedMemorySize, LDS_DQ);
+    if (q1 != hipSuccess || q2 != hipSuccess || q3 != hipSuccess || q4 != hipSuccess) { vlb_set_error("attention_bwd: LDS reservation failed (dq)"); return VLB_ERR_LAUNCH; }
+    dim3 gq(((S + QB - 1) / QB) * Hq * B);
+    if (rope) {
+      if (causal) hipLaunchKernelGGL((attn_bwd_dq_kernel<true, true>), gq, dim3(256), LDS_DQ, st, d);
+      else hipLaunchKernelGGL((attn_bwd_dq_kernel<false, true>), gq, dim3(256), LDS_DQ, st, d);
+    } else {
+      if (causal) hipLaunchKernelGGL(attn_bwd_dq_kernel<true>, gq, dim3(256), LDS_DQ, st, d);
+      else hipLaunchKernelGGL(attn_bwd_dq_kernel<false>, gq, dim3(256), LDS_DQ, st, d);
+    }
+    VLB_LAUNCH_CHECK();
+    return VLB_OK;
+  };
+
+  if (rope) {
+    if (const int rc = launch_dq()) return rc;
+  } else {
+    const int64_t th = rows * Hq;
+    hipLaunchKernelGGL(attn_delta_kernel, dim3((unsigned)((th + 15) / 16)), dim3(256), 0, st, (const bf16*)out, ldo,
+                       (const bf16*)dout, lddo, delta, S, Hq, B, cu_rows, th);
+    VLB_LAUNCH_CHECK();
+  }
   AttnBwdArgs a{(const bf16*)q, (const bf16*)k, (const bf16*)v, (const bf16*)dout, lse, delta, key_mask, cu_rows,
                 (bf16*)dk, (bf16*)dv, dq_acc, ldq, ldk, ldv, lddo, lddk, lddv, B, S, Hq, Hkv, scale, g_attn_ablate};
-  dim3 grid((S + BK_KEYS - 1) / BK_KEYS, Hkv, B);
   {
-    const int gsz = Hq / Hkv;
-    VLB_REQUIRE(gsz == 1 || dq_acc, "attention_bwd: the workspace (fp32 [rows, Hq, D]) is required for grouped-query heads");
-    VLB_REQUIRE(lddk % 8 == 0 && lddv % 8 == 0 && (((uintptr_t)dk | (uintptr_t)dv) % 16) == 0, "attention_bwd: dk/dv rows must be 16-byte aligned");
     constexpr int LDS_KV = BK_KEYS * 256 + 4 * BQ * 256 + 512;
     static const hipError_t k1 = hipFuncSetAttribute(reinterpret_cast<const void*>(&attn_bwd_dkdv_kernel<true>), hipFuncAttributeMaxDynamicSharedMemorySize, LDS_KV);
     static const hipError_t k2 = hipFuncSetAttribute(reinterpret_cast<const void*>(&attn_bwd_dkdv_kernel<false>), hipFuncAttributeMaxDynamicSharedMemorySize, LDS_KV);
     if (k1 != hipSuccess || k2 != hipSuccess) { vlb_set_error("attention_bwd: LDS reservation failed (dk/dv)"); return VLB_ERR_LAUNCH; }
     bf16* part = reinterpret_cast<bf16*>(dq_acc);
-    dim3 gridh(grid.x * Hq * B);
+    dim3 gridh(((S + BK_KEYS - 1) / BK_KEYS) * Hq * B);
     if (causal) hipLaunchKernelGGL(attn_bwd_dkdv_kernel<true>, gridh, dim3(256), LDS_KV, st, a, part);
     else hipLaunchKernelGGL(attn_bwd_dkdv_kernel<false>, gridh, dim3(256), LDS_KV, st, a, part);
     VLB_LAUNCH_CHECK();
-    if (gsz > 1) {
+    if (gsz > 1 && !rope) {
       const int64_t tot = rows * Hkv * 32;
       hipLaunchKernelGGL(attn_dkdv_reduce_kernel, dim3((unsigned)((tot + 255) / 256)), dim3(256), 0, st, part, (bf16*)dk, lddk,
                          (bf16*)dv, lddv, Hq, Hkv, tot);
       VLB_LAUNCH_CHECK();
-    }
-  }
-  AttnDqArgs d{(const bf16*)q, (const bf16*)k, (const bf16*)v, (const bf16*)dout, lse, delta, key_mask, cu_rows,
-               (bf16*)dq, ldq, ldk, ldv, lddo, lddq, B, S, Hq, Hkv, scale};
-  constexpr int LDS_DQ = 2 * 2 * KV * 256;
-  static const hipError_t q1 = hipFuncSetAttribute(reinterpret_cast<const void*>(&attn_bwd_dq_kernel<true>), hipFuncAttributeMaxDynamicSharedMemorySize, LDS_DQ);
-  static const hipError_t q2 = hipFuncSetAttribute(reinterpret_cast<const void*>(&attn_bwd_dq_kernel<false>), hipFuncAttributeMaxDynamicSharedMemorySize, LDS_DQ);
-  if (q1 != hipSuccess || q2 != hipSuccess) { vlb_set_error("attention_bwd: LDS reservation failed (dq)"); return VLB_ERR_LAUNCH; }
-  dim3 gq(((S + QB - 1) / QB) * Hq * B);
-  if (causal) hipLaunchKernelGGL(attn_bwd_dq_kernel<true>, gq, dim3(256), LDS_DQ, st, d);
-  else hipLaunchKernelGGL(attn_bwd_dq_kernel<false>, gq, dim3(256), LDS_DQ, st, d);
-  VLB_LAUNCH_CHECK();
-  return VLB_OK;
+    } else if (gsz > 1) {
+      const int64_t tot = rows * Hkv * 24;
+      hipLaunchKernelGGL(attn_dkdv_reduce_rope_kernel, dim3((unsigned)((tot + 255) / 256)), dim3(256), 0, st, part, (bf16*)dk,
+                         lddk, (bf16*)dv, lddv, Hq, Hkv, tot, rope->cs, rope->sn, rope->pos, S, -1.f);
+      VLB_LAUNCH_CHECK();
+    } else if (rope) {
+      if (const int rc = vlb_rope_inplace(dk, lddk, rope->cs, rope->sn, (int)rows, S, Hkv, D, -1, rope->pos, stream)) return rc;
+    }
+  }
+  return rope ? VLB_OK : launch_dq();
+}
+}
+
+extern "C" int vlb_attention_bwd(const void* q, int ldq, const void* k, int ldk, const void* v, int ldv, const void* out,
+                                 int ldo, const void* dout, int lddo, const float* lse, const uint8_t* key_mask, void* dq,
+                                 int lddq, void* dk, int lddk, void* dv, int lddv, float* delta, float* dq_acc, int B,
+                                 int S, int Hq, int Hkv, int D, int causal, float scale, const int* cu_rows, int total_rows,
+                                 void* stream) {
+  return attention_bwd_impl(q, ldq, k, ldk, v, ldv, out, ldo, dout, lddo, lse, key_mask, dq, lddq, dk, lddk, dv, lddv, delta,
+                            dq_acc, B, S, Hq, Hkv, D, causal, scale, cu_rows, total_rows, nullptr, stream);
+}
+
+extern "C" int vlb_attention_bwd_rope(const void* q, int ldq, const void* k, int ldk, const void* v, int ldv, const void* out,
+                                      int ldo, const void* dout, int lddo, const float* lse, const uint8_t* key_mask,
+                                      void* dq, int lddq, void* dk, int lddk, void* dv, int lddv, float* delta, float* dq_acc,
+                                      int B, int S, int Hq, int Hkv, int D, int causal, float scale, const int* cu_rows,
+                                      int total_rows, const float* cos_t, const float* sin_t, const int* pos, void* stream) {
+  const RopeArgs r{cos_t, sin_t, pos};
+  return attention_bwd_impl(q, ldq, k, ldk, v, ldv, out, ldo, dout, lddo, lse, key_mask, dq, lddq, dk, lddk, dv, lddv, delta,
+                            dq_acc, B, S, Hq, Hkv, D, causal, scale, cu_rows, total_rows, &r, stream);
 }
 
 #ifdef VLB_TOOLS
diff --git a/phantom_vlb_amd/csrc/common.hpp b/phantom_vlb_amd/csrc/common.hpp
--- a/phantom_vlb_amd/csrc/common.hpp
+++ b/phantom_vlb_amd/csrc/common.hpp
@@ -68,6 +68,23 @@
   return t;
 }
 
+__device__ __forceinline__ void rope_rotate(float a, float b, float co, float si, float& oa, float& ob) {
+#pragma clang fp contract(off)
+  const float bs = b * si, as = a * si;
+  oa = __builtin_fmaf(a, co, -bs);
+  ob = __builtin_fmaf(b, co, as);
+}
+__device__ __forceinline__ float dot8_seq(const bf16x8& a, const bf16x8& b) {
+#pragma clang fp contract(off)
+  float s = 0.f;
+#pragma unroll
+  for (int i = 0; i < 8; ++i) {
+    const float m = (float)a[i] * (float)b[i];
+    s = s + m;
+  }
+  return s;
+}
+
 __device__ __forceinline__ float sigmoid_f(float x) { return __builtin_amdgcn_rcpf(1.f + __expf(-x)); }
 __device__ __forceinline__ float silu_f(float x) { return x * sigmoid_f(x); }
 __device__ __forceinline__ float quick_gelu_f(float x) { return x * sigmoid_f(1.702f * x); }
diff --git a/phantom_vlb_amd/csrc/ops.hip b/phantom_vlb_amd/csrc/ops.hip
--- a/phantom_vlb_amd/csrc/ops.hip
+++ b/phantom_vlb_amd/csrc/ops.hip
@@ -283,8 +283,7 @@
 #pragma unroll
     for (int i = 0; i < 8; ++i) {
       const float co = c[i], si = sign * n[i];
-      oa[i] = a[i] * co - b[i] * si;
-      ob[i] = b[i] * co + a[i] * si;
+      rope_rotate(a[i], b[i], co, si, oa[i], ob[i]);
     }
     store8(p, oa); store8(p + half, ob);
   }
diff --git a/phantom_vlb_amd/fullft.py b/phantom_vlb_amd/fullft.py
--- a/phantom_vlb_amd/fullft.py
+++ b/phantom_vlb_amd/fullft.py
@@ -403,16 +403,14 @@
         x, key_mask = bb.splice(ids, vid, layout)
         self._ids_host = ids_host if ids_host is not None else ids.cpu()
         S = g.max_len
-        pos = None if layout is None else layout.pos
         qd, kd = g.heads * g.head_dim, g.kv_heads * g.head_dim
         self.saved = []
         for li in range(g.layers):
             lw = self._enter(li, backward=False)
             h1, h1q = self._norm(x, lw["in_norm"])
             qkv = self._lin(h1, li, "wqkv", xq=h1q)
-            ops.rope_(qkv, w.rope_cos, w.rope_sin, B, S, g.heads + g.kv_heads, g.head_dim, pos=pos)
-            a, lse = ops.attention_fwd(qkv[:, :qd], qkv[:, qd:qd + kd], qkv[:, qd + kd:], B, S, g.heads, g.kv_heads, g.head_dim,
-                                       True, g.head_dim ** -0.5, key_mask=key_mask, need_lse=True, layout=layout)
+            a, lse = ops.rope_attention_fwd(qkv, qd, kd, w.rope_cos, w.rope_sin, B, S, g.heads, g.kv_heads, g.head_dim,
+                                            g.head_dim ** -0.5, key_mask=key_mask, need_lse=True, layout=layout)
             x2 = self._lin(a, li, "wo", residual=x)
             h2, h2q = self._norm(x2, lw["post_norm"])
             gu = self._lin(h2, li, "wgu", xq=h2q)
@@ -432,7 +430,6 @@
         B, S = self.B, g.max_len
         qd, kd = g.heads * g.head_dim, g.kv_heads * g.head_dim
         layout = self.layout
-        pos = None if layout is None else layout.pos
         dx = ops.rmsnorm_bwd_full(self.x_last, w.final_norm, dhidden, g.rms_eps, G("norm"))
         delta = torch.empty(B, g.heads, S, dtype=torch.float32, device=self.dev)
         for li in range(g.layers - 1, -1, -1):
@@ -449,9 +446,8 @@
             dq_ = self._dual(dx2) or (None, None)
             self.wgrad(dx2, sv["a"], G(f"{pre}.wo"), fp8=self.fp8, dyTq=dq_[1])
             d_a = self._lin(dx2, li, "wo_t", xq=dq_[0])
-            dqkv = ops.attention_bwd(sv["qkv"], qd, kd, sv["a"], d_a, sv["lse"], self.key_mask, B, S, g.heads, g.kv_heads,
-                                     g.head_dim, True, g.head_dim ** -0.5, layout=layout, delta=delta)
-            ops.rope_(dqkv, w.rope_cos, w.rope_sin, B, S, g.heads + g.kv_heads, g.head_dim, sign=-1, pos=pos)
+            dqkv = ops.rope_attention_bwd(sv["qkv"], qd, kd, sv["a"], d_a, sv["lse"], self.key_mask, w.rope_cos, w.rope_sin,
+                                          B, S, g.heads, g.kv_heads, g.head_dim, g.head_dim ** -0.5, layout=layout, delta=delta)
             dq_ = self._dual(dqkv) or (None, None)
             self.wgrad(dqkv, sv["h1"], G(f"{pre}.wqkv"), fp8=self.fp8, dyTq=dq_[1])
             d_h1 = self._lin(dqkv, li, "wqkv_t", xq=dq_[0])
diff --git a/phantom_vlb_amd/lora.py b/phantom_vlb_amd/lora.py
--- a/phantom_vlb_amd/lora.py
+++ b/phantom_vlb_amd/lora.py
@@ -292,7 +292,6 @@
     def decoder_forward(self, backbone, x, key_mask, B, layout=None, train=True):
         g, w = self.g, self.w
         S = g.max_len
-        pos = None if layout is None else layout.pos
         qd, kd = g.heads * g.head_dim, g.kv_heads * g.head_dim
         if not train:
             return self._decoder_eval(backbone, x, key_mask, B, layout)
@@ -303,10 +302,8 @@
             sd = [self._seed(li, k) for k in range(7)]
             h1 = ops.rmsnorm(x, lw["in_norm"], g.rms_eps)
             qkv, t_qkv = self._adapted(h1, lw["wqkv"], lay["qkv"], sd[0:3], slot=(li, 0))
-            ops.rope_(qkv, w.rope_cos, w.rope_sin, B, S, g.heads + g.kv_heads, g.head_dim, pos=pos)
-            a, lse = ops.attention_fwd(qkv[:, :qd], qkv[:, qd:qd + kd], qkv[:, qd + kd:], B, S, g.heads, g.kv_heads,
-                                       g.head_dim, True, g.head_dim ** -0.5, key_mask=key_mask, need_lse=True,
-                                       layout=layout)
+            a, lse = ops.rope_attention_fwd(qkv, qd, kd, w.rope_cos, w.rope_sin, B, S, g.heads, g.kv_heads, g.head_dim,
+                                            g.head_dim ** -0.5, key_mask=key_mask, need_lse=True, layout=layout)
             x2, t_o = self._adapted(a, lw["wo"], lay["o"], sd[3:4], residual=x, slot=(li, 1))
             h2 = ops.rmsnorm(x2, lw["post_norm"], g.rms_eps)
             hh, gu, t_gu = self._adapted_mlp_in(h2, lw, lay["gu"], sd[4:6], (li, 2))
@@ -320,15 +317,13 @@
     def _decoder_eval(self, backbone, x, key_mask, B, layout):
         g, w = self.g, self.w
         S = g.max_len
-        pos = None if layout is None else layout.pos
         qd, kd = g.heads * g.head_dim, g.kv_heads * g.head_dim
         for li, lay in enumerate(self.layers):
             lw = backbone.layer_weights(li)
             h = ops.rmsnorm(x, lw["in_norm"], g.rms_eps)
             qkv, _ = self._adapted(h, lw["wqkv"], lay["qkv"], None, slot=(li, 0), p=0.0)
-            ops.rope_(qkv, w.rope_cos, w.rope_sin, B, S, g.heads + g.kv_heads, g.head_dim, pos=pos)
-            a = ops.attention_fwd(qkv[:, :qd], qkv[:, qd:qd + kd], qkv[:, qd + kd:], B, S, g.heads, g.kv_heads, g.head_dim,
-                                  True, g.head_dim ** -0.5, key_mask=key_mask, layout=layout)
+            a = ops.rope_attention_fwd(qkv, qd, kd, w.rope_cos, w.rope_sin, B, S, g.heads, g.kv_heads, g.head_dim,
+                                       g.head_dim ** -0.5, key_mask=key_mask, layout=layout, save_q=False)
             x, _ = self._adapted(a, lw["wo"], lay["o"], None, residual=x, slot=(li, 1), p=0.0)
             h = ops.rmsnorm(x, lw["post_norm"], g.rms_eps)
             hh, _, _ = self._adapted_mlp_in(h, lw, lay["gu"], None, (li, 2), p=0.0, save=False)
@@ -382,7 +377,6 @@
         B, S = self.B, g.max_len
         qd, kd = g.heads * g.head_dim, g.kv_heads * g.head_dim
         layout = self.layout
-        pos = None if layout is None else layout.pos
         M = self.x_last.shape[0]
         dx = ops.rmsnorm_bwd(self.x_last, w.final_norm, dhidden, g.rms_eps)
         delta = torch.empty(B, g.heads, S, dtype=torch.float32, device=self.dev)
@@ -394,9 +388,8 @@
             dx2 = ops.rmsnorm_bwd(sv["x2"], lw["post_norm"], d_h2, g.rms_eps, dx_in=dx)
             d_a = self._group_backward(li, "o", dx2, sv["a"], sv["t_o"], sd[3:4], lw["wo_t"], True)
             qkv = sv["qkv"]
-            dqkv = ops.attention_bwd(qkv, qd, kd, sv["a"], d_a, sv["lse"], self.key_mask, B, S, g.heads, g.kv_heads,
-                                     g.head_dim, True, g.head_dim ** -0.5, layout=layout, delta=delta)
-            ops.rope_(dqkv, w.rope_cos, w.rope_sin, B, S, g.heads + g.kv_heads, g.head_dim, sign=-1, pos=pos)
+            dqkv = ops.rope_attention_bwd(qkv, qd, kd, sv["a"], d_a, sv["lse"], self.key_mask, w.rope_cos, w.rope_sin, B, S,
+                                          g.heads, g.kv_heads, g.head_dim, g.head_dim ** -0.5, layout=layout, delta=delta)
             need_dx = li > 0
             d_h1 = self._group_backward(li, "qkv", dqkv, sv["h1"], sv["t_qkv"], sd[0:3], lw["wqkv_t"], need_dx)
             if need_dx:
diff --git a/phantom_vlb_amd/ops.py b/phantom_vlb_amd/ops.py
--- a/phantom_vlb_amd/ops.py
+++ b/phantom_vlb_amd/ops.py
@@ -258,6 +258,39 @@
                                 out.data_ptr(), out.stride(0), _p(lse), _p(key_mask), B, S, Hq, Hkv, D,
                                 1 if causal else 0, float(scale), _p(cu), _stream()), "vlb_attention_fwd")
     return (out, lse) if need_lse else out
+
+
+FUSE_ROPE_ATTN = True
+
+
+def attention_fwd_rope(qkv, qd, kd, cos, sin, B, S, Hq, Hkv, D, causal, scale, key_mask=None, need_lse=False, out=None,
+                       layout=None, pos=None, save_q=True):
+    _dev(qkv)
+    cu, rows = None, B * S
+    if layout is not None and layout.packed:
+        B, S, cu, rows = layout.B, layout.smax, layout.cu, layout.rows
+    assert qkv.shape[0] == rows, f"attention_fwd_rope: {qkv.shape[0]} rows, layout has {rows}"
+    assert cos.shape[0] >= S and (pos is None) == (cu is None)
+    if out is None:
+        out = torch.empty(rows, Hq * D, dtype=BF16, device=qkv.device)
+    lse = torch.empty(B, Hq, S, dtype=torch.float32, device=qkv.device) if need_lse else None
+    check(lib.vlb_attention_fwd_rope(qkv.data_ptr(), qkv.stride(0), qkv[:, qd:].data_ptr(), qkv.stride(0),
+                                     qkv[:, qd + kd:].data_ptr(), qkv.stride(0), out.data_ptr(), out.stride(0), _p(lse),
+                                     _p(key_mask), B, S, Hq, Hkv, D, 1 if causal else 0, float(scale), _p(cu), rows,
+                                     cos.data_ptr(), sin.data_ptr(), _p(pos), 1 if save_q else 0, _stream()),
+          "vlb_attention_fwd_rope")
+    return (out, lse) if need_lse else out
+
+
+def rope_attention_fwd(qkv, qd, kd, cos, sin, B, S, Hq, Hkv, D, scale, key_mask=None, need_lse=False, layout=None,
+                       save_q=True):
+    pos = None if layout is None else layout.pos
+    if FUSE_ROPE_ATTN and D == 128:
+        return attention_fwd_rope(qkv, qd, kd, cos, sin, B, S, Hq, Hkv, D, True, scale, key_mask=key_mask,
+                                  need_lse=need_lse, layout=layout, pos=pos, save_q=save_q)
+    rope_(qkv, cos, sin, B, S, (qd + kd) // D, D, pos=pos)
+    return attention_fwd(qkv[:, :qd], qkv[:, qd:qd + kd], qkv[:, qd + kd:], B, S, Hq, Hkv, D, True, scale,
+                         key_mask=key_mask, need_lse=need_lse, layout=layout)
 
 
 _ATTN_WS = [None]
@@ -292,6 +325,39 @@
     return dqkv
 
 
+def attention_bwd_rope(qkv, qd, kd, out, dout, lse, key_mask, cos, sin, B, S, Hq, Hkv, D, causal, scale, layout=None,
+                       delta=None, dq_acc=None, pos=None):
+    cu, rows = None, B * S
+    if layout is not None and layout.packed:
+        B, S, cu, rows = layout.B, layout.smax, layout.cu, layout.rows
+    assert qkv.shape[0] == rows and dout.shape[0] == rows
+    assert cos.shape[0] >= S and (pos is None) == (cu is None)
+    if delta is None:
+        delta = torch.empty(B, Hq, S, dtype=torch.float32, device=qkv.device)
+    if dq_acc is None and Hq != Hkv:
+        dq_acc = _attn_workspace(rows * qd, qkv.device)
+    assert delta.numel() >= B * Hq * S and (dq_acc is None or dq_acc.numel() >= rows * qd)
+    dqkv = torch.empty_like(qkv)
+    check(lib.vlb_attention_bwd_rope(qkv.data_ptr(), qkv.stride(0), qkv[:, qd:].data_ptr(), qkv.stride(0),
+                                     qkv[:, qd + kd:].data_ptr(), qkv.stride(0), out.data_ptr(), out.stride(0),
+                                     dout.data_ptr(), dout.stride(0), lse.data_ptr(), _p(key_mask),
+                                     dqkv.data_ptr(), dqkv.stride(0), dqkv[:, qd:].data_ptr(), dqkv.stride(0),
+                                     dqkv[:, qd + kd:].data_ptr(), dqkv.stride(0), delta.data_ptr(), _p(dq_acc),
+                                     B, S, Hq, Hkv, D, 1 if causal else 0, float(scale), _p(cu), rows,
+                                     cos.data_ptr(), sin.data_ptr(), _p(pos), _stream()), "vlb_attention_bwd_rope")
+    return dqkv
+
+
+def rope_attention_bwd(qkv, qd, kd, out, dout, lse, key_mask, cos, sin, B, S, Hq, Hkv, D, scale, layout=None, delta=None):
+    pos = None if layout is None else layout.pos
+    if FUSE_ROPE_ATTN and D == 128:
+        return attention_bwd_rope(qkv, qd, kd, out, dout, lse, key_mask, cos, sin, B, S, Hq, Hkv, D, True, scale,
+                                  layout=layout, delta=delta, pos=pos)
+    dqkv = attention_bwd(qkv, qd, kd, out, dout, lse, key_mask, B, S, Hq, Hkv, D, True, scale, layout=layout, delta=delta)
+    rope_(dqkv, cos, sin, B, S, (qd + kd) // D, D, sign=-1, pos=pos)
+    return dqkv
+
+
 def rmsnorm(x, w, eps, out=None):
     rows, dim = x.shape
     if out is None:
```

After: 15.28 clips/s (median of 6 runs). About the same (+0.4%).
